# cbg-ethz/LongSom

Measured on AMD Instinct MI355X. Metric: genomic sites/s pileup+call, 10M-read BAM x 5k barcodes, 1/2/4/8 MI355X, higher is better.
Workload: dtype u32

## Files before the change

### longsom_amd/csrc/call.hip

```cpp
#include "lsg_ctx.h"
#include "call_rec.h"
#include "bb_tail.h"
#include <cstdio>
#include <cstring>
#include <cstdlib>
#include <hipcub/hipcub.hpp>

namespace lsg {

enum { CT_CAND = 0, CT_NCAND = 1, CT_HEADS = 4, CT_PASS = 6, CT_LIGHT = 16, CT_HEAVY = 32, CT_QTAIL = 48, CT_DEFER = 64, CT_WORDS = 80 };
struct CallArgs {
    const uint32_t* ne_units; const uint64_t* ne_mask; const uint32_t* ne_rowbase; const int2* ne_geom;
    uint32_t n_ne; int32_t n_ct;
    const uint32_t* rows[LSG_MAX_CELLTYPES]; uint64_t row_cap;
    const uint8_t* const* ref_ptr; const int64_t* contig_len;
    lsg_call_params p;
    double lgc0[2], lgcn[2];
    uint32_t* pass_list;
    const int16_t* tail_table;
    uint32_t* site_cnt; uint32_t* site_off;
    SiteRec* sites; CandCt* cands; uint64_t cand_cap;
    struct TailTask* light; struct TailTask* heavy; uint64_t task_cap;
    unsigned long long* counters;
    uint32_t arena_waves;
// ... 215 lines not shown
        h_next = h_new + (tot_h - h_room); h_end = h_new + HEAVY_CHUNK * ((tot_h - h_room + HEAVY_CHUNK - 1) / HEAVY_CHUNK);
    } else h_next += tot_h;
    if (!site) continue;
    const uint32_t cand = cbase + (uint32_t)__popcll(cm & below);
    uint32_t li = pl - n_light, hi = ph - n_heavy;
    const int16_t* TT = a.tail_table;
    auto table_at = [&](uint32_t k, uint32_t n, int set) { return TT[tail_in_table(k, n) ? (uint32_t)set * TAIL_ENTRIES + tail_index(k, n) : 0u]; };
    int16_t t_bc[NCT][4], t_cc[NCT][4];
#pragma unroll
    for (int ct = 0; ct < NCT; ++ct) {
#pragma unroll
        for (int s = 0; s < 4; ++s) { t_bc[ct][s] = 0; t_cc[ct][s] = 0; }
    }
    if (cm) {
#pragma unroll
        for (int ct = 0; ct < NCT; ++ct) {
#pragma unroll
            for (int s = 0; s < 4; ++s) { t_bc[ct][s] = table_at(v_bc[ct][s], v_dp[ct], 0); t_cc[ct][s] = table_at(v_cc[ct][s], v_nc[ct], 1); }
        }
    }
    const int16_t t_nb = table_at((uint32_t)s_alts_bc, (uint32_t)s_dp, 0), t_nc = table_at((uint32_t)s_alts_cc, (uint32_t)s_nc, 1);
    auto emit_task = [&](uint32_t k, uint32_t n, int set, int16_t* dst, int16_t* loc, int16_t from_table) {
        if (tail_in_table(k, n)) { *loc = from_table; return; }
        TailTask t; t.k = k; t.n = n; t.dst = (uint64_t)dst | (uint64_t)set;
        if (tail_work(k, n) > 64) { const uint32_t p = hi < h_room ? h_old + hi : h_new + (hi - h_room); if (p < a.task_cap) a.heavy[p] = t; ++hi; }
        else { const uint32_t p = li < l_room ? l_old + li : l_new + (li - l_room); if (p < a.task_cap) a.light[p] = t; ++li; }
    };

    SiteRec sr;
    sr.key = ((int64_t)tid << 32) | pos; sr.ref = refb; sr.present = 0; sr.considered = 0; sr.has_cand = 0;
    sr.pad[0] = sr.pad[1] = sr.pad[2] = 0; sr.pad2 = 0; sr.cand = has_any ? cand : 0xFFFFFFFFu;
    sr.site_filter = 0;
    int n_considered = 0;
    bool alts_differ = false;
    uint32_t first_altset = 0; bool have_first = false;
    int lc_up = 0, lc_down = 0;
    SiteRec* srp = &a.sites[idx];
    const bool all_known = (n_light | n_heavy) == 0u;
    int f_pass = 0, f_nonsig = 0, f_with = 0; bool f_multi = false;

#pragma unroll
    for (int ct = 0; ct < NCT; ++ct) {
        CandCt cd;
        cd.n_alt = 0; cd.ct_filter = 0; cd.pad[0] = cd.pad[1] = 0;
#pragma unroll
        for (int q = 0; q < LSG_CALL_MAX_ALT; ++q) { cd.alt[q] = 0; cd.alt_bc[q] = 0; cd.alt_cc[q] = 0; cd.p_bc[q] = 0; cd.p_cc[q] = 0; }
        CandCt* cdp = has_any && cand < a.cand_cap ? &a.cands[(uint64_t)cand * NCT + ct] : nullptr;
        if ((mask[ct] >> lane) & 1ull) {
            sr.present |= (uint8_t)(1u << ct);
            const uint32_t dp = v_dp[ct], nc = v_nc[ct];
            if ((int)dp >= P.min_cov && (int)nc >= P.min_cells) {
                sr.considered |= (uint8_t)(1u << ct);
                ++n_considered;
                int na = 0; uint32_t altset = 0;
#pragma unroll
                for (int oi = 0; oi < 4; ++oi) {
                    const int s = order[oi];
                    const uint32_t b = v_bc[ct][s];
                    if (s == rsym || b == 0) continue;
                    const uint32_t c = v_cc[ct][s];
                    if (na < LSG_CALL_MAX_ALT) {
                        cd.alt[na] = (uint8_t)s; cd.alt_bc[na] = b; cd.alt_cc[na] = c;
                        if (cdp) { emit_task(b, dp, 0, &cdp->p_bc[na], &cd.p_bc[na], t_bc[ct][s]); emit_task(c, nc, 1, &cdp->p_cc[na], &cd.p_cc[na], t_cc[ct][s]); }
                    }
                    ++na; altset |= 1u << s;
                }
                cd.n_alt = (uint8_t)na;
                if (na > 0) {
                    sr.has_cand |= (uint8_t)(1u << ct);
                    if (!have_first) { first_altset = altset; have_first = true; } else if (altset != first_altset) alts_differ = true;
                    if (have_ctx) {
                        int first_s = -1, last_s = -1;
                        for (int oi = 0; oi < 4; ++oi) { const int s = order[oi]; if ((altset >> s) & 1u) { if (first_s < 0) first_s = s; last_s = s; } }
                        const int u = base_of_sym(first_s) == up4 ? up_run + 1 : 1;
                        const int ub = u > up_best ? u : up_best;
                        lc_up = ub > lc_up ? ub : lc_up;
                        int db = 1;
                        if (down_len > 0) { const int d = base_of_sym(last_s) == dn0 ? dn_run + 1 : 1; db = d > dn_best ? d : dn_best; }
                        lc_down = db > lc_down ? db : lc_down;
                    }
                }
            }
        }
        if (all_known && cd.n_alt > 0) {
            int32_t min_pbc = 100000, min_pcc = 100000;
#pragma unroll
            for (int q = 0; q < LSG_CALL_MAX_ALT; ++q) if (q < (int)cd.n_alt) { min_pbc = cd.p_bc[q] < min_pbc ? cd.p_bc[q] : min_pbc; min_pcc = cd.p_cc[q] < min_pcc ? cd.p_cc[q] : min_pcc; }
            uint8_t f;
            if (min_pbc >= 500 || min_pcc >= 500) f = LSG_CF_NONSIG;
            else if ((min_pbc > 10 && min_pbc < 500) || (min_pcc > 10 && min_pcc < 500)) f = LSG_CF_LOWSIG;
            else if (cd.n_alt > 1) f = LSG_CF_MULTI;
            else if ((int)cd.alt_cc[0] < P.min_ac_cells) f = LSG_CF_LOW_CELLS;
            else if ((int)cd.alt_bc[0] < P.min_ac_reads) f = LSG_CF_LOW_READS;
            else f = LSG_CF_PASS;
            cd.ct_filter = f;
            ++f_with; f_pass += f == LSG_CF_PASS; f_nonsig += f == LSG_CF_NONSIG; f_multi |= f == LSG_CF_MULTI;
        }
        if (cdp) *cdp = cd;
    }
    sr.cell_types_min = (uint8_t)n_considered;
    sr.sum_alts_bc = s_alts_bc; sr.sum_dp = s_dp; sr.sum_alts_cc = s_alts_cc; sr.sum_nc = s_nc;
    sr.noise_p_bc = -1; sr.noise_p_cc = -1;
    if (s_alts_bc > 0) {
        sr.noise_p_bc = -2; sr.noise_p_cc = -2;
        if (s_dp >= 0) emit_task((uint32_t)s_alts_bc, (uint32_t)s_dp, 0, &srp->noise_p_bc, &sr.noise_p_bc, t_nb);
        if (s_nc >= 0 && s_alts_cc >= 0) emit_task((uint32_t)s_alts_cc, (uint32_t)s_nc, 1, &srp->noise_p_cc, &sr.noise_p_cc, t_nc);
    }
    uint32_t sf = 0;
    if (sr.has_cand) {
        sf |= LSG_SF_CANDIDATE;
        if (alts_differ) sf |= LSG_SF_MULTI_ALLELIC;
        if (n_considered < P.min_cell_types) sf |= LSG_SF_MIN_CELL_TYPES;
        if (have_ctx && lc_up >= 4) sf |= LSG_SF_LC_UP;
        if (have_ctx && lc_down >= 4) sf |= LSG_SF_LC_DOWN;
    }
    bool pass_site = false;
    if (all_known) {
        const int32_t npb = sr.noise_p_bc, npc = sr.noise_p_cc;
        if (sr.has_cand) {
            if (f_pass > P.max_cell_types) sf |= LSG_SF_MULTIPLE_CELL_TYPES;
            if (f_multi) sf |= LSG_SF_MULTI_ALLELIC;
            if (f_with - f_pass - f_nonsig > 0) sf |= LSG_SF_CELL_TYPE_NOISE;
            if (s_alts_bc > 0 && ((npb >= 0 && npb < 500) || (npc >= 0 && npc < 500))) sf |= LSG_SF_NOISY_SITE;
            pass_site = sf == (uint32_t)LSG_SF_CANDIDATE && f_pass > 0;
        } else if (s_alts_bc > 0 && ((npb >= 0 && npb < 10) || (npc >= 0 && npc < 10))) sf |= LSG_SF_NOISY_SITE;
    }
    sr.site_filter = sf;
    *srp = sr;
    if (pass_site) {
        const unsigned long long q = atomicAdd(&a.counters[CT_PASS], 1ull);
        if (q < PASS_CAP) a.pass_list[q] = (uint32_t)idx;
    }
    const unsigned long long dm = __ballot(!all_known);
    if (dm) {
        unsigned long long q0 = 0;
        if (lane == __ffsll((long long)dm) - 1) q0 = atomicAdd(&a.counters[CT_DEFER], (unsigned long long)__popcll(dm));
        q0 = ((unsigned long long)(uint32_t)__shfl((int)(uint32_t)(q0 >> 32), __ffsll((long long)dm) - 1) << 32) | (uint32_t)__shfl((int)(uint32_t)q0, __ffsll((long long)dm) - 1);
        const unsigned long long q = q0 + __popcll(dm & below);
        if (!all_known && q < a.defer_cap) a.defer_list[q] = (uint32_t)idx;
    }
    }
    TailTask nul; nul.k = 0; nul.n = 0; nul.dst = 0;
    for (uint32_t p = l_next + (uint32_t)lane; p < l_end; p += 64) if (p < a.task_cap) a.light[p] = nul;
    for (uint32_t p = h_next + (uint32_t)lane; p < h_end; p += 64) if (p < a.task_cap) a.heavy[p] = nul;
    if (lane == 0 && n_cand_exact) atomicAdd(&a.counters[CT_NCAND], (unsigned long long)n_cand_exact);
}

__device__ __forceinline__ double tail_of_task(const TailTask& t, const CallArgs& a) {
    const int set = (int)(t.dst & 1ull);
    const double al = set ? a.p.alpha2 : a.p.alpha1, be = set ? a.p.beta2 : a.p.beta1;
    return bb_upper_tail(t.k, t.n, al, be, bb_pm0(t.n, al, be, a.lgc0[set]), a.lgcn[set]);
}

__global__ __launch_bounds__(256) void k_call_tails(CallArgs a) {
    const uint64_t n_all = a.counters[CT_LIGHT] + (uint64_t)a.arena_waves * TASK_CHUNK;
    const uint64_t n = n_all < a.task_cap ? n_all : a.task_cap;
    for (uint64_t i = (uint64_t)blockIdx.x * blockDim.x + threadIdx.x; i < n; i += (uint64_t)gridDim.x * blockDim.x) {
        const TailTask t = a.light[i];
        if (!(t.dst & ~1ull)) continue;
        *reinterpret_cast<int16_t*>(t.dst & ~1ull) = (int16_t)round4(tail_of_task(t, a));
    }
}

template <int G>
__device__ __forceinline__ double group_tail(uint32_t k, uint32_t n, int set, const CallArgs& a, int lane, bool live = true) {
    const double al = set ? a.p.alpha2 : a.p.alpha1, be = set ? a.p.beta2 : a.p.beta1;
    const double dn = (double)n;
    const bool lower = (uint64_t)k <= (uint64_t)n - k + 1;
    const uint32_t m_lo = lower ? 0u : k, m_hi = live ? (lower ? k : n + 1) : m_lo;
    const uint32_t cnt = m_hi - m_lo, chunk = (cnt + G - 1) / G;
    const uint32_t b = m_lo + (uint32_t)(lane & (G - 1)) * chunk;
    const uint32_t e = b + chunk < m_hi ? b + chunk : m_hi;
    double sum = 0.0;
    if (b < e) {
        double pm = exp(bb_logpmf((double)b, dn, al, be));
        sum = pm;
        for (uint32_t m = b + 1; m < e; ++m) {
            if (((m - b) & 1023u) == 0) pm = exp(bb_logpmf((double)m, dn, al, be));
            else { const double mm = (double)(m - 1); pm *= (dn - mm) * (mm + al) / ((mm + 1.0) * (dn - mm - 1.0 + be)); }
            sum += pm;
        }
    }
    for (int o = G / 2; o > 0; o >>= 1) sum += __shfl_down(sum, o, G);
    return lower ? 1.0 - sum : sum;
}
__device__ __forceinline__ uint32_t tail_terms(uint32_t k, uint32_t n) { return (uint64_t)k <= (uint64_t)n - k + 1 ? k : n + 1 - k; }
constexpr uint32_t GROUP8_MAX_TERMS = 1024;

__global__ __launch_bounds__(256) void k_tail_table(CallArgs a, int16_t* table) {
    const int lane = threadIdx.x & 63;
    const uint64_t n_thr = (uint64_t)gridDim.x * blockDim.x, tid = (uint64_t)blockIdx.x * blockDim.x + threadIdx.x;
    for (uint64_t i = tid; i < 2ull * TAIL_ENTRIES; i += n_thr) {
        const int set = i >= TAIL_ENTRIES;
        const uint32_t idx = (uint32_t)(i - (set ? TAIL_ENTRIES : 0));
        uint32_t n = (uint32_t)((sqrt(8.0 * (double)idx + 1.0) - 1.0) * 0.5);
        while (tail_index(0, n + 1) <= idx) ++n;
        while (tail_index(0, n) > idx) --n;
        const uint32_t k = idx - tail_index(0, n);
        if (tail_work(k, n) > 64) continue;
        TailTask t; t.k = k; t.n = n; t.dst = (uint64_t)set;
        table[i] = (int16_t)round4(tail_of_task(t, a));
    }
    for (uint64_t i = tid >> 3; i < 2ull * TAIL_ENTRIES; i += n_thr >> 3) {
        const int set = i >= TAIL_ENTRIES;
        const uint32_t idx = (uint32_t)(i - (set ? TAIL_ENTRIES : 0));
        uint32_t n = (uint32_t)((sqrt(8.0 * (double)idx + 1.0) - 1.0) * 0.5);
        while (tail_index(0, n + 1) <= idx) ++n;
        while (tail_index(0, n) > idx) --n;
        const uint32_t k = idx - tail_index(0, n);
        const bool heavy = tail_work(k, n) > 64;
        const double tail = group_tail<8>(k, n, set, a, lane, heavy);
        if (heavy && (lane & 7) == 0) table[i] = (int16_t)round4(tail);
    }
}

__global__ __launch_bounds__(256) void k_call_tails_heavy(CallArgs a) {
    const int lane = threadIdx.x & 63;
    const uint64_t n_all = a.counters[CT_HEAVY] + (uint64_t)a.arena_waves * HEAVY_CHUNK;
    const uint64_t n_tasks = n_all < a.task_cap ? n_all : a.task_cap;
    const uint64_t n_waves = ((uint64_t)gridDim.x * blockDim.x) >> 6;
    uint64_t batch = ((uint64_t)blockIdx.x * blockDim.x + threadIdx.x) >> 6;
    const uint64_t n_batches = (n_tasks + 15) / 16;
    while (batch < n_batches) {
        const uint64_t i = (uint64_t)lane * n_batches + batch;
        TailTask t; t.k = 0; t.n = 0; t.dst = 0;
        if (lane < 16 && i < n_tasks) t = a.heavy[i];
        const bool is_live = (t.dst & ~1ull) != 0;
        const bool is_big = is_live && tail_terms(t.k, t.n) > GROUP8_MAX_TERMS;
#pragma unroll
        for (int round = 0; round < 2; ++round) {
            const int l = 8 * round + (lane >> 3);
            const uint32_t k = (uint32_t)__shfl((int)t.k, l), n = (uint32_t)__shfl((int)t.n, l);
            const uint64_t dst = ((uint64_t)(uint32_t)__shfl((int)(uint32_t)(t.dst >> 32), l) << 32) | (uint32_t)__shfl((int)(uint32_t)t.dst, l);
            const bool mine = (dst & ~1ull) != 0 && tail_terms(k, n) <= GROUP8_MAX_TERMS;
            if (__ballot(mine) == 0ull) continue;
            const double tail = group_tail<8>(k, n, (int)(dst & 1ull), a, lane, mine);
            if (mine && (lane & 7) == 0) *reinterpret_cast<int16_t*>(dst & ~1ull) = (int16_t)round4(tail);
        }
        unsigned long long big = __ballot(is_big);
        while (big) {
            const int l = __ffsll((long long)big) - 1; big &= big - 1;
            const uint32_t k = (uint32_t)__shfl((int)t.k, l), n = (uint32_t)__shfl((int)t.n, l);
            const uint64_t dst = ((uint64_t)(uint32_t)__shfl((int)(uint32_t)(t.dst >> 32), l) << 32) | (uint32_t)__shfl((int)(uint32_t)t.dst, l);
            const double tail = group_tail<64>(k, n, (int)(dst & 1ull), a, lane);
            if (lane == 0) *reinterpret_cast<int16_t*>(dst & ~1ull) = (int16_t)round4(tail);
        }
        unsigned long long nb = 0;
        if (lane == 0) nb = atomicAdd(&a.counters[CT_QTAIL], 1ull) + n_waves;
        batch = ((uint64_t)(uint32_t)__builtin_amdgcn_readfirstlane((int)(uint32_t)(nb >> 32)) << 32) | (uint32_t)__builtin_amdgcn_readfirstlane((int)(uint32_t)nb);
    }
}

__global__ void k_call_finish(CallArgs a, uint32_t n_sites) {
    const unsigned long long n_def = a.counters[CT_DEFER] < a.defer_cap ? a.counters[CT_DEFER] : a.defer_cap;
    for (unsigned long long j = (unsigned long long)blockIdx.x * blockDim.x + threadIdx.x; j < n_def; j += (unsigned long long)gridDim.x * blockDim.x) {
    const uint32_t i = a.defer_list[j];
    if (i >= n_sites) continue;
    SiteRec s = a.sites[i];
    const lsg_call_params& P = a.p;
    const int32_t npb = s.noise_p_bc, npc = s.noise_p_cc;
    const bool bc_lt05 = npb >= 0 && npb < 500, cc_lt05 = npc >= 0 && npc < 500;
    const bool bc_lt001 = npb >= 0 && npb < 10, cc_lt001 = npc >= 0 && npc < 10;
    uint32_t sf = s.site_filter;
    if (s.has_cand) {
        int n_pass = 0, n_nonsig = 0, n_with = 0; bool any_multi = false;
        for (int ct = 0; ct < a.n_ct; ++ct) {
            if (!((s.has_cand >> ct) & 1u)) continue;
            CandCt* d = &a.cands[(uint64_t)s.cand * a.n_ct + ct];
            const int na = d->n_alt;
            int32_t min_pbc = 100000, min_pcc = 100000;
            for (int q = 0; q < na && q < LSG_CALL_MAX_ALT; ++q) { min_pbc = d->p_bc[q] < min_pbc ? d->p_bc[q] : min_pbc; min_pcc = d->p_cc[q] < min_pcc ? d->p_cc[q] : min_pcc; }
            uint8_t f;
            if (min_pbc >= 500 || min_pcc >= 500) f = LSG_CF_NONSIG;
            else if ((min_pbc > 10 && min_pbc < 500) || (min_pcc > 10 && min_pcc < 500)) f = LSG_CF_LOWSIG;
            else if (na > 1) f = LSG_CF_MULTI;
            else if ((int)d->alt_cc[0] < P.min_ac_cells) f = LSG_CF_LOW_CELLS;
            else if ((int)d->alt_bc[0] < P.min_ac_reads) f = LSG_CF_LOW_READS;
            else f = LSG_CF_PASS;
            d->ct_filter = f;
            ++n_with; n_pass += f == LSG_CF_PASS; n_nonsig += f == LSG_CF_NONSIG; any_multi |= f == LSG_CF_MULTI;
        }
        if (n_pass > P.max_cell_types) sf |= LSG_SF_MULTIPLE_CELL_TYPES;
        if (any_multi) sf |= LSG_SF_MULTI_ALLELIC;
        if (n_with - n_pass - n_nonsig > 0) sf |= LSG_SF_CELL_TYPE_NOISE;
        if (s.sum_alts_bc > 0 && (bc_lt05 || cc_lt05)) sf |= LSG_SF_NOISY_SITE;
        if (sf == (uint32_t)LSG_SF_CANDIDATE && n_pass > 0) {
            const unsigned long long idx = atomicAdd(&a.counters[CT_PASS], 1ull);
            if (idx < PASS_CAP) a.pass_list[idx] = i;
        }
    } else if (s.sum_alts_bc > 0 && (bc_lt001 || cc_lt001)) {
        sf |= LSG_SF_NOISY_SITE;
    }
    if (sf != s.site_filter) a.sites[i].site_filter = sf;
    }
}

__device__ __forceinline__ bool keep_site(const SiteRec& s, const CandCt* cands, int n_ct, int kind) {
    if (kind == 0) return true;
    if (kind == 1) return s.site_filter != 0;
    if (s.site_filter != (uint32_t)LSG_SF_CANDIDATE) return false;
    bool pass = false;
    for (int ct = 0; ct < n_ct; ++ct) pass |= cands[(uint64_t)s.cand * n_ct + ct].ct_filter == LSG_CF_PASS;
    return pass;
}
__global__ void k_flag_keep(const SiteRec* sites, const CandCt* cands, int n_ct, int64_t n, int kind, uint32_t* keep) {
    int64_t i = (int64_t)blockIdx.x * blockDim.x + threadIdx.x;
    if (i <= n) keep[i] = (i < n && keep_site(sites[i], cands, n_ct, kind)) ? 1u : 0u;
}
__device__ __forceinline__ void expand_site(const SiteRec& s, const CandCt* cands, int n_ct, const uint8_t* const* ref_ptr, const int64_t* contig_len,
                                            lsg_call* dst) {
    lsg_call c;
    memset(&c, 0, sizeof(c));
    c.key = s.key; c.ref = s.ref; c.present = s.present; c.considered = s.considered; c.has_cand = s.has_cand;
    c.site_filter = s.site_filter; c.cell_types_min = s.cell_types_min;
    c.sum_alts_bc = s.sum_alts_bc; c.sum_dp = s.sum_dp; c.sum_alts_cc = s.sum_alts_cc; c.sum_nc = s.sum_nc;
    c.noise_p_bc = s.noise_p_bc; c.noise_p_cc = s.noise_p_cc;
    if (s.cand != 0xFFFFFFFFu) {
        for (int ct = 0; ct < n_ct; ++ct) {
            const CandCt& d = cands[(uint64_t)s.cand * n_ct + ct];
            c.n_alt[ct] = d.n_alt; c.ct_filter[ct] = d.ct_filter;
            for (int q = 0; q < LSG_CALL_MAX_ALT; ++q) {
                c.alt[ct][q] = d.alt[q]; c.alt_bc[ct][q] = d.alt_bc[q]; c.alt_cc[ct][q] = d.alt_cc[q];
                c.p_bc[ct][q] = d.p_bc[q]; c.p_cc[ct][q] = d.p_cc[q];
            }
        }
    }
    const int tid = (int)(s.key >> 32);
    const int64_t pos = s.key & 0xffffffffll;
    if (pos >= 5) {
        const uint8_t* ref = ref_ptr[tid];
        for (int q = 0; q < 5; ++q) c.up_ctx[q] = ref[pos - 5 + q];
        for (int q = 0; q < 5 && pos + 1 + q < contig_len[tid]; ++q) c.down_ctx[q] = ref[pos + 1 + q];
    }
    *dst = c;
}
__global__ void k_expand(const SiteRec* sites, const CandCt* cands, int n_ct, int64_t n, const uint32_t* keep, const uint32_t* off,
                         const uint8_t* const* ref_ptr, const int64_t* contig_len, lsg_call* out) {
    int64_t i = (int64_t)blockIdx.x * blockDim.x + threadIdx.x;
    if (i >= n || !keep[i]) return;
    expand_site(sites[i], cands, n_ct, ref_ptr, contig_len, out + off[i]);
}
__global__ __launch_bounds__(1024) void k_expand_list(const SiteRec* sites, const CandCt* cands, int n_ct, const uint32_t* list, uint32_t n,
                                                      const uint8_t* const* ref_ptr, const int64_t* contig_len, lsg_call* out) {
    __shared__ uint32_t v[PASS_CAP];
    const uint32_t t = threadIdx.x;
    uint32_t m = 1; while (m < n) m <<= 1;
    for (uint32_t i = t; i < m; i += 1024) v[i] = i < n ? list[i] : 0xFFFFFFFFu;
    __syncthreads();
    for (uint32_t k = 2; k <= m; k <<= 1)
        for (uint32_t j = k >> 1; j > 0; j >>= 1) {
            for (uint32_t i = t; i < m; i += 1024) {
                const uint32_t l = i ^ j;
                if (l > i) {
                    const uint32_t x = v[i], y = v[l];
                    if (((i & k) == 0) == (x > y)) { v[i] = y; v[l] = x; }
                }
            }
            __syncthreads();
        }
    for (uint32_t i = t; i < n; i += 1024) expand_site(sites[v[i]], cands, n_ct, ref_ptr, contig_len, out + i);
}

__global__ void k_probe(const int64_t* set, int64_t n_set, const int64_t* keys, int64_t n, uint8_t* hits) {
    int64_t i = (int64_t)blockIdx.x * blockDim.x + threadIdx.x;
    if (i >= n) return;
    const int64_t key = keys[i];
    int64_t lo = 0, hi = n_set;
    while (lo < hi) { int64_t mid = (lo + hi) >> 1; if (set[mid] < key) lo = mid + 1; else hi = mid; }
    hits[i] = (lo < n_set && set[lo] == key) ? 1 : 0;
}

__global__ void k_sf4_batch(const uint32_t* k, const uint32_t* n, int64_t items, double al, double be, double lgc0, double lgcn, int32_t* out, double* raw) {
    for (int64_t i = (int64_t)blockIdx.x * blockDim.x + threadIdx.x; i < items; i += (int64_t)gridDim.x * blockDim.x) {
        const double p = bb_upper_tail(k[i], n[i], al, be, bb_pm0(n[i], al, be, lgc0), lgcn);
        out[i] = round4(p);
        if (raw) raw[i] = p;
    }
}

int run_sf4(lsg_ctx* c, int64_t items, const uint32_t* k, const uint32_t* n, double al, double be, int32_t* out, double* raw) {
    if (items < 0 || (items > 0 && (!k || !n || !out))) { set_error("lsg_betabinom_sf4: bad arguments"); return -2; }
    if (!(al > 0.0) || !(be > 0.0)) { set_error("lsg_betabinom_sf4: alpha and beta must be positive"); return -2; }
    if (items == 0) return 0;
    hipStream_t st = c->stream;
    DevBuf dk, dn, dout, draw;
    auto done = [&](int rc) { dk.release(); dn.release(); dout.release(); draw.release(); return rc; };
    if (dk.reserve((size_t)items * 4) || dn.reserve((size_t)items * 4) || dout.reserve((size_t)items * 4) || (raw && draw.reserve((size_t)items * 8))) return done(-1);
    if (hipMemcpyAsync(dk.p, k, (size_t)items * 4, hipMemcpyHostToDevice, st) != hipSuccess ||
        hipMemcpyAsync(dn.p, n, (size_t)items * 4, hipMemcpyHostToDevice, st) != hipSuccess) { set_error("lsg_betabinom_sf4: upload failed"); return done(-1); }
    unsigned g = (unsigned)((items + 255) / 256); if (g > (unsigned)(c->n_cus * 16)) g = (unsigned)(c->n_cus * 16);
    hipLaunchKernelGGL(k_sf4_batch, dim3(g), dim3(256), 0, st, dk.as<uint32_t>(), dn.as<uint32_t>(), items, al, be,
                       lgamma(al + be) - lgamma(be), lgamma(al + be) - lgamma(al), dout.as<int32_t>(), raw ? draw.as<double>() : (double*)nullptr);
    if (raw && hipMemcpyAsync(raw, draw.p, (size_t)items * 8, hipMemcpyDeviceToHost, st) != hipSuccess) { set_error("lsg_betabinom_sf4: failed"); return done(-1); }
    if (hipMemcpyAsync(out, dout.p, (size_t)items * 4, hipMemcpyDeviceToHost, st) != hipSuccess || hipStreamSynchronize(st) != hipSuccess) { set_error("lsg_betabinom_sf4: failed"); return done(-1); }
    return done(0);
}

struct HasSites {
    const uint32_t* cnt;
    __host__ __device__ bool operator()(const uint32_t& w) const { return cnt[w] != 0; }
};

static int run_call_sized(lsg_ctx* c, const lsg_call_params* p, uint32_t tasks_per_site);
int run_call(lsg_ctx* c, const lsg_call_params* p) {
    int rc = run_call_sized(c, p, c->call_tasks_per_site);
    if (rc == -3) {
        c->call_tasks_per_site = (uint32_t)(8 * c->n_ct + 2);
        rc = run_call_sized(c, p, c->call_tasks_per_site);
    }
    return rc;
}
static int run_call_sized(lsg_ctx* c, const lsg_call_params* p, uint32_t tasks_per_site) {
    if (!c->counted) { set_error("lsg_call_step1: call lsg_pileup_count first"); return -2; }
    for (int t = 0; t < c->n_contigs; ++t)
        if (!c->ref_ptr[t]) { set_error("lsg_call_step1: reference of contig %d not loaded", t); return -2; }
    hipStream_t st = c->stream;
    const uint32_t n_ne = c->n_ne;
    c->n_sites = 0; c->n_cand = 0; c->n_pass = -1;
    if (n_ne == 0) { c->called = true; return 0; }
    if (c->d_site_off.reserve((size_t)(n_ne + 2) * 12 + 128 + CT_WORDS * 8 + (size_t)n_ne * 72 + 64)) return -1;
    CallArgs a{};
    a.ne_units = c->d_ne_units.as<uint32_t>(); a.ne_mask = c->d_ne_mask.as<uint64_t>(); a.ne_rowbase = c->d_ne_rowbase.as<uint32_t>();
    a.ne_geom = c->ws[WS_NE_GEOM].as<int2>();
    a.n_ne = n_ne; a.n_ct = c->n_ct;
    for (int i = 0; i < LSG_MAX_CELLTYPES; ++i) a.rows[i] = c->d_rows[i].as<uint32_t>();
    for (int i = 0; i < c->n_ct; ++i) if (!a.rows[i] || c->d_rows[i].cap < ROW_BLOCK_WORDS * 4) { set_error("lsg_call_step1: a cell type has no row block"); return -2; }
    a.row_cap = c->row_cap;
    a.ref_ptr = c->d_ref_ptrs.as<const uint8_t*>(); a.contig_len = c->d_contig_len.as<int64_t>();
    a.p = *p;
    a.lgc0[0] = lgamma(p->alpha1 + p->beta1) - lgamma(p->beta1); a.lgcn[0] = lgamma(p->alpha1 + p->beta1) - lgamma(p->alpha1);
    a.lgc0[1] = lgamma(p->alpha2 + p->beta2) - lgamma(p->beta2); a.lgcn[1] = lgamma(p->alpha2 + p->beta2) - lgamma(p->alpha2);
    {
        const double key[4] = {p->alpha1, p->beta1, p->alpha2, p->beta2};
        if (!c->tail_table_valid || memcmp(key, c->tail_table_key, sizeof key) != 0) {
            if (c->d_tail_table.reserve((size_t)2 * TAIL_ENTRIES * 2)) return -1;
            hipLaunchKernelGGL(k_tail_table, dim3((unsigned)(c->n_cus * 8)), dim3(256), 0, st, a, c->d_tail_table.as<int16_t>());
            memcpy(c->tail_table_key, key, sizeof key); c->tail_table_valid = true;
        }
        a.tail_table = c->d_tail_table.as<int16_t>();
    }
    if (c->d_pass_list.reserve((size_t)PASS_CAP * 4)) return -1;
    a.pass_list = c->d_pass_list.as<uint32_t>();
    a.site_cnt = c->d_site_off.as<uint32_t>();
    a.site_off = a.site_cnt + (n_ne + 2);
    a.counters = reinterpret_cast<unsigned long long*>(a.site_off + (n_ne + 2));
    uint32_t* heads = reinterpret_cast<uint32_t*>(a.counters + CT_WORDS);
    a.heads = heads;
    a.head_recs = reinterpret_cast<uint32_t*>((reinterpret_cast<uintptr_t>(heads + n_ne) + 63) & ~(uintptr_t)63);
    a.head_ref = reinterpret_cast<uint64_t*>(a.head_recs + (size_t)n_ne * 16);
    LSG_HIP(hipMemsetAsync(a.counters, 0, CT_WORDS * 8, st));
    hipLaunchKernelGGL(k_site_count, dim3((n_ne + 256) / 256), dim3(256), 0, st, a);
    size_t tb = 0;
    LSG_HIP(hipcub::DeviceScan::ExclusiveSum(nullptr, tb, a.site_cnt, a.site_off, (int)(n_ne + 1), st));
    if (c->d_cub_tmp.reserve(tb + 256)) return -1;
    tb = c->d_cub_tmp.cap;
    LSG_HIP(hipcub::DeviceScan::ExclusiveSum(c->d_cub_tmp.p, tb, a.site_cnt, a.site_off, (int)(n_ne + 1), st));
    {
        HasSites pred{a.site_cnt};
        hipcub::CountingInputIterator<uint32_t> it(0);
        uint32_t* d_nh = reinterpret_cast<uint32_t*>(a.counters + CT_HEADS);
        size_t tb2 = 0;
        LSG_HIP(hipcub::DeviceSelect::If(nullptr, tb2, it, heads, d_nh, (int)n_ne, pred, st));
        if (c->d_cub_tmp.reserve(tb2 + 256)) return -1;
        tb2 = c->d_cub_tmp.cap;
        LSG_HIP(hipcub::DeviceSelect::If(c->d_cub_tmp.p, tb2, it, heads, d_nh, (int)n_ne, pred, st));
    }
    hipLaunchKernelGGL(k_head_recs, dim3((n_ne + 255) / 256), dim3(256), 0, st, a);
    LSG_HIP(hipMemcpyAsync(c->h_pin, a.site_off + n_ne, 4, hipMemcpyDeviceToHost, st));
    LSG_HIP(hipStreamSynchronize(st));
    const uint32_t n_sites = *reinterpret_cast<const uint32_t*>(c->h_pin);
    if (n_sites > 0) {
        if (c->d_calls.reserve((size_t)n_sites * sizeof(SiteRec))) return -1;
        const unsigned gather_grid = (unsigned)(c->n_cus * 4);
        const uint64_t gather_waves = (uint64_t)gather_grid * GATHER_WAVES;
        if (c->ws[WS_CALL_CANDS].reserve(((size_t)n_sites + (size_t)2 * gather_waves * CAND_CHUNK) * sizeof(CandCt) * (size_t)c->n_ct)) return -1;
        a.arena_waves = (uint32_t)gather_waves;
        a.sites = c->d_calls.as<SiteRec>(); a.cands = c->ws[WS_CALL_CANDS].as<CandCt>(); a.cand_cap = n_sites + 2 * gather_waves * CAND_CHUNK;
        a.task_cap = (uint64_t)n_sites * (uint64_t)(8 * c->n_ct + 2);
        if (a.task_cap > (uint64_t)n_sites * tasks_per_site + 1024) a.task_cap = (uint64_t)n_sites * tasks_per_site + 1024;
        if (a.task_cap > 0x7fffffffull) a.task_cap = 0x7fffffffull;
        a.task_cap += gather_waves * TASK_CHUNK * 3;
        if (c->ws[WS_CALL_TASKS].reserve((size_t)a.task_cap * sizeof(TailTask) * 2)) return -1;
        a.light = c->ws[WS_CALL_TASKS].as<TailTask>(); a.heavy = a.light + a.task_cap;
        a.defer_cap = n_sites;
        if (c->d_defer_list.reserve((size_t)a.defer_cap * 4 + 64)) return -1;
        a.defer_list = c->d_defer_list.as<uint32_t>();
        switch (c->n_ct) {
            case 1: hipLaunchKernelGGL(k_call_gather<1>, dim3(gather_grid), dim3(GATHER_WAVES * 64), 0, st, a); break;
            case 2: hipLaunchKernelGGL(k_call_gather<2>, dim3(gather_grid), dim3(GATHER_WAVES * 64), 0, st, a); break;
            case 3: hipLaunchKernelGGL(k_call_gather<3>, dim3(gather_grid), dim3(GATHER_WAVES * 64), 0, st, a); break;
            default: hipLaunchKernelGGL(k_call_gather<4>, dim3(gather_grid), dim3(GATHER_WAVES * 64), 0, st, a); break;
        }
        hipLaunchKernelGGL(k_call_tails, dim3((unsigned)(c->n_cus * 16)), dim3(256), 0, st, a);
        hipLaunchKernelGGL(k_call_tails_heavy, dim3((unsigned)(c->n_cus * 8)), dim3(256), 0, st, a);
        hipLaunchKernelGGL(k_call_finish, dim3((unsigned)(c->n_cus * 2)), dim3(256), 0, st, a, n_sites);
        LSG_HIP(hipGetLastError());
    }
    unsigned long long cnt4[CT_WORDS];
    LSG_HIP(hipMemcpyAsync(c->h_pin, a.counters, CT_WORDS * 8, hipMemcpyDeviceToHost, st));
    LSG_HIP(hipStreamSynchronize(st));
    memcpy(cnt4, c->h_pin, CT_WORDS * 8);
    if (getenv("LSG_TIMING")) fprintf(stderr, "[lsg] call: %u sites in %llu tiles, light task slots %llu (+%llu of the first chunks), heavy %llu (+%llu), sites that waited for a tail %llu, PASS %llu\n", n_sites, cnt4[CT_HEADS],
                                      cnt4[CT_LIGHT], (unsigned long long)a.arena_waves * TASK_CHUNK, cnt4[CT_HEAVY], (unsigned long long)a.arena_waves * HEAVY_CHUNK, cnt4[CT_DEFER], cnt4[CT_PASS]);
    c->n_pass = (int64_t)cnt4[CT_PASS];
    const unsigned long long cand = cnt4[CT_NCAND];
    if (n_sites > 0 && (cnt4[CT_LIGHT] + (uint64_t)a.arena_waves * TASK_CHUNK > a.task_cap || cnt4[CT_HEAVY] + (uint64_t)a.arena_waves * HEAVY_CHUNK > a.task_cap)) { set_error("lsg_call_step1: tail task buffer too small (%llu/%llu tasks)", cnt4[CT_LIGHT], cnt4[CT_HEAVY]); return -3; }
    c->n_sites = n_sites; c->n_cand = (int64_t)cand;
    c->called = true;
    return 0;
}

int run_select_calls(lsg_ctx* c, int kind, lsg_call* dst_device, int64_t capacity, int64_t* n_out) {
    if (!c->called) { set_error("lsg_export_calls: call lsg_call_step1 first"); return -2; }
    hipStream_t st = c->stream;
    const int64_t n = c->n_sites;
    if (n_out) *n_out = 0;
    if (n == 0) return 0;
    if (kind == 2 && c->n_pass >= 0 && c->n_pass <= (int64_t)PASS_CAP && !getenv("LSG_NO_PASS_LIST")) {
        const int64_t k = c->n_pass;
        if (n_out) *n_out = k;
        if (!dst_device || k == 0) return 0;
        if (k > capacity) { set_error("lsg_export_calls: capacity %lld < %lld rows", (long long)capacity, (long long)k); return -2; }
        hipLaunchKernelGGL(k_expand_list, dim3(1), dim3(1024), 0, st, c->d_calls.as<SiteRec>(), c->ws[WS_CALL_CANDS].as<CandCt>(), c->n_ct,
                           c->d_pass_list.as<uint32_t>(), (uint32_t)k, c->d_ref_ptrs.as<const uint8_t*>(), c->d_contig_len.as<int64_t>(), dst_device);
        LSG_HIP(hipGetLastError());
        LSG_HIP(hipStreamSynchronize(st));
        if (getenv("LSG_TIMING")) fprintf(stderr, "[lsg] export: kind 2 from the PASS list, %lld rows\n", (long long)k);
        return 0;
    }
    DevBuf& flags = c->ws[WS_CALL_FLAGS];
    if (flags.reserve((size_t)(n + 2) * 8)) return -1;
    uint32_t* keep = flags.as<uint32_t>();
    uint32_t* off = keep + (n + 2);
    const SiteRec* sites = c->d_calls.as<SiteRec>();
    const CandCt* cands = c->ws[WS_CALL_CANDS].as<CandCt>();
    hipLaunchKernelGGL(k_flag_keep, dim3((unsigned)((n + 256) / 256)), dim3(256), 0, st, sites, cands, c->n_ct, n, kind, keep);
    size_t tb = 0;
    LSG_HIP(hipcub::DeviceScan::ExclusiveSum(nullptr, tb, keep, off, (int)(n + 1), st));
    if (c->d_cub_tmp.reserve(tb + 256)) return -1;
    tb = c->d_cub_tmp.cap;
    LSG_HIP(hipcub::DeviceScan::ExclusiveSum(c->d_cub_tmp.p, tb, keep, off, (int)(n + 1), st));
    LSG_HIP(hipMemcpyAsync(c->h_pin, off + n, 4, hipMemcpyDeviceToHost, st));
    LSG_HIP(hipStreamSynchronize(st));
    const uint32_t k = *reinterpret_cast<const uint32_t*>(c->h_pin);
    if (n_out) *n_out = k;
    if (!dst_device || k == 0) return 0;
    if ((int64_t)k > capacity) { set_error("lsg_export_calls: capacity %lld < %lld rows", (long long)capacity, (long long)k); return -2; }
    hipLaunchKernelGGL(k_expand, dim3((unsigned)((n + 255) / 256)), dim3(256), 0, st, sites, cands, c->n_ct, n, keep, off,
                       c->d_ref_ptrs.as<const uint8_t*>(), c->d_contig_len.as<int64_t>(), dst_device);
    LSG_HIP(hipGetLastError());
    LSG_HIP(hipStreamSynchronize(st));
    if (kind == 2 && getenv("LSG_TIMING")) fprintf(stderr, "[lsg] export: kind 2 from the scan, %u rows\n", k);
    return 0;
}

int run_fetch_calls(lsg_ctx* c, lsg_call* out, int64_t capacity, int candidates_only, int64_t* n_out) {
    if (!c->called) { set_error("lsg_fetch_calls: call lsg_call_step1 first"); return -2; }
    hipStream_t st = c->stream;
    if (n_out) *n_out = 0;
    if (c->n_sites == 0) return 0;
    int64_t k = 0;
    int rc = run_select_calls(c, candidates_only, nullptr, 0, &k);
    if (rc) return rc;
    if (k > capacity) { set_error("lsg_fetch_calls: capacity %lld < %lld rows", (long long)capacity, (long long)k); return -2; }
    if (k > 0) {
        DevBuf& sel = c->ws[WS_CALL_SEL];
        if (sel.reserve((size_t)k * sizeof(lsg_call))) return -1;
        rc = run_select_calls(c, candidates_only, sel.as<lsg_call>(), k, &k);
        if (rc) return rc;
        LSG_HIP(hipMemcpyAsync(out, sel.p, (size_t)k * sizeof(lsg_call), hipMemcpyDeviceToHost, st));
        LSG_HIP(hipStreamSynchronize(st));
    }
    if (n_out) *n_out = k;
    return 0;
}

int run_probe(lsg_ctx* c, const PosSet& s, const char* who, const int64_t* keys, int64_t n, uint8_t* hits, int on_device) {
    hipStream_t st = c->stream;
    if (n == 0) return 0;
    DevBuf dk, dh;
    const int64_t* k = keys; uint8_t* h = hits;
    int rc = 0;
    if (!on_device) {
        if (dk.reserve((size_t)n * 8) || dh.reserve((size_t)n)) { dk.release(); dh.release(); return -1; }
        if (hipMemcpyAsync(dk.p, keys, (size_t)n * 8, hipMemcpyHostToDevice, st) != hipSuccess) rc = -1;
        k = dk.as<int64_t>(); h = dh.as<uint8_t>();
    }
    if (!rc) {
        hipLaunchKernelGGL(k_probe, dim3((unsigned)((n + 255) / 256)), dim3(256), 0, st, s.keys.as<int64_t>(), s.n, k, n, h);
        if (!on_device && hipMemcpyAsync(hits, dh.p, (size_t)n, hipMemcpyDeviceToHost, st) != hipSuccess) rc = -1;
        if (hipStreamSynchronize(st) != hipSuccess) rc = -1;
    }
    if (rc) set_error("%s: %s", who, hipGetErrorString(hipGetLastError()));
    dk.release(); dh.release();
    return rc;
}

}
```

### longsom_amd/csrc/lsg_ctx.h

```cpp
#pragma once
#include <hip/hip_runtime.h>
#include <cstdint>
#include <cstdio>
#include <string>
#include <vector>
#include "../../include/longsom_hip.h"
#include "../../include/longsom_synth.h"

namespace lsg {

constexpr int TILE_W = 64;
constexpr int ROW_PLANES = 34;
constexpr int NCTR = 33;

constexpr int ROW_QUADS = (ROW_PLANES + 3) / 4;
constexpr uint64_t ROW_BLOCK_WORDS = (uint64_t)ROW_QUADS * 256;
constexpr uint64_t ROW_STORED_WORDS = (uint64_t)ROW_QUADS * 4;
constexpr uint32_t ROW_NARROW = 1u << 31;
constexpr uint32_t ROW_NARROW_MAX = 256;
static_assert(ROW_NARROW_MAX * 255u < (1u << 16), "a narrow row's quality sum (two planes share a word) fits 16 bits");
__host__ __device__ inline uint64_t row_word(uint64_t row, int plane) {
    return (row >> 6) * ROW_BLOCK_WORDS + (uint64_t)(plane >> 2) * 256 + (row & 63) * 4 + (uint64_t)(plane & 3);
}

void set_error(const char* fmt, ...);
const char* get_error();

#define LSG_HIP(call)                                                                          \
    do {                                                                                       \
        hipError_t e_ = (call);                                                                \
        if (e_ != hipSuccess) {                                                                \
            lsg::set_error("%s failed: %s (%s:%d)", #call, hipGetErrorString(e_), __FILE__, __LINE__); \
            return -1;                                                                         \
        }                                                                                      \
    } while (0)

struct DevBuf {
    void* p = nullptr;
    size_t cap = 0;
    int reserve(size_t bytes) {
        if (bytes <= cap) return 0;
        if (p) { (void)hipFree(p); p = nullptr; cap = 0; }
        const size_t slack = bytes / 16 < ((size_t)64 << 20) ? bytes / 16 : ((size_t)64 << 20);
        size_t want = bytes + slack + 256;
        LSG_HIP(hipMalloc(&p, want));
        cap = want;
        return 0;
    }
    void release() { if (p) (void)hipFree(p); p = nullptr; cap = 0; }
    template <class T> T* as() const { return reinterpret_cast<T*>(p); }
};

struct PosSet { DevBuf keys; int64_t n = 0; };

struct CellGeno {
    DevBuf keys, alt_sym, is_chrm, dp, alt, vaf4, p4, status, bin, n_cov, n_pass, text, scratch, filt;
    int64_t n_sites = 0; int32_t n_cb = 0; bool valid = false;
    bool cells_only = false;
    bool text_valid = false; int64_t n_long = 0, n_mat = 0; int32_t n_cols = 0, float_cells = 0;
    size_t head_off_at = 0, index_off_at = 0, label_off_at = 0, cb_off_at = 0, ct_off_at = 0, long_order_at = 0, mat_order_at = 0, col_src_at = 0,
           head_at = 0, index_at = 0, label_at = 0, cb_at = 0, ct_at = 0;
    bool filt_valid = false; int64_t n_rows_kept = 0; int32_t n_cols_kept = 0;
    size_t f_row_mut_at = 0, f_cov_kept_at = 0, f_cov_all_at = 0, f_rows_at = 0, f_cols_at = 0, f_nsel_at = 0, f_row_keep_at = 0, f_col_keep_at = 0,
           f_col_int_at = 0, f_col_ok_at = 0;
    void release() { for (DevBuf* b : {&keys, &alt_sym, &is_chrm, &dp, &alt, &vaf4, &p4, &status, &bin, &n_cov, &n_pass, &text, &scratch, &filt}) b->release(); valid = text_valid = filt_valid = false; }
};

struct Bnpc {
    DevBuf lab, raw, params, dist, cuts, sums, rank, flags, owner, cl16, idx, mean, part, ord2, small;
    DevBuf work, wsmall, rec;
    std::vector<double> Z;
    std::vector<int32_t> cut_order;
    int64_t n_samples = 0; int32_t n_cells = 0, pitch = 0, k_max = 0, n_muts = 0;
    bool valid = false, dist_valid = false, has_params = false, tree_valid = false;
    void release() {
        for (DevBuf* b : {&lab, &raw, &params, &dist, &cuts, &sums, &rank, &flags, &owner, &cl16, &idx, &mean, &part, &ord2, &small, &work, &wsmall, &rec}) b->release();
        Z = {}; cut_order = {};
        valid = dist_valid = has_params = tree_valid = false;
    }
};

struct Bnpcs {
    DevBuf one, zero, pop, seeds, lab, size, colof, live, nlive, hi, theta, L1, L0, LL, alpha, prow, n1, n0, rowml, rowb, order, keys, rec_lab, rec_sc, arena, err;
    DevBuf sm_i, sm_d, sm_c, sm_t, rec_sm;
    DevBuf rates, rec_err, err_cnt, err_out;
    DevBuf psrf, psrf_out;
    DevBuf used;
    double err_prob = 0.0, err_prior[4] = {}, mix[2] = {};
    bool learn = false, fixed_assign = false;
    double sm_prob = 0.0, sm_ratio[2] = {0.75, 0.25};
    int32_t sm_scans = 3;
    int32_t n_cells = 0, n_muts = 0, n_words = 0, n_chains = 0, steps1 = 0, k_max = 0, ll_pitch = 0, pending = -1, next_step = 0;
    int32_t test_ml_end = 0;
    int64_t arena_rows = 0;
    double p = 1.0, q = 1.0, g0 = 0.0, g1 = 0.0, dpa_prob = 0.0, betaln = 0.0;
    bool valid = false, prepared = false;
    std::vector<int32_t> h_k;
    std::vector<int64_t> h_used;
    void release() {
        for (DevBuf* b : {&one, &zero, &pop, &seeds, &lab, &size, &colof, &live, &nlive, &hi, &theta, &L1, &L0, &LL, &alpha, &prow, &n1, &n0, &rowml, &rowb, &order, &keys, &rec_lab, &rec_sc,
                          &arena, &err, &sm_i, &sm_d, &sm_c, &sm_t, &rec_sm, &rates, &rec_err, &err_cnt, &err_out, &psrf, &psrf_out, &used}) b->release();
        valid = prepared = false;
    }
};

struct Bbfit {
    DevBuf hist, tails, out, ref, tmp;
    int64_t cap = 0;
    bool valid = false;
    void release() { for (DevBuf* b : {&hist, &tails, &out, &ref, &tmp}) b->release(); valid = false; cap = 0; }
};

struct GeneCounts {
    DevBuf iv, row_of_gene, matrix, tallies, state, small, text, scratch;
    int64_t n_iv = 0; int32_t n_genes = 0, n_rows = 0, n_cb = 0, n_cols = 0; char sep = ',';
    bool ann_valid = false, mat_valid = false, text_valid = false;
    size_t row_off_at = 0, col_src_at = 0, col_off_at = 0, row_txt_at = 0, col_txt_at = 0;
    void release() { for (DevBuf* b : {&iv, &row_of_gene, &matrix, &tallies, &state, &small, &text, &scratch}) b->release(); ann_valid = mat_valid = text_valid = false; n_iv = 0; n_genes = n_rows = n_cb = n_cols = 0; }
};

enum { WS_NE_NSLOT = 0, WS_NE_ACC, WS_NE_GEOM, WS_MULTI_LIST, WS_MACC, WS_EXPORT_K, WS_EXPORT_R,
       WS_EXPORT_C, WS_CALL_FLAGS, WS_CALL_SEL, WS_CALL_CANDS, WS_CALL_TASKS, WS_SEG_INFO };

constexpr uint32_t CB_MASK = 0x00FFFFFFu;
constexpr uint32_t TM_RUNSTART = 1u << 31, TM_FWD = 1u << 30, TM_WHI = 1u << 29;
constexpr uint32_t TM_PAD_S0 = CB_MASK | TM_RUNSTART;
constexpr int TM_GROUP = 4;
enum { TM_STORE = 0, TM_S0, TM_B, TM_RD, TM_META, TM_BLK_TILE, TM_BLK_OFF, TM_EXT,
       TM_JOBS, TM_NE_UNITS, TM_NE_GEOM, TM_NE_NSLOT, TM_NE_ACC, TM_MULTI, TM_CHUNKS, TM_NBUF };
struct TmJob { uint32_t e0, e1, w0, slab, nj, cnt, tile, emid, base, off; int32_t tstart, tid; };
constexpr int TM_JOB_WORDS = 12;
static_assert(sizeof(TmJob) == 4 * TM_JOB_WORDS, "TmJob layout");
constexpr uint32_t TMJ_WIDE = 1u << 31;
constexpr int TM_JOB_TGT = 3072, TM_JOB_LIMIT = 4095;

}

struct lsg_ctx;
namespace lsg {
int build_store(lsg_ctx* c, const uint16_t* events, int64_t n_events, const int64_t* seg_ev_off, const lsg_reads* src = nullptr);
int ensure_plan(lsg_ctx* c);
void drop_store(lsg_ctx* c);
int live_read_bound(lsg_ctx* c);
int live_read_bound_exact(lsg_ctx* c);
int live_read_bound_all(lsg_ctx* c);
__global__ void k_read_end(const uint32_t* seg_read, const int32_t* seg_start, const int32_t* seg_len, int64_t n_segs, int32_t* read_end);
__global__ void k_read_end_init(const int32_t* read_pos, int64_t n_reads, int32_t* read_end);
int depth_cap_drops(lsg_ctx* c, const lsg_count_params* p);
struct GatherCountSrc { const uint16_t* events; int64_t n_events; const uint64_t* key; const uint32_t* rdv; int32_t cb_bits; int32_t src_shift; int32_t wsh; };
int unit_row_offsets(lsg_ctx* c, int ct, const uint32_t** off);
int run_gather_count(lsg_ctx* c, const lsg_count_params* p, const GatherCountSrc& src, bool direct);
}

struct lsg_ctx {
    int device = 0;
    hipStream_t stream = nullptr;
    hipStream_t own_stream = nullptr;
    hipStream_t copy_stream = nullptr;
    hipEvent_t ev_copy = nullptr;
    hipEvent_t ev_blk = nullptr;
    hipEvent_t ev_lpt = nullptr;
    hipEvent_t ev[6] = {nullptr, nullptr, nullptr, nullptr, nullptr, nullptr};
    hipEvent_t evb[5] = {nullptr, nullptr, nullptr, nullptr, nullptr};

    int32_t n_contigs = 0;
    std::vector<int64_t> contig_len;
    std::vector<uint32_t> tile_base;
    uint32_t n_tiles = 0;
    uint32_t tile_lo = 0, tile_hi = 0;
    lsg::DevBuf d_tile_base, d_contig_len, d_ref_ptrs;
    std::vector<lsg::DevBuf> ref;
    std::vector<const uint8_t*> ref_ptr;

    int32_t n_cb = 0, n_ct = 0;
    lsg::DevBuf d_celltype_of, d_ct_rank;
    std::vector<uint8_t> h_celltype_of;
    uint32_t ct_size[LSG_MAX_CELLTYPES] = {0, 0, 0, 0};

    lsg_reads rd{};
    lsg::DevBuf b_read_tid, b_read_pos, b_read_flag, b_read_mapq, b_read_cb;
    lsg::DevBuf b_seg_read, b_seg_start, b_seg_len, b_seg_ev_off, b_events;
    int32_t plp_window = 50000, st_window = 50000;
    int32_t lf_min_mq = 0, lf_ignore_orphans = 0; uint32_t lf_flag_exclude = 0;
    int32_t st_min_mq = 0, st_ignore_orphans = 0; uint32_t st_flag_exclude = 0;
    bool keep_unlisted = false;
    int32_t split_max_nm = -1, split_max_nh = -1, split_n_trim = 0;
    int64_t split_n[18] = {}, split_first[18] = {};
    bool keep_reads = false;
    lsg::DevBuf d_tile_cap, d_tile_off;
    lsg::DevBuf tm[lsg::TM_NBUF];
    lsg::DevBuf bt[18];
    uint64_t tm_n = 0;
    int64_t tm_events = 0;
    uint64_t tm_np = 0;
    uint32_t tm_nblk = 0, tm_njobs = 0, tm_nchunks = 0, tm_n_ne = 0, tm_n_multi = 0, tm_n_slabs = 0, tm_n_wide = 0;
    int plan_n_ct = 0;
    int plan1_n_ct = 0;
    uint32_t plan1_tot[4] = {0, 0, 0, 0};
    uint32_t plan_misc[2] = {0, 0};
    uint32_t* d_plan_misc = nullptr;
    bool cal_enabled = false; lsg_count_params cal_params{};
    bool counted_at_load = false;
    bool load_was_fused = false;
    bool tm_valid = false;
    int32_t store_policy = 0;
    bool store_skipped = false;
    double layout_build_ms = 0;
    float build_ms[4] = {0, 0, 0, 0};
    int64_t max_live_reads = -1;
    int64_t max_live_all = -1;
    int32_t wsh = 0;
    int32_t events_layout = 0;
    const void* hint_phased_events = nullptr;
    bool src_phased = false;
    bool line_loads = false;
    int64_t max_live_exact = -1;
    lsg::DevBuf d_read_drop;
    lsg::DevBuf d_drop_pairs; int64_t n_drop_pairs = 0;
    lsg::DevBuf d_read_adm;
    bool has_drops = false;
    int64_t n_depth_dropped = 0;

    lsg::DevBuf d_read_key;
    lsg::DevBuf d_ne_units, d_ne_mask, d_ne_rowbase, d_ne_rowoff, d_scalars, d_cub_tmp, d_ix_stat;
    lsg::DevBuf d_rows[LSG_MAX_CELLTYPES];
    uint64_t row_cap = 0;
    uint32_t arena = 256;
    uint32_t n_ne = 0;
    int64_t n_rows[LSG_MAX_CELLTYPES] = {0, 0, 0, 0};
    int64_t n_columns = 0;
    lsg_count_params last_params{};
    lsg_count_stats stats{};
    bool counted = false;

    lsg::DevBuf d_calls, d_site_off, d_tail_table;
    double tail_table_key[4] = {0, 0, 0, 0}; bool tail_table_valid = false;
    int64_t n_sites = 0, n_cand = 0, n_pass = -1;
    lsg::DevBuf d_pass_list, d_defer_list, d_xcd_queues;
    uint32_t call_tasks_per_site = 1;
    bool called = false;

    lsg::DevBuf tab_keys[LSG_MAX_CELLTYPES], tab_refs[LSG_MAX_CELLTYPES], tab_rows[LSG_MAX_CELLTYPES], tab_names, tab_scratch, tab_scratch2;
    int32_t tab_scratch_table = -1; int64_t tab_scratch_rows = 0;
    uint64_t tab_rows_serial[LSG_MAX_CELLTYPES] = {0, 0, 0, 0};
    uint64_t count_serial = 0;
    lsg::DevBuf tab_text[LSG_TABLE_ALL_SLOTS];
    int64_t tab_bytes[LSG_TABLE_ALL_SLOTS];
    lsg_ctx() { for (auto& b : tab_bytes) b = -1; }
    int32_t tab_n_contigs = 0, tab_n_ct = 0; uint32_t tab_ct_off_at = 0, tab_order_at = 0, tab_ct_txt_at = 0, tab_contig_txt_at = 0;

    lsg::CellGeno cg;

    lsg::Bnpc bnpc;
    lsg::Bnpcs bnpcs;
    lsg::Bbfit bb;
    lsg::GeneCounts gc;

    lsg::PosSet posset[3];
    lsg::PosSet alleleset; bool alleleset_loaded = false;
    lsg::DevBuf syn[12];
    lsg::DevBuf gen[10];
    lsg::DevBuf ws[16];
    int n_cus = 256;
    unsigned long long* h_pin = nullptr;
    uint32_t n_multi = 0;
};
```

### longsom_amd/csrc/pileup.hip

```cpp
#include "lsg_ctx.h"
#include <hipcub/hipcub.hpp>
#include <cstdio>
#include <cstdlib>
#include <cstring>

namespace lsg {

#define LSG_AS3 __attribute__((address_space(3)))
__device__ __forceinline__ uint32_t lds_addr(const void* p) { return (uint32_t)(uintptr_t)(LSG_AS3 const void*)p; }
constexpr int ARENA = 256;

enum { SC_COLS = 8, SC_OVERFLOW = 9, SC_READS = 10, SC_SEGS = 11, SC_EVENTS = 12, SC_ROWS_DEEP = 15,
       SC_ROWS = 16, SC_ROWS_SRC = 28, SC_NENT = 38, SC_QWALK = 48,
       SC_ROWALLOC = 160, SC_ROWALLOC_STRIDE = 16, SC_COUNT = SC_ROWALLOC + SC_ROWALLOC_STRIDE * LSG_MAX_CELLTYPES };

struct CountArgs {
    int64_t n_reads;
    const int32_t* read_tid; const uint16_t* read_flag; const uint8_t* read_mapq; const int32_t* read_cb;
    const int64_t* contig_len; const uint8_t* const* ref_ptr;
    const uint8_t* celltype_of;
    int32_t n_contigs, n_cb, n_ct;
    uint32_t tile_lo, tile_hi;
    int32_t min_bq, min_mq, min_dp, min_cc, ignore_orphans;
    uint32_t flag_exclude;
// ... 1420 lines not shown
            if (jb.nj == 1 && mine) { const int64_t pos = (int64_t)jb.tstart + 64 * wv + lane; if (pos >= 1 && pos < a.contig_len[jb.tid]) refb = a.ref_ptr[jb.tid][pos]; }
            __syncthreads();
            q.ask();
            if (counting) tm_zero_planes<2 * 2 * 2 * 8 * 64, 2 * 2 * 64>(pl, &nc_sh[0][0][0]);
            __syncthreads();
            const uint32_t s0r = wv ? jb.emid : jb.e0, s1r = wv ? jb.e1 : jb.emid;
            const uint32_t i0 = s0r - jb.base, i1 = s1r - jb.base < jb.tcnt ? s1r - jb.base : jb.tcnt;
            if (counting && i1 > i0) {
                TmState st0, st1; st0.nc = 0; st0.mask = 0; st1.nc = 0; st1.mask = 0;
                tw_range(a, tm, tg, st0, st1, stat, i0, i1, jb.off, jb.tcnt, thr, pkl0, one, lane, K64, kb);
                uint32_t* nq = &nc_sh[0][lane >> 5][2 * (lane & 31)];
                if (st0.nc & 0xffffu) atomicAdd(nq, st0.nc & 0xffffu);
                if (st0.nc >> 16) atomicAdd(nq + 128, st0.nc >> 16);
                if (st1.nc & 0xffffu) atomicAdd(nq + 1, st1.nc & 0xffffu);
                if (st1.nc >> 16) atomicAdd(nq + 129, st1.nc >> 16);
            }
            if (threadIdx.x == 0) s_q[2] = q.answer();
            const JobRec cj = jb;
            jb.load(jw);
            prefetch();
            __syncthreads();
            const uint32_t nn = rl(s_q[2], 0);
            if (mine) {
                for (int v = 0; v < 2; ++v) {
                    const int ct = tm.ct_base + v;
                    if (ct >= a.n_ct) break;
                    const uint32_t uw = (uint32_t)wv * (uint32_t)a.n_ct + (uint32_t)ct;
                    tm_finish<TwCounters>(a, pl + v * 1024 + wv * 512, nc_sh[v][wv][lane], cj.w0 + uw, cj.slab + uw * cj.nj, cj.nj, cj.tcnt, ct, cj.tid, cj.tstart + 64 * wv,
                                          lane, &book, refb, 2 * v);
                }
            }
            if (nxt == XcdQueue::NO_JOB) break;
            cur = nxt; nxt = nn;
        }
    }
    lds_fence();
    __syncthreads();
    stat_flush(tg.stat_slots, stat, lane, wv);
    books_flush(a, books, lane);
}

struct WideEntry {
    bool rs; uint32_t cls; bool fwd;
    uint32_t nev; bool segfirst;
    uint32_t ev[2];
};
__device__ __forceinline__ uint32_t tm_meta_one(const CountArgs& a, const TmArgs& tm, uint64_t p) {
    const uint32_t s = tm.s0[p], b8 = tm.b[p], cb = s & CB_MASK;
    uint32_t cls = 2;
    bool ok = cb < (uint32_t)a.n_cb;
    if (ok && a.adm) { const uint32_t r = tm.rd[p]; ok = (reinterpret_cast<const uint32_t*>(a.adm)[r >> 5] >> (r & 31u)) & 1u; }
    if (ok && a.drop_pairs && a.read_drop[tm.rd[p]] == 2) ok = !tm_dropped_here(a, tm.rd[p], tm.blk_tile[p >> 3], s);
    if (ok) { const uint32_t ct = a.celltype_of[cb]; if (ct < (uint32_t)a.n_ct && (ct >> 1) == (uint32_t)(tm.ct_base >> 1)) cls = ct & 1u; }
    uint32_t m = cls < 2 ? (cls ? (TMM_CT4 | TMM_CT12) : 0u) | ((s & TM_FWD) ? TMM_FWD : 0u) | ((b8 & 128u) ? TMM_SINGLE : 0u) : TMM_SKIP;
    if (s & TM_RUNSTART) m |= TMM_RS;
    return m;
}
struct WideFromStore {
    static constexpr int H = 1;
    int inline_meta;
    __device__ __forceinline__ unsigned long long* stat_slots() const { return nullptr; }
    __device__ __forceinline__ WideEntry entry(const CountArgs& a, const TmArgs& tm, const TmJob&, uint32_t p, int lane) const {
        const uint32_t m = rl(inline_meta ? tm_meta_one(a, tm, p) : tm.meta[p], 0);
        WideEntry e{(m & TMM_RS) != 0, (m & TMM_SKIP) ? 2u : ((m & TMM_CT4) ? 1u : 0u), (m & TMM_FWD) != 0, 0u, false, {0u, 0u}};
        if (e.cls < 2) {
            const uint32_t x = tm.ext[p >> 3];
            if ((uint32_t)lane >= (x & 0xffu) && (uint32_t)lane < (x >> 8)) e.ev[0] = reinterpret_cast<const uint16_t*>(tm.store)[((uint64_t)(p >> 3) * 64 + lane) * 8 + (p & 7u)];
        }
        return e;
    }
};
template <int WSH>
struct WideFromKeys {
    static constexpr int H = 1 << WSH;
    TgArgs tg;
    __device__ __forceinline__ unsigned long long* stat_slots() const { return tg.stat_slots; }
    __device__ __forceinline__ WideEntry entry(const CountArgs& a, const TmArgs& tm, const TmJob& jb, uint32_t p, int lane) const {
        constexpr uint32_t PB = 6 + WSH, PM = (1u << PB) - 1u;
        const uint32_t i = p - jb.base, cbm = (1u << tg.cb_bits) - 1u;
        const uint64_t k = tg.key[jb.off + i];
        const uint32_t v = tg.rdv ? tg.rdv[jb.off + i] : (uint32_t)(k >> 32) & (TG_RV_FWD | TG_RV_SEGFIRST), cb = (uint32_t)k & cbm, r = v & TG_RV_READ;
        const uint32_t geom = (uint32_t)(k >> tg.cb_bits), first = geom & PM, nev = ((geom >> PB) & PM) + 1u;
        const uint64_t src = (((k >> (tg.cb_bits + 2 * PB)) & tg.src_mask) << tg.src_shift) | (tg.src_shift ? first : 0u);
        uint32_t cls = 2;
        bool ok = cb < (uint32_t)a.n_cb;
        if (ok && a.adm) ok = (reinterpret_cast<const uint32_t*>(a.adm)[r >> 5] >> (r & 31u)) & 1u;
        if (ok) { const uint32_t ct = a.celltype_of[cb]; if (ct < (uint32_t)a.n_ct && (ct >> 1) == (uint32_t)(tm.ct_base >> 1)) cls = ct & 1u; }
        WideEntry e{i == 0 || ((uint32_t)tg.key[jb.off + i - 1] & cbm) != cb, cls, (v & TG_RV_FWD) != 0, nev, (v & TG_RV_SEGFIRST) != 0, {0u, 0u}};
        if (cls < 2)
            for (int h = 0; h < H; ++h) { const uint32_t q = (uint32_t)(64 * h + lane) - first; if (q < nev) e.ev[h] = tg.events[src + q]; }
        return e;
    }
};
static_assert(TM_JOB_TGT <= TM_JOB_LIMIT, "a one-job tile's job fits the packed planes: the wide walk writes slabs only");
template <class SRC>
__global__ __launch_bounds__(64) void k_tm_walk_wide(CountArgs a, TmArgs tm, SRC src, const uint32_t* n_wide) {
    constexpr int H = SRC::H;
    __shared__ uint32_t pl[H][2][4][8 * 64];
    const int lane = threadIdx.x;
    if (n_wide && rl(*n_wide, 0) == 0u) return;
    const uint32_t thr = bq_threshold(a);
    unsigned long long s_ev = 0, s_sg = 0, s_ne = 0;
    for (uint32_t jx = blockIdx.x; jx < tm.njobs; jx += gridDim.x) {
        const TmJob jb = tm.jobs[jx];
        bool in_t[H], any = false;
        for (int h = 0; h < H; ++h) { const uint32_t t = (uint32_t)H * jb.tile + h; in_t[h] = t >= a.tile_lo && t < a.tile_hi; any |= in_t[h]; }
        if (!(jb.nj & TMJ_WIDE) || !any) continue;
        const uint32_t nj = jb.nj & ~TMJ_WIDE;
        lds_fence();
        for (int i = lane; i < H * 2 * 4 * 8 * 64; i += 64) (&pl[0][0][0][0])[i] = 0;
        lds_fence();
        uint32_t nc[H][2], mask[H], run_ct = 0;
        for (int h = 0; h < H; ++h) { nc[h][0] = nc[h][1] = 0; mask[h] = 0; }
        for (uint32_t p = jb.e0; p < jb.e1 && p - jb.base < jb.cnt; ++p) {
            const WideEntry e = src.entry(a, tm, jb, p, lane);
            if (e.rs) for (int h = 0; h < H; ++h) { nc[h][run_ct] += mask[h] ? 1u : 0u; mask[h] = 0; }
            if (e.cls >= 2) continue;
            s_ev += e.nev; s_sg += e.segfirst ? 1u : 0u; ++s_ne;
            run_ct = e.cls;
            for (int h = 0; h < H; ++h) {
                const uint32_t ev = e.ev[h];
                if ((ev & 0x8ffu) >= thr) {
                    const uint32_t sym = (ev >> 8) & 7u;
                    uint32_t* w = &pl[h][run_ct][0][sym * 64 + lane];
                    w[0] += ev & 0xffu; w[512] += e.fwd ? 1u : 0u; w[1024] += 1u; w[1536] += (mask[h] >> sym) & 1u;
                    mask[h] |= 1u << sym;
                }
            }
        }
        for (int h = 0; h < H; ++h) nc[h][run_ct] += mask[h] ? 1u : 0u;
        lds_fence();
        for (int h = 0; h < H; ++h) {
            if (!in_t[h]) continue;
            for (int v = 0; v < 2; ++v) {
                const int ct = tm.ct_base + v;
                if (ct >= a.n_ct) break;
                const uint32_t* pc = &pl[h][v][0][0];
                uint32_t dp = 0;
#pragma unroll
                for (int k = 0; k < 8; ++k) dp += pc[1024 + k * 64 + lane];
                uint32_t* dst = a.macc + (uint64_t)(jb.slab + ((uint32_t)h * (uint32_t)a.n_ct + (uint32_t)ct) * nj) * (NCTR * 64);
                dst[lane] = dp - nc[h][v];
#pragma unroll
                for (int k = 0; k < 8; ++k) {
                    dst[(1 + k) * 64 + lane] = pc[1536 + k * 64 + lane]; dst[(9 + k) * 64 + lane] = pc[1024 + k * 64 + lane];
                    dst[(17 + k) * 64 + lane] = pc[k * 64 + lane]; dst[(25 + k) * 64 + lane] = pc[512 + k * 64 + lane];
                }
            }
        }
    }
    if (unsigned long long* slots = src.stat_slots()) stat_add(slots, blockIdx.x, s_ev, s_sg, s_ne, lane);
}

struct CountLaunch { CountArgs a; TmArgs tm; unsigned grid_walk, grid_fin; int n_pass; };
struct PrepOp { void* dst; const void* src; uint64_t words; };
struct PrepArgs { PrepOp op[10]; int n; };
__global__ __launch_bounds__(256) void k_prep_ops(PrepArgs a) {
    const uint64_t g = (uint64_t)blockIdx.x * blockDim.x + threadIdx.x, gs = (uint64_t)gridDim.x * blockDim.x;
    for (int k = 0; k < a.n; ++k) {
        uint32_t* d = reinterpret_cast<uint32_t*>(a.op[k].dst);
        const uint32_t* sp = reinterpret_cast<const uint32_t*>(a.op[k].src);
        const uint64_t nq = a.op[k].words / 4;
        for (uint64_t i = g; i < nq; i += gs) reinterpret_cast<uint4*>(d)[i] = sp ? reinterpret_cast<const uint4*>(sp)[i] : make_uint4(0u, 0u, 0u, 0u);
        for (uint64_t i = nq * 4 + g; i < a.op[k].words; i += gs) d[i] = sp ? sp[i] : 0u;
    }
}
static int count_prepare(lsg_ctx* c, const lsg_count_params* p, CountLaunch& L) {
    hipStream_t st = c->stream;
    const uint32_t n_ne = c->tm_n_ne;
    if (c->d_scalars.reserve(SC_COUNT * 8) || c->d_ne_units.reserve(((size_t)n_ne + 2) * 4) ||
        c->d_ne_mask.reserve(((size_t)n_ne + 2) * 8) || c->d_ne_rowbase.reserve(((size_t)n_ne + 2) * 4) || c->ws[WS_NE_NSLOT].reserve(((size_t)n_ne + 2) * 4) ||
        c->ws[WS_NE_ACC].reserve(((size_t)n_ne + 2) * 4) || c->ws[WS_NE_GEOM].reserve(((size_t)n_ne + 2) * 8) || c->ws[WS_MULTI_LIST].reserve(((size_t)c->tm_n_multi + 2) * 4) ||
        c->ws[WS_MACC].reserve(((size_t)c->tm_n_slabs + 1) * NCTR * 64 * 4) || c->d_ix_stat.reserve(IX_STAT_SLOTS * 64) ||
        c->d_read_adm.reserve(((size_t)c->rd.n_reads / 64 + 2) * 8))
        return -1;
    L.grid_walk = (unsigned)(c->n_cus * tune_int("LSG_GRID_TM", 16));
    L.grid_fin = (unsigned)(c->n_cus * 8);
    L.n_pass = (c->n_ct + 1) / 2;
    {
        uint64_t want_rows = (uint64_t)n_ne / (uint64_t)c->n_ct * TILE_W;
        if (p->min_dp > 0) {
            const uint64_t by_depth = (uint64_t)c->rd.n_events / (uint64_t)p->min_dp + 64;
            if (by_depth < want_rows) want_rows = by_depth;
        }
        const uint64_t emitters = (uint64_t)L.grid_walk * TMW_WAVES * 2 + L.grid_fin + (uint64_t)c->n_cus * 4 + (c->wsh ? (uint64_t)c->n_cus * 16 * TMW_WAVES * 4 : 0u);
        uint64_t arena = want_rows / (emitters * 8) / ARENA * ARENA;
        c->arena = (uint32_t)(arena < (uint64_t)ARENA ? (uint64_t)ARENA : (arena > 8ull * ARENA ? 8ull * ARENA : arena));
        want_rows += emitters * c->arena + 64;
        want_rows = (want_rows + 63) / 64 * 64 + 64;
        if (want_rows > c->row_cap) c->row_cap = want_rows;
        for (int i = 0; i < c->n_ct; ++i)
            if (c->d_rows[i].reserve((size_t)c->row_cap * ROW_STORED_WORDS * 4)) return -1;
    }
    c->n_ne = n_ne; c->n_multi = c->tm_n_multi;
    L.a = CountArgs{};
    fill_args(c, p, L.a);
    TmArgs& tm = L.tm;
    tm = TmArgs{};
    tm.store = c->tm[TM_STORE].as<uint4>(); tm.s0 = c->tm[TM_S0].as<uint32_t>(); tm.b = c->tm[TM_B].as<uint8_t>(); tm.rd = c->tm[TM_RD].as<uint32_t>();
    tm.meta = c->tm[TM_META].as<uint32_t>(); tm.blk_tile = c->tm[TM_BLK_TILE].as<uint32_t>(); tm.jobs = c->tm[TM_JOBS].as<TmJob>(); tm.np = c->tm_np; tm.nblk = c->tm_nblk;
    tm.njobs = c->tm_njobs; tm.nchunks = c->tm_nchunks; tm.chunk_start = c->tm[TM_CHUNKS].as<uint32_t>(); tm.ext = c->tm[TM_EXT].as<uint16_t>();
    LSG_HIP(hipEventRecord(c->ev[0], st));
    {
        PrepArgs pa{}; int k = 0;
        auto op = [&](void* dst, const void* src, size_t bytes) { if (bytes) { pa.op[k].dst = dst; pa.op[k].src = src; pa.op[k].words = (bytes + 3) / 4; ++k; } };
        op(c->d_scalars.p, nullptr, SC_COUNT * 8);
        op(c->d_ix_stat.p, nullptr, IX_STAT_SLOTS * 64);
        if (n_ne) {
            op(c->d_ne_units.p, c->tm[TM_NE_UNITS].p, (size_t)n_ne * 4);
            op(c->ws[WS_NE_GEOM].p, c->tm[TM_NE_GEOM].p, (size_t)n_ne * 8);
            op(c->ws[WS_NE_NSLOT].p, c->tm[TM_NE_NSLOT].p, ((size_t)n_ne + 1) * 4);
            op(c->ws[WS_NE_ACC].p, c->tm[TM_NE_ACC].p, ((size_t)n_ne + 1) * 4);
            if (c->tm_n_multi) op(c->ws[WS_MULTI_LIST].p, c->tm[TM_MULTI].p, (size_t)c->tm_n_multi * 4);
            op(c->d_ne_mask.p, nullptr, ((size_t)n_ne + 1) * 8);
            op(c->d_ne_rowbase.p, nullptr, ((size_t)n_ne + 1) * 4);
        }
        pa.n = k;
        hipLaunchKernelGGL(k_prep_ops, dim3((unsigned)(c->n_cus * 4)), dim3(256), 0, st, pa);
    }
    const int64_t R = c->rd.n_reads;
    if (R > 0) { unsigned g = (unsigned)((R + 255) / 256); if (g > (unsigned)(c->n_cus * 8)) g = (unsigned)(c->n_cus * 8); hipLaunchKernelGGL(k_read_stats, dim3(g), dim3(256), 0, st, L.a); }
    return 0;
}
static int count_passes(lsg_ctx* c, CountLaunch& L, int first_pass, bool wide_of_pass0) {
    hipStream_t st = c->stream;
    const unsigned grid_wide = c->tm_n_wide ? (c->tm_n_wide < (unsigned)(c->n_cus * 4) ? c->tm_n_wide : (unsigned)(c->n_cus * 4)) : 0u;
    for (int pass = wide_of_pass0 ? 0 : first_pass; pass < L.n_pass && c->tm_nblk; ++pass) {
        const bool wide_only = pass < first_pass;
        if (wide_only && !grid_wide) continue;
        L.tm.ct_base = 2 * pass;
        if (pass) LSG_HIP(hipMemsetAsync(L.a.scalars + SC_QWALK, 0, 8, st));
        if (L.a.drop_pairs) hipLaunchKernelGGL(k_tm_resolve<true>, dim3((c->tm_nblk + 255) / 256), dim3(256), 0, st, L.a, L.tm, wide_only ? (unsigned long long*)nullptr : c->d_ix_stat.as<unsigned long long>());
        else hipLaunchKernelGGL(k_tm_resolve<false>, dim3((c->tm_nblk + 255) / 256), dim3(256), 0, st, L.a, L.tm, wide_only ? (unsigned long long*)nullptr : c->d_ix_stat.as<unsigned long long>());
        if (pass == 0) { LSG_HIP(hipEventRecord(c->ev[1], st)); LSG_HIP(hipEventRecord(c->ev[3], st)); }
        if (c->tm_njobs && !wide_only) hipLaunchKernelGGL(k_tm_walk, dim3(L.grid_walk), dim3(TMW_WAVES * 64), 0, st, L.a, L.tm);
        if (pass == 0) LSG_HIP(hipEventRecord(c->ev[4], st));
        if (grid_wide) hipLaunchKernelGGL(k_tm_walk_wide<WideFromStore>, dim3(grid_wide), dim3(64), 0, st, L.a, L.tm, WideFromStore{0}, (const uint32_t*)nullptr);
    }
    return 0;
}
static int count_finish(lsg_ctx* c, const lsg_count_params* p, CountLaunch& L) {
    hipStream_t st = c->stream;
    if (c->tm_nblk) hipLaunchKernelGGL(k_resolve_stats, dim3(1), dim3(256), 0, st, L.a, c->d_ix_stat.as<unsigned long long>());
    if (c->tm_n_multi) hipLaunchKernelGGL(k_finalize_multi, dim3(c->tm_n_multi < L.grid_fin ? c->tm_n_multi : L.grid_fin), dim3(FIN_THREADS), 0, st, L.a);
    LSG_HIP(hipEventRecord(c->ev[5], st));
    LSG_HIP(hipGetLastError());
    unsigned long long sc[SC_COUNT];
    if (read_scalars(c, sc)) return -1;
    if (sc[SC_OVERFLOW]) { set_error("lsg_pileup_count: row buffer overflow (cap %llu)", (unsigned long long)c->row_cap); return -3; }
    for (int i = 0; i < LSG_MAX_CELLTYPES; ++i) c->n_rows[i] = (int64_t)sc[SC_ROWS + i];
    c->n_columns = (int64_t)sc[SC_COLS];
    c->stats.n_reads_admitted = (int64_t)sc[SC_READS];
    c->stats.n_segs_admitted = (int64_t)sc[SC_SEGS];
    c->stats.n_events_admitted = (int64_t)sc[SC_EVENTS];
    c->stats.n_units = c->n_ne;
    c->stats.n_deep_units = c->tm_n_multi;
    c->stats.n_entries = (int64_t)sc[SC_NENT];
    float ms = 0;
    LSG_HIP(hipEventElapsedTime(&ms, c->ev[0], c->ev[1])); c->stats.ms_bin = ms;
    LSG_HIP(hipEventElapsedTime(&ms, c->ev[1], c->ev[5])); c->stats.ms_deep = ms;
    LSG_HIP(hipEventElapsedTime(&ms, c->ev[3], c->ev[4])); c->stats.ms_walk = ms;
    c->stats.ms_wave = 0;
    LSG_HIP(hipEventElapsedTime(&ms, c->ev[0], c->ev[5])); c->stats.ms_total = ms;
    for (int i = 0; i < 4; ++i) { c->stats.rows_by_kernel[i] = (int64_t)sc[SC_ROWS_SRC + i]; c->stats.events_by_kernel[i] = 0; }
    c->stats.events_by_kernel[1] = (int64_t)sc[SC_EVENTS];
    c->stats.n_events_wave = 0; c->stats.n_events_deep = (int64_t)sc[SC_EVENTS];
    c->stats.n_rows_deep = (int64_t)sc[SC_ROWS_DEEP];
    c->stats.n_rows_wave = -c->stats.n_rows_deep;
    for (int i = 0; i < LSG_MAX_CELLTYPES; ++i) c->stats.n_rows_wave += c->n_rows[i];
    c->last_params = *p;
    c->counted = true;
    c->called = false;
    ++c->count_serial;
    return 0;
}

int run_gather_count(lsg_ctx* c, const lsg_count_params* p, const GatherCountSrc& src, bool direct) {
    hipStream_t st = c->stream;
    c->has_drops = false; c->n_depth_dropped = 0;
    CountLaunch L;
    if (int rc = count_prepare(c, p, L)) return rc;
    TgArgs tg{};
    tg.events = src.events; tg.n_events = src.n_events; tg.key = src.key; tg.rdv = src.rdv; tg.cb_bits = src.cb_bits;
    tg.src_mask = (1ull << ((src.rdv ? 52 : 50) - src.cb_bits)) - 1ull; tg.src_shift = src.src_shift;
    if (!src.rdv && (!direct || L.a.adm)) return 1;
    tg.tile_off = c->d_tile_off.as<uint32_t>(); tg.blk_off = c->tm[TM_BLK_OFF].as<uint32_t>();
    tg.s0 = c->tm[TM_S0].as<uint32_t>(); tg.b8 = c->tm[TM_B].as<uint8_t>(); tg.rd = c->tm[TM_RD].as<uint32_t>();
    tg.store = c->tm[TM_STORE].as<uint4>(); tg.ext = c->tm[TM_EXT].as<uint16_t>();
    tg.nchunks = c->d_plan_misc + 1; tg.stat_slots = c->d_ix_stat.as<unsigned long long>();
    L.tm.ct_base = 0;
    const bool dbg = getenv("LSG_DEBUG_SYNC") != nullptr;
    auto stage = [&](const char* what) { if (dbg) { const hipError_t e = hipStreamSynchronize(st); fprintf(stderr, "[lsg] fused load: %s: %s\n", what, hipGetErrorString(e)); fflush(stderr); } };
    stage("count prepared");
    LSG_HIP(hipEventRecord(c->ev[1], st)); LSG_HIP(hipEventRecord(c->ev[3], st));
    enum { GATHER, TILES, WINDOWS } form = !direct ? GATHER : (src.wsh ? WINDOWS : TILES);
    const char* what = "k_tm_gather_count";
    if (direct) {
        if (c->d_xcd_queues.reserve(8 * 128)) return -1;
        LSG_HIP(hipMemsetAsync(c->d_xcd_queues.p, 0, 8 * 128, st));
        tg.queues = c->d_xcd_queues.as<unsigned long long>();
    }
    if (form == WINDOWS) {
        if (tg.rdv || L.a.adm || p->min_bq < 1 || p->min_bq > 255 || tg.src_shift != 7) return 1;
        tg.src_mask = (1ull << (48 - src.cb_bits)) - 1ull;
        c->line_loads = true;
        const unsigned gridw = (unsigned)(c->n_cus * tune_int("LSG_GRID_TW", 9));
        hipLaunchKernelGGL(k_tm_count_win, dim3(gridw), dim3(TMW_WAVES * 64), 0, st, L.a, L.tm, tg);
        what = "k_tm_count_win";
    } else if (form == TILES) {
        const unsigned grid = (unsigned)(c->n_cus * tune_int("LSG_GRID_TD", 12));
        const bool al = tg.src_shift == 6 && p->min_bq >= 1 && p->min_bq <= 255;
        c->line_loads = al;
        if (tg.rdv && al) hipLaunchKernelGGL((k_tm_count_direct<false, true>), dim3(grid), dim3(TMW_WAVES * 64), 0, st, L.a, L.tm, tg);
        else if (tg.rdv) hipLaunchKernelGGL((k_tm_count_direct<false, false>), dim3(grid), dim3(TMW_WAVES * 64), 0, st, L.a, L.tm, tg);
        else if (al) hipLaunchKernelGGL((k_tm_count_direct<true, true>), dim3(grid), dim3(TMW_WAVES * 64), 0, st, L.a, L.tm, tg);
        else hipLaunchKernelGGL((k_tm_count_direct<true, false>), dim3(grid), dim3(TMW_WAVES * 64), 0, st, L.a, L.tm, tg);
        what = "k_tm_count_direct";
    } else {
        const unsigned grid = (unsigned)(c->n_cus * tune_int("LSG_GRID_TG", 9));
        hipLaunchKernelGGL(k_tm_gather_count, dim3(grid), dim3(TMW_WAVES * 64), 0, st, L.a, L.tm, tg);
    }
    LSG_HIP(hipEventRecord(c->ev[4], st));
    LSG_HIP(hipEventRecord(c->evb[4], st));
    stage(what);
    const dim3 grid_wide((unsigned)(c->n_cus * 2));
    const uint32_t* n_wide = c->d_plan_misc;
    if (form == WINDOWS) hipLaunchKernelGGL(k_tm_walk_wide<WideFromKeys<1>>, grid_wide, dim3(64), 0, st, L.a, L.tm, WideFromKeys<1>{tg}, n_wide);
    else if (form == TILES) hipLaunchKernelGGL(k_tm_walk_wide<WideFromKeys<0>>, grid_wide, dim3(64), 0, st, L.a, L.tm, WideFromKeys<0>{tg}, n_wide);
    else hipLaunchKernelGGL(k_tm_walk_wide<WideFromStore>, grid_wide, dim3(64), 0, st, L.a, L.tm, WideFromStore{1}, n_wide);
    stage("wide walk");
    return count_finish(c, p, L);
}

int run_count(lsg_ctx* c, const lsg_count_params* p) {
    if (c->n_contigs <= 0) { set_error("lsg_pileup_count: no contigs set"); return -2; }
    if (c->n_ct <= 0) { set_error("lsg_pileup_count: no barcodes set"); return -2; }
    if (c->store_skipped) { set_error("lsg_pileup_count: the load kept no store (lsg_set_store_policy): only the count it made is there - load the reads again to count with other parameters, tables or regions"); return -2; }
    if (!c->tm_valid) { set_error("lsg_pileup_count: no reads loaded"); return -2; }
    for (int t = 0; t < c->n_contigs; ++t)
        if (!c->ref_ptr[t]) { set_error("lsg_pileup_count: reference of contig %d not loaded", t); return -2; }
    if (int rc = ensure_plan(c)) return rc;
    if (depth_cap_drops(c, p)) return -1;
    CountLaunch L;
    if (int rc = count_prepare(c, p, L)) return rc;
    hipStream_t st = c->stream;
    if (int rc = count_passes(c, L, 0, false)) return rc;
    if (!c->tm_nblk) { LSG_HIP(hipEventRecord(c->ev[1], st)); LSG_HIP(hipEventRecord(c->ev[3], st)); LSG_HIP(hipEventRecord(c->ev[4], st)); }
    c->counted_at_load = false;
    return count_finish(c, p, L);
}

__global__ void k_unit_rowcount(const uint32_t* ne_units, const uint64_t* ne_mask, uint32_t n_ne, int n_ct, int ct, uint32_t* cnt) {
    uint32_t w = blockIdx.x * blockDim.x + threadIdx.x;
    if (w > n_ne) return;
    uint32_t v = 0;
    if (w < n_ne && (int)(ne_units[w] % (uint32_t)n_ct) == ct) v = (uint32_t)__popcll(ne_mask[w]);
    cnt[w] = v;
}

__global__ void k_export_rows(CountArgs a, int ct, const uint32_t* rowoff, int64_t* keys, uint8_t* refs, uint32_t* counts) {
    const int lane = threadIdx.x & 63;
    uint32_t w = (uint32_t)(((uint64_t)blockIdx.x * blockDim.x + threadIdx.x) >> 6);
    if (w >= a.n_ne) return;
    const int2 geom = a.ne_geom[w];
    if ((int)((uint32_t)geom.y >> 24) != ct) return;
    const int tid = geom.y & 0xffffff;
    uint64_t em = a.ne_mask[w];
    if (!((em >> lane) & 1ull)) return;
    const uint32_t rb = a.ne_rowbase[w];
    uint64_t src = (uint64_t)(rb & ~ROW_NARROW) + __popcll(em & ((1ull << lane) - 1ull));
    uint64_t dst = (uint64_t)rowoff[w] + __popcll(em & ((1ull << lane) - 1ull));
    int64_t pos = (int64_t)geom.x + lane;
    keys[dst] = ((int64_t)tid << 32) | pos;
    refs[dst] = a.ref_ptr[tid][pos];
    if (rb & ROW_NARROW) {
        const uint16_t* h = reinterpret_cast<const uint16_t*>(a.rows[ct] + (src >> 6) * ROW_BLOCK_WORDS);
        for (int k = 0; k < ROW_PLANES; ++k) counts[dst * LSG_ROW_WORDS + k] = h[(k >> 2) * 256 + (src & 63) * 4 + (k & 3)];
    } else {
        for (int k = 0; k < ROW_PLANES; ++k) counts[dst * LSG_ROW_WORDS + k] = a.rows[ct][row_word(src, k)];
    }
    for (int sy = 0; sy < 8; ++sy)
        counts[dst * LSG_ROW_WORDS + 34 + sy] = counts[dst * LSG_ROW_WORDS + 10 + sy] - counts[dst * LSG_ROW_WORDS + 26 + sy];
}

int unit_row_offsets(lsg_ctx* c, int ct, const uint32_t** off_out) {
    hipStream_t st = c->stream;
    const uint32_t n_ne = c->n_ne;
    if (c->d_ne_rowoff.reserve((size_t)(n_ne + 2) * 8)) return -1;
    uint32_t* cnt = c->d_ne_rowoff.as<uint32_t>();
    uint32_t* off = cnt + (n_ne + 2);
    hipLaunchKernelGGL(k_unit_rowcount, dim3((n_ne + 256) / 256), dim3(256), 0, st, c->d_ne_units.as<uint32_t>(), c->d_ne_mask.as<uint64_t>(), n_ne, c->n_ct, ct, cnt);
    SCAN_U32(cnt, off, n_ne + 1);
    *off_out = off;
    return 0;
}

int run_export_rows(lsg_ctx* c, int ct, DevBuf& dk, DevBuf& dr, DevBuf& dc) {
    int64_t n = c->n_rows[ct];
    if (n == 0) return 0;
    hipStream_t st = c->stream;
    CountArgs a{};
    fill_args(c, &c->last_params, a);
    uint32_t n_ne = c->n_ne;
    const uint32_t* off = nullptr;
    if (int rc = unit_row_offsets(c, ct, &off)) return rc;
    if (dk.reserve((size_t)n * 8) || dr.reserve((size_t)n) || dc.reserve((size_t)n * LSG_ROW_WORDS * 4)) return -1;
    uint64_t threads = (uint64_t)n_ne * 64;
    hipLaunchKernelGGL(k_export_rows, dim3((unsigned)((threads + 255) / 256)), dim3(256), 0, st, a, ct, off,
                       dk.as<int64_t>(), dr.as<uint8_t>(), dc.as<uint32_t>());
    LSG_HIP(hipGetLastError());
    return 0;
}

int run_fetch_counts(lsg_ctx* c, int ct, int64_t* keys, uint8_t* ref, uint32_t* counts, int64_t capacity) {
    if (!c->counted) { set_error("lsg_fetch_counts: call lsg_pileup_count first"); return -2; }
    if (ct < 0 || ct >= c->n_ct) { set_error("lsg_fetch_counts: bad cell type %d", ct); return -2; }
    int64_t n = c->n_rows[ct];
    if (capacity < n) { set_error("lsg_fetch_counts: capacity %lld < %lld rows", (long long)capacity, (long long)n); return -2; }
    if (n == 0) return 0;
    hipStream_t st = c->stream;
    DevBuf &dk = c->ws[WS_EXPORT_K], &dr = c->ws[WS_EXPORT_R], &dc = c->ws[WS_EXPORT_C];
    if (int rc = run_export_rows(c, ct, dk, dr, dc)) return rc;
    LSG_HIP(hipMemcpyAsync(keys, dk.p, (size_t)n * 8, hipMemcpyDeviceToHost, st));
    LSG_HIP(hipMemcpyAsync(ref, dr.p, (size_t)n, hipMemcpyDeviceToHost, st));
    LSG_HIP(hipMemcpyAsync(counts, dc.p, (size_t)n * LSG_ROW_WORDS * 4, hipMemcpyDeviceToHost, st));
    LSG_HIP(hipStreamSynchronize(st));
    return 0;
}

}
```

### longsom_amd/csrc/store.hip

```cpp
#include "lsg_ctx.h"
#include <hipcub/hipcub.hpp>
#include <chrono>
#include <cstdio>
#include <cstdlib>
#include <utility>

namespace lsg {

constexpr uint32_t KEY_INVALID = 0xFFFFFFFFu;

constexpr uint32_t RV_WHI = 1u << 29, RV_SEGFIRST = 1u << 30, RV_FWD = 1u << 31, RV_READ = RV_WHI - 1u;
__host__ __device__ __forceinline__ uint64_t sort_key(uint32_t cb, uint32_t first, uint32_t nev1, uint64_t src, int cb_bits, int wsh = 0) {
    return (uint64_t)cb | ((uint64_t)(first | (nev1 << (6 + wsh))) << cb_bits) | (src << (cb_bits + 12 + 2 * wsh));
}

struct BuildArgs {
    int64_t n_reads, n_segs, n_events;
    const int32_t* read_tid; const uint16_t* read_flag; const uint8_t* read_mapq; const int32_t* read_cb;
    const uint32_t* seg_read; const int32_t* seg_start; const int32_t* seg_len; const int64_t* seg_ev_off;
    const uint32_t* tile_base; const int64_t* contig_len;
    int32_t n_contigs; uint32_t n_tiles;
    uint2* seg_info;
    uint32_t* tile_cap;
    uint32_t* cursor;
    uint64_t* key; uint32_t* rdv;
    int32_t cb_bits;
    unsigned long long* qhead;
    int32_t lf_min_mq, lf_ignore_orphans; uint32_t lf_flag_exclude;
    uint32_t* bad;
    unsigned long long* n_ev;
    int32_t* span_diff;
    int32_t* cap_diff;
    int32_t window;
    int32_t wsh;
    int32_t src_shift;
};

__device__ __forceinline__ int64_t win_edge_after(int64_t x, int32_t W) { return 1 + (int64_t)W * (int64_t)((x >= 1 ? (uint32_t)(x - 1) / (uint32_t)W : 0u) + 1u); }
__device__ __forceinline__ int64_t win_edge_in_tile(int64_t tstart, int32_t W) {
    const int64_t b = win_edge_after(tstart, W);
    return b < tstart + TILE_W ? b : -1;
}

constexpr int SEG_THREADS = 256, SEG_U = 4, SEG_H = 2048, SEG_MAX_SINCE = 6;
__global__ __launch_bounds__(SEG_THREADS) void k_seg_static(BuildArgs a) {
    __shared__ uint32_t hkey[SEG_H];
    __shared__ int32_t hval[SEG_H];
    __shared__ unsigned long long s_ev;
    __shared__ uint32_t s_new, s_flush;
    for (int i = threadIdx.x; i < SEG_H; i += SEG_THREADS) { hkey[i] = KEY_INVALID; hval[i] = 0; }
    if (threadIdx.x == 0) { s_ev = 0; s_new = 0; s_flush = 0; }
    auto slot = [&](uint32_t t) -> int {
        uint32_t h = (t * 2654435761u) >> 21;
        for (int tries = 0; tries < 16; ++tries) {
            const uint32_t prev = atomicCAS(&hkey[h], KEY_INVALID, t);
            if (prev == KEY_INVALID) { atomicAdd(&s_new, 1u); return (int)h; }
            if (prev == t) return (int)h;
            h = (h + 1) & (SEG_H - 1);
        }
        return -1;
    };
    auto mark = [&](uint32_t t, int32_t v) { const int h = slot(t); if (h >= 0) atomicAdd(&hval[h], v); else atomicAdd(a.span_diff + t, v); };
    auto mark_cap = [&](uint32_t t, int32_t v) { const int h = slot(t); if (h >= 0) atomicAdd(&hval[h], v * 65536); else atomicAdd(a.cap_diff + t, v); };
    unsigned long long n_ev = 0;
    bool unphased = false;
    constexpr int64_t BATCH = (int64_t)SEG_THREADS * SEG_U;
    const int64_t n_batches = (a.n_segs + BATCH - 1) / BATCH;
    const int64_t per_wg = (n_batches + gridDim.x - 1) / gridDim.x;
    const int64_t b_lo = (int64_t)blockIdx.x * per_wg, b_hi = b_lo + per_wg < n_batches ? b_lo + per_wg : n_batches;
    const int64_t last_seg = a.n_segs - 1;
    int since = 0;
    __syncthreads();
    for (int64_t bt = b_lo; bt < b_hi; ++bt) {
        int64_t sg[SEG_U], st_[SEG_U], ln_[SEG_U], of_[SEG_U]; uint32_t rd_[SEG_U], rp_[SEG_U], rn_[SEG_U]; bool in_[SEG_U];
#pragma unroll
        for (int u = 0; u < SEG_U; ++u) {
            sg[u] = bt * BATCH + (int64_t)u * SEG_THREADS + threadIdx.x;
            in_[u] = sg[u] < a.n_segs;
            const int64_t si = in_[u] ? sg[u] : last_seg;
            rd_[u] = a.seg_read[si]; st_[u] = a.seg_start[si]; ln_[u] = a.seg_len[si]; of_[u] = a.seg_ev_off[si];
            rp_[u] = a.seg_read[si > 0 ? si - 1 : 0]; rn_[u] = a.seg_read[si < last_seg ? si + 1 : last_seg];
        }
        int32_t tid_[SEG_U], cb_[SEG_U]; uint32_t flag_[SEG_U], mq_[SEG_U];
#pragma unroll
        for (int u = 0; u < SEG_U; ++u) {
            const int64_t ri = (int64_t)rd_[u] < a.n_reads ? (int64_t)rd_[u] : 0;
            tid_[u] = a.read_tid[ri]; cb_[u] = a.read_cb[ri]; flag_[u] = a.read_flag[ri]; mq_[u] = (uint32_t)a.read_mapq[ri];
        }
        int64_t clen_[SEG_U]; uint32_t tb_[SEG_U], te_[SEG_U];
#pragma unroll
        for (int u = 0; u < SEG_U; ++u) {
            const int ti = tid_[u] >= 0 && tid_[u] < a.n_contigs ? tid_[u] : 0;
            clen_[u] = a.contig_len[ti]; tb_[u] = a.tile_base[ti]; te_[u] = a.tile_base[ti + 1];
        }
#pragma unroll
        for (int u = 0; u < SEG_U; ++u) {
        const int64_t s = sg[u];
        uint32_t edge_tile = KEY_INVALID;
        if (in_[u]) {
            const uint32_t r = rd_[u];
            uint32_t key = KEY_INVALID, tb = 0;
            if ((int64_t)r >= a.n_reads) atomicOr(a.bad, 2u);
            else {
                const int64_t st = st_[u], ln = ln_[u], o = of_[u];
                const int32_t tid = tid_[u], cb = cb_[u];
                const bool on_contig = tid >= 0 && tid < a.n_contigs;
                if (ln > 0 && (o < 0 || o + ln > a.n_events)) atomicOr(a.bad, 1u);
                else {
                    const uint32_t flag = flag_[u];
                    bool pool = (int)mq_[u] >= a.lf_min_mq && (flag & a.lf_flag_exclude) == 0;
                    if (pool && a.lf_ignore_orphans && (flag & 1u) && !(flag & 2u)) pool = false;
                    if (pool && on_contig && cb >= 0 && (uint32_t)cb < CB_MASK && !(st < 0 || ln <= 0 || st + ln > clen_[u])) {
                        key = (uint32_t)cb | (((flag >> 4) & 1u) << 24);
                        tb = tb_[u];
                        n_ev += (unsigned long long)ln;
                        unphased |= ((o - st) & (int64_t)((64 << a.wsh) - 1)) != 0;
                        mark_cap((tb + ((uint32_t)st >> 6)) >> a.wsh, 1);
                        mark_cap(((tb + ((uint32_t)(st + ln - 1) >> 6)) >> a.wsh) + 1, -1);
                        int nb = 0;
                        for (int64_t b = win_edge_after(st, a.window); b < st + ln; b += a.window) {
                            if ((b & (int64_t)((64 << a.wsh) - 1)) == 0) continue;
                            const uint32_t t = (tb + (uint32_t)(b >> 6)) >> a.wsh;
                            if (nb++ == 0) edge_tile = t;
                            else { atomicAdd(a.cap_diff + t, 1); atomicAdd(a.cap_diff + t + 1, -1); }
                        }
                    }
                }
                if (a.span_diff && on_contig && cb >= 0) {
                    const bool first = s == 0 || rp_[u] != r, last = s + 1 == a.n_segs || rn_[u] != r;
                    const uint32_t t0 = tb_[u], te = te_[u];
                    if ((first || last) && te > t0) {
                        int64_t b = st < 0 ? 0 : st, e = st + (ln > 0 ? ln : 0);
                        if (e < 0) e = 0;
                        if (first) { uint32_t t = t0 + (uint32_t)(b >> 6); if (t >= te) t = te - 1; mark(t >> a.wsh, 1); }
                        if (last) { uint32_t t = t0 + (uint32_t)(e >> 6); if (t >= te) t = te - 1; mark((t >> a.wsh) + 1, -1); }
                    }
                }
            }
            a.seg_info[s] = make_uint2(key, tb);
        }
        for (unsigned long long todo = __ballot(edge_tile != KEY_INVALID); todo;) {
            const uint32_t lt = (uint32_t)__shfl((int)edge_tile, __ffsll((long long)todo) - 1);
            const unsigned long long same = __ballot(edge_tile == lt);
            if ((threadIdx.x & 63) == (unsigned)(__ffsll((long long)todo) - 1)) { const int n = __popcll(same); atomicAdd(a.cap_diff + lt, n); atomicAdd(a.cap_diff + lt + 1, -n); }
            todo &= ~same;
        }
        }
        ++since;
        __syncthreads();
        if (threadIdx.x == 0) {
            s_flush = (bt + 1 == b_hi || s_new > SEG_H / 2 || since >= SEG_MAX_SINCE) ? 1u : 0u;
            if (s_flush) s_new = 0;
        }
        __syncthreads();
        if (s_flush) {
            since = 0;
            for (int i = threadIdx.x; i < SEG_H; i += SEG_THREADS)
                if (hkey[i] != KEY_INVALID) {
                    const int32_t w = hval[i], v = (int32_t)(int16_t)(w & 0xffff), cp = (w - v) >> 16;
                    if (v != 0) atomicAdd(a.span_diff + hkey[i], v);
                    if (cp != 0) atomicAdd(a.cap_diff + hkey[i], cp);
                    hkey[i] = KEY_INVALID; hval[i] = 0;
                }
            __syncthreads();
        }
    }
    for (int o = 32; o > 0; o >>= 1) n_ev += __shfl_down(n_ev, o);
    __syncthreads();
    if ((threadIdx.x & 63) == 0 && n_ev) atomicAdd(&s_ev, n_ev);
    __syncthreads();
    if (threadIdx.x == 0 && s_ev) atomicAdd(a.n_ev, s_ev);
    if (__syncthreads_or(unphased ? 1 : 0) && threadIdx.x == 0) atomicOr(a.bad, 4u);
}

constexpr int BIN_THREADS = 256;
constexpr int BIN_TPR = 8;
constexpr int BIN_H = 4096;
constexpr int BIN_SUPER = 16;
constexpr int BIN_MAXI = 32;
constexpr uint32_t BIN_FILL = BIN_H * 5 / 8;

template <class OP>
__device__ __forceinline__ uint32_t wave_reduce_last(uint32_t v, OP op) {
    v = op(v, (uint32_t)__builtin_amdgcn_update_dpp(0, (int)v, 0x111, 0xf, 0xf, true));
    v = op(v, (uint32_t)__builtin_amdgcn_update_dpp(0, (int)v, 0x112, 0xf, 0xf, true));
    v = op(v, (uint32_t)__builtin_amdgcn_update_dpp(0, (int)v, 0x114, 0xf, 0xf, true));
    v = op(v, (uint32_t)__builtin_amdgcn_update_dpp(0, (int)v, 0x118, 0xf, 0xf, true));
    v = op(v, (uint32_t)__builtin_amdgcn_update_dpp(0, (int)v, 0x142, 0xa, 0xf, false));
    v = op(v, (uint32_t)__builtin_amdgcn_update_dpp(0, (int)v, 0x143, 0xc, 0xf, false));
    return v;
}
struct BinSeg { uint32_t key, tb, t0, rd; int32_t st, ln, ntile; int64_t evoff, b1; };

struct BinRaw { uint2 info; int32_t st, ln; int64_t evoff; uint32_t rd; };
__device__ __forceinline__ BinRaw bin_fetch(const BuildArgs& a, int64_t s) {
    const int64_t si = s < a.n_segs ? s : a.n_segs - 1;
    BinRaw w;
    w.info = a.seg_info[si]; w.st = a.seg_start[si]; w.ln = a.seg_len[si]; w.evoff = a.seg_ev_off[si]; w.rd = a.seg_read[si];
    return w;
}
template <bool FULL>
__device__ __forceinline__ BinSeg bin_make(const BuildArgs& a, int64_t s, const BinRaw& w) {
    BinSeg g; g.key = KEY_INVALID; g.tb = 0; g.t0 = 0; g.rd = 0; g.b1 = 0; g.st = 0; g.ln = 0; g.ntile = 0; g.evoff = 0;
    if (FULL) asm volatile("" :: "v"(w.info.x), "v"(w.info.y), "v"(w.st), "v"(w.ln), "v"(w.evoff), "v"(w.rd));
    else asm volatile("" :: "v"(w.info.x), "v"(w.info.y), "v"(w.st), "v"(w.ln));
    const uint2 info = w.info;
    const int bs = 6 + a.wsh;
    if (s < a.n_segs && info.x != KEY_INVALID) {
        g.key = info.x; g.tb = info.y >> a.wsh;
        g.st = w.st; g.ln = w.ln; g.evoff = w.evoff; g.rd = w.rd;
        g.t0 = g.tb + ((uint32_t)g.st >> bs);
        g.ntile = (int)(((uint32_t)(g.st + g.ln - 1) >> bs) - ((uint32_t)g.st >> bs)) + 1;
        g.b1 = win_edge_after(g.st, a.window);
        for (int64_t b = g.b1; b < (int64_t)g.st + g.ln; b += a.window) g.ntile += (b & (int64_t)((1 << bs) - 1)) != 0;
    } else if (s < a.n_segs) g.tb = info.y >> a.wsh;
    return g;
}
__device__ __forceinline__ void bin_piece(const BinSeg& g, int32_t W, int bs, int k, uint32_t& tile_rel, int32_t& lo, int32_t& hi) {
    const int32_t en = g.st + g.ln;
    const int64_t bmask = (int64_t)((1 << bs) - 1);
    int shift = 0;
    int64_t b = g.b1;
    for (; b < en; b += W) {
        if ((b & bmask) == 0) continue;
        const int idx = (int)((b >> bs) - (g.st >> bs)) + shift + 1;
        if (k < idx) break;
        if (k == idx) {
            tile_rel = (uint32_t)((b >> bs) - (g.st >> bs)); lo = (int32_t)b;
            const int32_t tend = (int32_t)(((b >> bs) + 1) << bs);
            hi = en < tend ? en : tend;
            return;
        }
        ++shift;
    }
    tile_rel = (uint32_t)(k - shift);
    const int32_t tstart = (int32_t)((((uint32_t)g.st >> bs) + tile_rel) << bs);
    lo = g.st > tstart ? g.st : tstart;
    hi = en < tstart + (1 << bs) ? en : tstart + (1 << bs);
    if (b < hi && b > lo && (b & bmask) != 0) hi = (int32_t)b;
}

__global__ __launch_bounds__(BIN_THREADS) void k_bin(BuildArgs a) {
    __shared__ uint32_t hkey[BIN_H], hcnt[BIN_H];
    __shared__ uint32_t s_newb[BIN_MAXI], s_ib[BIN_MAXI], s_ir[BIN_MAXI];
    __shared__ int s_maxb[BIN_MAXI];
    __shared__ uint32_t s_super;
    const int t = threadIdx.x, lane = t & 63;
    constexpr int HSHIFT = 32 - __builtin_ctz(BIN_H);
    for (int i = t; i < BIN_H; i += BIN_THREADS) { hkey[i] = KEY_INVALID; hcnt[i] = 0; }
    const int64_t n_batches = (a.n_segs + BIN_THREADS - 1) / BIN_THREADS;
    const int64_t n_super = (n_batches + BIN_SUPER - 1) / BIN_SUPER;
    for (bool first = true;; first = false) {
        __syncthreads();
        if (t == 0) s_super = first ? blockIdx.x : (uint32_t)atomicAdd(a.qhead, 1ull) + gridDim.x;
        __syncthreads();
        const int64_t sup = (uint32_t)__builtin_amdgcn_readfirstlane((int)s_super);
        if (sup >= n_super) break;
        const int64_t b0 = sup * BIN_SUPER;
        const int64_t b1 = b0 + BIN_SUPER < n_batches ? b0 + BIN_SUPER : n_batches;
        int64_t cb = b0; int cr = 0;
        BinRaw nx = bin_fetch(a, cb * BIN_THREADS + t);
        while (cb < b1) {
            if (t < BIN_MAXI) { s_newb[t] = 0; s_maxb[t] = 0; }
            __syncthreads();
            int ni = 0; uint32_t tot = 0;
            int64_t b = cb; int r = cr;
            bool stop = false;
            while (!stop && b < b1) {
                const BinSeg g = bin_make<false>(a, b * BIN_THREADS + t, nx);
                nx = bin_fetch(a, (b + 1 < b1 ? b + 1 : b) * BIN_THREADS + t);
                const int ni_first = ni;
                const int wmax = (int)wave_reduce_last((uint32_t)g.ntile, [](uint32_t x, uint32_t y) { return x > y ? x : y; });
                if (lane == 63 && wmax) atomicMax(&s_maxb[ni_first], wmax);
                int R = -1;
                for (;;) {
                    uint32_t newc = 0;
                    uint32_t x[BIN_TPR], h[BIN_TPR], prev[BIN_TPR];
#pragma unroll
                    for (int j = 0; j < BIN_TPR; ++j) {
                        const int k = r * BIN_TPR + j;
                        x[j] = KEY_INVALID; h[j] = 0; prev[j] = 0;
                        if (k < g.ntile) {
                            uint32_t trel; int32_t lo_, hi_;
                            bin_piece(g, a.window, 6 + a.wsh, k, trel, lo_, hi_);
                            x[j] = g.t0 + trel;
                            h[j] = (x[j] * 2654435761u) >> HSHIFT;
                        }
                    }
#pragma unroll
                    for (int j = 0; j < BIN_TPR; ++j)
                        if (x[j] != KEY_INVALID) prev[j] = atomicCAS(&hkey[h[j]], KEY_INVALID, x[j]);
#pragma unroll
                    for (int j = 0; j < BIN_TPR; ++j)
                        if (x[j] != KEY_INVALID) {
                            uint32_t hh = h[j], p = prev[j];
                            if (p == KEY_INVALID) ++newc;
                            else
                                while (p != x[j]) {
                                    hh = (hh + 1) & (BIN_H - 1);
                                    p = atomicCAS(&hkey[hh], KEY_INVALID, x[j]);
                                    if (p == KEY_INVALID) { ++newc; break; }
                                }
                            atomicAdd(&hcnt[hh], 1u);
                        }
                    newc = wave_reduce_last(newc, [](uint32_t x, uint32_t y) { return x + y; });
                    if (lane == 63 && newc) atomicAdd(&s_newb[ni], newc);
                    if (t == 0) { s_ib[ni] = (uint32_t)(b - b0); s_ir[ni] = (uint32_t)r; }
                    __syncthreads();
                    if (R < 0) R = __builtin_amdgcn_readfirstlane((s_maxb[ni_first] + BIN_TPR - 1) / BIN_TPR);
                    tot += (uint32_t)__builtin_amdgcn_readfirstlane((int)s_newb[ni]);
                    ++ni; ++r;
                    if (r >= R) { ++b; r = 0; }
                    if (ni >= BIN_MAXI || tot + BIN_THREADS * BIN_TPR > BIN_FILL) { stop = true; break; }
                    if (r == 0) break;
                }
            }
            nx = bin_fetch(a, cb * BIN_THREADS + t);
            for (int i = t; i < BIN_H; i += BIN_THREADS) {
                const uint32_t cnt = hcnt[i];
                if (cnt) hcnt[i] = atomicAdd(&a.cursor[hkey[i]], cnt);
            }
            __syncthreads();
            {
                const uint32_t ibl = (uint32_t)__builtin_amdgcn_readfirstlane((int)s_ib[ni - 1]);
                const int64_t b_next = b < b1 ? b : b1 - 1;
                uint32_t ib = (uint32_t)(cb - b0);
                BinSeg g = bin_make<true>(a, cb * BIN_THREADS + t, nx);
                nx = bin_fetch(a, (ib < ibl ? b0 + ib + 1 : b_next) * BIN_THREADS + t);
                for (int it = 0; it < ni; ++it) {
                    const int rr = __builtin_amdgcn_readfirstlane((int)s_ir[it]);
                    const uint32_t nb = it + 1 < ni ? (uint32_t)__builtin_amdgcn_readfirstlane((int)s_ib[it + 1]) : ib;
                    uint32_t x_[BIN_TPR], h_[BIN_TPR], hk_[BIN_TPR], pos_[BIN_TPR]; int32_t lo_[BIN_TPR], hi_[BIN_TPR];
#pragma unroll
                    for (int j = 0; j < BIN_TPR; ++j) {
                        const int k = rr * BIN_TPR + j;
                        x_[j] = KEY_INVALID; h_[j] = 0; hk_[j] = KEY_INVALID; pos_[j] = 0; lo_[j] = 0; hi_[j] = 0;
                        if (k < g.ntile) {
                            uint32_t trel;
                            bin_piece(g, a.window, 6 + a.wsh, k, trel, lo_[j], hi_[j]);
                            x_[j] = g.t0 + trel;
                            h_[j] = (x_[j] * 2654435761u) >> HSHIFT;
                            hk_[j] = hkey[h_[j]];
                        }
                    }
#pragma unroll
                    for (int j = 0; j < BIN_TPR; ++j)
                        if (x_[j] != KEY_INVALID) {
                            while (hk_[j] != x_[j]) { h_[j] = (h_[j] + 1) & (BIN_H - 1); hk_[j] = hkey[h_[j]]; }
                            pos_[j] = atomicAdd(&hcnt[h_[j]], 1u);
                        }
                    BinSeg gn = g;
                    if (nb != ib) {
                        gn = bin_make<true>(a, (b0 + nb) * BIN_THREADS + t, nx);
                        nx = bin_fetch(a, (nb < ibl ? b0 + nb + 1 : b_next) * BIN_THREADS + t);
                    }
#pragma unroll
                    for (int j = 0; j < BIN_TPR; ++j) {
                        if (x_[j] != KEY_INVALID) {
                            const uint32_t x = x_[j]; const int32_t lo = lo_[j], hi = hi_[j];
                            const uint32_t pos = pos_[j];
                            const int32_t tstart = (int32_t)((x - g.tb) << (6 + a.wsh));
                            int64_t edge = -1;
                            { int64_t e = g.b1 - a.window; while (e + a.window <= lo) e += a.window; if (e > tstart && e <= lo && e > 1) edge = e; }
                            const uint64_t src = (uint64_t)(g.evoff + (lo - g.st)) >> a.src_shift;
                            const uint64_t key = sort_key(g.key & CB_MASK, (uint32_t)(lo - tstart), (uint32_t)(hi - lo - 1), src, a.cb_bits, a.wsh);
                            const uint32_t flags = (lo == g.st ? RV_SEGFIRST : 0u) | (((g.key >> 24) & 1u) ? 0u : RV_FWD);
                            if (a.rdv) { a.key[pos] = key; a.rdv[pos] = g.rd | flags | (edge >= 0 && lo >= edge ? RV_WHI : 0u); }
                            else a.key[pos] = key | ((uint64_t)flags << 32);
                        }
                    }
                    g = gn; ib = nb;
                }
                __syncthreads();
                for (int i = t; i < BIN_H; i += BIN_THREADS)
                    if (hkey[i] != KEY_INVALID) { hkey[i] = KEY_INVALID; hcnt[i] = 0; }
            }
            cb = b; cr = r;
        }
    }
}

constexpr int TT_THREADS = 256, TT_SUB = TT_THREADS * 4, TT_MAX_CHUNKS = 1024;
struct TtAgg1 { int32_t d, s, smax, pad; };
struct TtAgg2 { unsigned long long c; uint32_t b, ne; };
struct TtArgs {
    const int32_t* cap_diff; const int32_t* span_diff; uint32_t T; uint32_t chunk;
    uint32_t n_chunks;
    TtAgg1* agg1; int32_t* din; TtAgg2* agg2; TtAgg2* in2;
    uint32_t* cap; uint32_t* tile_off; uint32_t* blk_off; uint32_t* netile;
    uint32_t* d_small; unsigned long long* d_sum;
};
template <int NT, class V>
__device__ __forceinline__ V tt_wg_exscan(V v, V& total, V* sh ) {
    const int lane = threadIdx.x & 63, wv = threadIdx.x >> 6;
    V inc = v;
    for (int o = 1; o < 64; o <<= 1) { const V u = __shfl_up(inc, o); if (lane >= o) inc += u; }
    __syncthreads();
    if (lane == 63) sh[wv] = inc;
    __syncthreads();
    V base = 0, tot = 0;
    for (int w = 0; w < NT / 64; ++w) { const V x = sh[w]; if (w < wv) base += x; tot += x; }
    total = tot;
    return base + inc - v;
}
__global__ __launch_bounds__(TT_THREADS) void k_tt_marks(TtArgs a) {
    __shared__ int32_t sh[TT_THREADS / 64 + 1];
    __shared__ int32_t sh_max[TT_THREADS / 64];
    const uint32_t lo = blockIdx.x * a.chunk, hi = lo + a.chunk < a.T + 1 ? lo + a.chunk : a.T + 1;
    int32_t dsum = 0, srun = 0, smax = INT32_MIN;
    for (uint32_t b0 = lo; b0 < hi; b0 += TT_SUB) {
        const uint32_t i0 = b0 + threadIdx.x * 4;
        int32_t d[4], sp[4];
#pragma unroll
        for (int k = 0; k < 4; ++k) { const bool in = i0 + k < hi; d[k] = in ? a.cap_diff[i0 + k] : 0; sp[k] = in && a.span_diff ? a.span_diff[i0 + k] : 0; }
        int32_t ds = d[0] + d[1] + d[2] + d[3];
        int32_t r = 0, m = INT32_MIN;
#pragma unroll
        for (int k = 0; k < 4; ++k) { r += sp[k]; if (i0 + k < hi) m = r > m ? r : m; }
        int32_t tot_s; const int32_t ex = tt_wg_exscan<TT_THREADS>(r, tot_s, sh);
        if (m != INT32_MIN) { const int32_t v = srun + ex + m; smax = v > smax ? v : smax; }
        srun += tot_s; dsum += ds;
    }
    for (int o = 32; o > 0; o >>= 1) { const int32_t u = __shfl_down(smax, o); smax = u > smax ? u : smax; dsum += __shfl_down(dsum, o); }
    __syncthreads();
    if ((threadIdx.x & 63) == 0) { sh_max[threadIdx.x >> 6] = smax; sh[threadIdx.x >> 6] = dsum; }
    __syncthreads();
    if (threadIdx.x == 0) {
        int32_t m = INT32_MIN, dd = 0;
        for (int w = 0; w < TT_THREADS / 64; ++w) { m = sh_max[w] > m ? sh_max[w] : m; dd += sh[w]; }
        a.agg1[blockIdx.x] = TtAgg1{dd, srun, m, 0};
    }
}
__global__ __launch_bounds__(TT_MAX_CHUNKS) void k_tt_scan1(TtArgs a) {
    __shared__ int32_t sh[TT_MAX_CHUNKS / 64 + 1];
    __shared__ int32_t sh_max[TT_MAX_CHUNKS / 64];
    const uint32_t i = threadIdx.x;
    TtAgg1 g{0, 0, INT32_MIN, 0};
    if (i < a.n_chunks) g = a.agg1[i];
    int32_t tot;
    const int32_t din = tt_wg_exscan<TT_MAX_CHUNKS>(g.d, tot, sh);
    const int32_t sin = tt_wg_exscan<TT_MAX_CHUNKS>(g.s, tot, sh);
    if (i < a.n_chunks) a.din[i] = din;
    int32_t m = i < a.n_chunks && g.smax != INT32_MIN ? sin + g.smax : INT32_MIN;
    for (int o = 32; o > 0; o >>= 1) { const int32_t u = __shfl_down(m, o); m = u > m ? u : m; }
    __syncthreads();
    if ((i & 63) == 0) sh_max[i >> 6] = m;
    __syncthreads();
    if (i == 0) { int32_t mm = INT32_MIN; for (int w = 0; w < TT_MAX_CHUNKS / 64; ++w) mm = sh_max[w] > mm ? sh_max[w] : mm; a.d_small[3] = (uint32_t)mm; }
}
__global__ __launch_bounds__(TT_THREADS) void k_tt_caps(TtArgs a) {
    __shared__ int32_t sh[TT_THREADS / 64 + 1];
    __shared__ unsigned long long sh_c[TT_THREADS / 64];
    __shared__ uint32_t sh_b[TT_THREADS / 64], sh_n[TT_THREADS / 64];
    const uint32_t lo = blockIdx.x * a.chunk, hi = lo + a.chunk < a.T + 1 ? lo + a.chunk : a.T + 1;
    int32_t run = a.din[blockIdx.x];
    unsigned long long csum = 0; uint32_t bsum = 0, nsum = 0;
    for (uint32_t b0 = lo; b0 < hi; b0 += TT_SUB) {
        const uint32_t i0 = b0 + threadIdx.x * 4;
        int32_t d[4];
#pragma unroll
        for (int k = 0; k < 4; ++k) d[k] = i0 + k < hi ? a.cap_diff[i0 + k] : 0;
        int32_t tot; const int32_t ex = tt_wg_exscan<TT_THREADS>(d[0] + d[1] + d[2] + d[3], tot, sh);
        int32_t r = run + ex;
#pragma unroll
        for (int k = 0; k < 4; ++k) {
            r += d[k];
            if (i0 + k < hi) {
                a.cap[i0 + k] = (uint32_t)r;
                if (i0 + k < a.T) { const uint32_t cv = (uint32_t)r; csum += cv; bsum += (cv + 7u) / 8u; nsum += cv != 0u; }
            }
        }
        run += tot;
    }
    for (int o = 32; o > 0; o >>= 1) { csum += __shfl_down(csum, o); bsum += __shfl_down(bsum, o); nsum += __shfl_down(nsum, o); }
    __syncthreads();
    if ((threadIdx.x & 63) == 0) { sh_c[threadIdx.x >> 6] = csum; sh_b[threadIdx.x >> 6] = bsum; sh_n[threadIdx.x >> 6] = nsum; }
    __syncthreads();
    if (threadIdx.x == 0) {
        TtAgg2 g{0, 0, 0};
        for (int w = 0; w < TT_THREADS / 64; ++w) { g.c += sh_c[w]; g.b += sh_b[w]; g.ne += sh_n[w]; }
        a.agg2[blockIdx.x] = g;
    }
}
__global__ __launch_bounds__(TT_MAX_CHUNKS) void k_tt_scan2(TtArgs a) {
    __shared__ unsigned long long sh64[TT_MAX_CHUNKS / 64 + 1];
    __shared__ uint32_t sh32[TT_MAX_CHUNKS / 64 + 1];
    const uint32_t i = threadIdx.x;
    TtAgg2 g{0, 0, 0};
    if (i < a.n_chunks) g = a.agg2[i];
    unsigned long long tc; uint32_t tb, tn;
    TtAgg2 in;
    in.c = tt_wg_exscan<TT_MAX_CHUNKS>(g.c, tc, sh64);
    in.b = tt_wg_exscan<TT_MAX_CHUNKS>(g.b, tb, sh32);
    in.ne = tt_wg_exscan<TT_MAX_CHUNKS>(g.ne, tn, sh32);
    if (i < a.n_chunks) a.in2[i] = in;
    if (i == 0) { *a.d_sum = tc; a.d_small[1] = tn; }
}
__global__ __launch_bounds__(TT_THREADS) void k_tt_offsets(TtArgs a) {
    __shared__ uint32_t sh[TT_THREADS / 64 + 1];
    const uint32_t lo = blockIdx.x * a.chunk, hi = lo + a.chunk < a.T + 1 ? lo + a.chunk : a.T + 1;
    const TtAgg2 in = a.in2[blockIdx.x];
    uint32_t crun = (uint32_t)in.c, brun = in.b, nrun = in.ne;
    for (uint32_t b0 = lo; b0 < hi; b0 += TT_SUB) {
        const uint32_t i0 = b0 + threadIdx.x * 4;
        uint32_t cv[4], bv[4], nv[4];
#pragma unroll
        for (int k = 0; k < 4; ++k) { cv[k] = i0 + k < hi && i0 + k < a.T ? a.cap[i0 + k] : 0u; bv[k] = (cv[k] + 7u) / 8u; nv[k] = cv[k] != 0u; }
        uint32_t tc, tb, tn;
        uint32_t ec = crun + tt_wg_exscan<TT_THREADS>(cv[0] + cv[1] + cv[2] + cv[3], tc, sh);
        uint32_t eb = brun + tt_wg_exscan<TT_THREADS>(bv[0] + bv[1] + bv[2] + bv[3], tb, sh);
        uint32_t en = nrun + tt_wg_exscan<TT_THREADS>(nv[0] + nv[1] + nv[2] + nv[3], tn, sh);
#pragma unroll
        for (int k = 0; k < 4; ++k) {
            if (i0 + k < hi) {
                a.tile_off[i0 + k] = ec; a.blk_off[i0 + k] = eb;
                if (nv[k]) a.netile[en] = i0 + k;
            }
            ec += cv[k]; eb += bv[k]; en += nv[k];
        }
        crun += tc; brun += tb; nrun += tn;
    }
}
constexpr uint32_t SORT_LARGE = 256;
__global__ void k_seg_bounds(const uint32_t* netile, uint32_t n, const uint32_t* tile_off, uint32_t* begin, uint32_t* end, uint32_t* begin2, uint32_t* end2) {
    const uint32_t i = blockIdx.x * blockDim.x + threadIdx.x;
    if (i >= n) return;
    const uint32_t t = netile[i], b = tile_off[t], e = tile_off[t + 1];
    const bool large = e - b > SORT_LARGE;
    begin[i] = b; end[i] = large ? e : b;
    begin2[i] = b; end2[i] = large ? b : e;
}
__global__ void k_tile_caps(const uint32_t* tiles, uint32_t n, const uint32_t* cap, uint32_t* out) {
    const uint32_t i = blockIdx.x * blockDim.x + threadIdx.x;
    if (i < n) out[i] = cap[tiles[i]] >> 11;
}
__global__ void k_tm_blk_mark(const uint32_t* cap, const uint32_t* blk_off, uint32_t n_tiles, uint32_t* blk_tile) {
    const uint32_t t = blockIdx.x * blockDim.x + threadIdx.x;
    if (t < n_tiles && cap[t]) blk_tile[blk_off[t]] = t;
}

constexpr int TMG_BLOCKS = 4, TMG_WAVES = 4;
typedef uint32_t u32x4 __attribute__((ext_vector_type(4)));
struct __attribute__((packed, aligned(2))) U4A2 { u32x4 v; };
__global__ __launch_bounds__(TMG_WAVES * 64) void k_tm_gather(const uint16_t* events, int64_t n_events, const uint64_t* key, const uint32_t* rdv, int cb_bits, int src_shift,
                                                               const uint32_t* tile_off, const uint32_t* blk_off, const uint32_t* blk_tile, uint32_t nblk,
                                                               uint32_t* s0, uint8_t* b8, uint32_t* rd, uint4* store, uint16_t* ext) {
    __shared__ __attribute__((aligned(16))) uint16_t lds[TMG_WAVES][TMG_BLOCKS][8][64];
    const int lane = threadIdx.x & 63, wv = threadIdx.x >> 6;
    const uint32_t per_xcd = gridDim.x >> 3;
    const uint32_t vwg = (blockIdx.x & 7u) * per_xcd + (blockIdx.x >> 3);
    const uint32_t blk0 = (vwg * TMG_WAVES + (uint32_t)wv) * TMG_BLOCKS;
    if (blk0 >= nblk) return;
    uint32_t e_src = 0, e_info = 0;
    if (lane < 8 * TMG_BLOCKS) {
        const uint32_t blk = blk0 + ((uint32_t)lane >> 3);
        if (blk < nblk) {
            const uint64_t p = (uint64_t)blk * 8 + (lane & 7);
            const uint32_t t = blk_tile[blk];
            const uint32_t i = (uint32_t)(p - (uint64_t)blk_off[t] * 8), off = tile_off[t], n = tile_off[t + 1] - off;
            auto put = [](auto* q, auto v) { __builtin_nontemporal_store(v, q); };
            if (i >= n) { put(s0 + p, (uint32_t)TM_PAD_S0); put(b8 + p, (uint8_t)0); put(rd + p, 0u); }
            else {
                const uint32_t j = off + i, cbm = (1u << cb_bits) - 1u;
                const uint64_t k64 = key[j];
                const uint32_t k = (uint32_t)k64 & cbm, v = rdv[j];
                const bool rs = i == 0 || ((uint32_t)key[j - 1] & cbm) != k;
                const bool single = rs && (i + 1 == n || ((uint32_t)key[j + 1] & cbm) != k);
                const uint32_t geom = (uint32_t)(k64 >> cb_bits), first = geom & 63u, nev1 = (geom >> 6) & 63u;
                const uint64_t src = ((k64 >> (cb_bits + 12)) << src_shift) | (src_shift ? first : 0u);
                put(s0 + p, k | ((v & RV_FWD) ? TM_FWD : 0u) | ((v & RV_WHI) ? TM_WHI : 0u) | (rs ? TM_RUNSTART : 0u));
                put(b8 + p, (uint8_t)(nev1 | ((v & RV_SEGFIRST) ? 64u : 0u) | (single ? 128u : 0u)));
                put(rd + p, v & RV_READ);
                e_src = (uint32_t)src; e_info = (uint32_t)(src >> 32) | (first << 8) | ((nev1 + 1u) << 16);
            }
        }
    }
    const int u = lane >> 3, c = lane & 7;
    u32x4 chunk[TMG_BLOCKS];
    uint32_t info[TMG_BLOCKS];
#pragma unroll
    for (int q = 0; q < TMG_BLOCKS; ++q) {
        chunk[q] = u32x4{0u, 0u, 0u, 0u};
        const uint32_t lo32 = (uint32_t)__shfl((int)e_src, q * 8 + u), inf = (uint32_t)__shfl((int)e_info, q * 8 + u);
        info[q] = inf;
        const uint32_t nev = inf >> 16;
        if ((uint32_t)c * 8u < nev) {
            const int64_t off = (int64_t)(((uint64_t)(inf & 0xffu) << 32) | lo32) + c * 8;
            if (off + 8 <= n_events) chunk[q] = reinterpret_cast<const U4A2*>(events + off)->v;
            else {
                uint32_t w[4] = {0u, 0u, 0u, 0u};
                for (int i = 0; i < 8; ++i) if (off + i < n_events) w[i >> 1] |= (uint32_t)events[off + i] << (16 * (i & 1));
                chunk[q] = u32x4{w[0], w[1], w[2], w[3]};
            }
        }
    }
#pragma unroll
    for (int q = 0; q < TMG_BLOCKS; ++q) *reinterpret_cast<u32x4*>(&lds[wv][q][u][c * 8]) = chunk[q];
    __builtin_amdgcn_fence(__ATOMIC_ACQ_REL, "workgroup");
    __builtin_amdgcn_wave_barrier();
#pragma unroll
    for (int q = 0; q < TMG_BLOCKS; ++q) {
        const uint32_t blk = blk0 + q;
        if (blk >= nblk) break;
        uint32_t e[8], any = 0;
#pragma unroll
        for (int uu = 0; uu < 8; ++uu) {
            const uint32_t inf = (uint32_t)__builtin_amdgcn_readlane((int)info[q], uu * 8);
            const uint32_t idx = (uint32_t)lane - ((inf >> 8) & 63u);
            e[uu] = idx < (inf >> 16) ? (uint32_t)lds[wv][q][uu][idx & 63u] : 0u;
            any |= e[uu];
        }
        const unsigned long long m = __ballot(any != 0u);
        const int first = m ? __ffsll((long long)m) - 1 : 0, last = m ? 64 - __clzll((long long)m) : 0;
        if (lane >= first && lane < last) {
            const u32x4 row = {e[0] | (e[1] << 16), e[2] | (e[3] << 16), e[4] | (e[5] << 16), e[6] | (e[7] << 16)};
            u32x4* dst = reinterpret_cast<u32x4*>(store) + (uint64_t)blk * 64 + lane;
            __builtin_nontemporal_store(row, dst);
        }
        if (lane == 0) ext[blk] = (uint16_t)(first | (last << 8));
    }
}

#define SCAN_U32(in, out, n)                                                                              \
    do {                                                                                                  \
        size_t tb_ = 0;                                                                                   \
        LSG_HIP(hipcub::DeviceScan::ExclusiveSum(nullptr, tb_, (in), (out), (int)(n), st));              \
        if (c->d_cub_tmp.reserve(tb_ + 256)) return -1;                                                   \
        tb_ = c->d_cub_tmp.cap;                                                                           \
        LSG_HIP(hipcub::DeviceScan::ExclusiveSum(c->d_cub_tmp.p, tb_, (in), (out), (int)(n), st));       \
    } while (0)

enum { BT_KEY_A = 0, BT_KEY_B, BT_VAL_A, BT_VAL_B, BT_PEX, BT_NETILE, BT_SEG_BEGIN, BT_SEG_END, BT_TMP, BT_PER_TILE, BT_OFFS, BT_SPAN, BT_CURSOR, BT_LPT, BT_COPY_TMP, BT_N };

void drop_store(lsg_ctx* c) {
    c->tm_valid = false; c->plan_n_ct = 0; c->plan1_n_ct = 0; c->tm_n = 0; c->tm_events = 0; c->tm_np = 0; c->tm_nblk = 0; c->tm_njobs = 0; c->tm_nchunks = 0;
    c->tm_n_ne = 0; c->tm_n_multi = 0; c->tm_n_slabs = 0; c->tm_n_wide = 0;
    c->max_live_reads = -1; c->max_live_all = -1; c->max_live_exact = -1; c->has_drops = false;
    c->counted = c->called = false; c->counted_at_load = false; c->load_was_fused = false; c->store_skipped = false;
}

static void settle_temporaries(lsg_ctx* c) {
    size_t held = 0, mem_free = 0, mem_total = 0;
    for (auto& b : c->bt) held += b.cap;
    held += c->ws[WS_SEG_INFO].cap;
    if (hipMemGetInfo(&mem_free, &mem_total) != hipSuccess) return;
    const bool tight = c->store_skipped ? mem_free < mem_total / 4 : (held > mem_total / 8 || mem_free < mem_total / 8);
    if (tight) { for (auto& b : c->bt) b.release(); c->ws[WS_SEG_INFO].release(); c->plan1_n_ct = 0; }
}

static int plan_tiles(lsg_ctx* c, hipStream_t st);
static int plan_jobs(lsg_ctx* c, bool finish, const uint64_t* skey = nullptr, int cb_bits = 0);
static void plan_finish(lsg_ctx* c);
static void plan_finish_tiles(lsg_ctx* c);

template <unsigned RB, unsigned BS = 256, unsigned IPT = 8>
using LsgSortConfig = rocprim::segmented_radix_sort_config<RB, rocprim::kernel_config<BS, IPT>, rocprim::WarpSortConfig<16, 4, 256, 64, 32, 8, 256>>;
template <unsigned RB, unsigned BS, unsigned IPT, class... Args>
static hipError_t lsg_segmented_sort(Args&&... args) { return rocprim::segmented_radix_sort_pairs<LsgSortConfig<RB, BS, IPT>>(std::forward<Args>(args)...); }
template <unsigned RB, unsigned BS, unsigned IPT, class... Args>
static hipError_t lsg_segmented_sort_keys(Args&&... args) { return rocprim::segmented_radix_sort_keys<LsgSortConfig<RB, BS, IPT>>(std::forward<Args>(args)...); }

static bool count_in_load(const lsg_ctx* c) { return c->cal_enabled && c->n_ct >= 1 && c->n_ct <= 2 && c->n_cb > 0 && c->copy_stream; }

static int print_tile_hist(const lsg_ctx* c, uint32_t T) {
    std::vector<uint32_t> caps(T);
    LSG_HIP(hipMemcpy(caps.data(), c->d_tile_cap.p, (size_t)T * 4, hipMemcpyDeviceToHost));
    unsigned long long nt[8] = {0}, ne[8] = {0}; uint32_t mx = 0;
    const uint32_t lim[7] = {64, 256, 2048, 8192, 32768, 131072, 524288};
    for (uint32_t i = 0; i < T; ++i) { const uint32_t v = caps[i]; if (!v) continue; int k = 0; while (k < 7 && v > lim[k]) ++k; ++nt[k]; ne[k] += v; if (v > mx) mx = v; }
    for (int k = 0; k < 8; ++k) fprintf(stderr, "tiles <= %u: %llu tiles, %llu entries\n", k < 7 ? lim[k] : 0xffffffffu, nt[k], ne[k]);
    fprintf(stderr, "largest tile: %u entries\n", mx);
    return 0;
}

enum LoadRung { RUNG_WINDOWS = 1, RUNG_TILE_KEYS, RUNG_TILE_VALUES };

static int build_once(lsg_ctx* c, const uint16_t* events, int64_t n_events, const int64_t* seg_ev_off, const lsg_reads* src, int rung) {
    drop_store(c);
    hipStream_t st = c->stream;
    const int64_t S = c->rd.n_segs, R = c->rd.n_reads;
    const bool counts = count_in_load(c) && n_events >= 64 && n_events < (1ll << 39);
    const bool skip_store = c->cal_enabled && c->store_policy == LSG_STORE_SKIP_WHEN_COUNTED;
    const bool win = rung == RUNG_WINDOWS && skip_store && counts && n_events >= 128 &&
                     (c->events_layout == LSG_LAYOUT_PHASED || (c->hint_phased_events && c->hint_phased_events == (const void*)events)) && ((uintptr_t)events & 255u) == 0 && c->plp_window >= 128 &&
                     c->cal_params.min_bq >= 1 && c->cal_params.min_bq <= 255 && (c->n_tiles & 1u) == 0;
    const int wsh = win ? 1 : 0;
    c->wsh = wsh;
    const uint32_t T = c->n_tiles >> wsh;
    const auto t_wall = std::chrono::steady_clock::now();
    auto finish = [&]() {
        c->layout_build_ms = std::chrono::duration<double, std::milli>(std::chrono::steady_clock::now() - t_wall).count();
        c->tm_valid = true;
        return 0;
    };
    for (auto& v : c->build_ms) v = 0;
    c->st_min_mq = c->lf_min_mq; c->st_flag_exclude = c->lf_flag_exclude; c->st_ignore_orphans = c->lf_ignore_orphans;
    if (c->d_tile_cap.reserve(((size_t)T + 2) * 4) || c->d_tile_off.reserve(((size_t)T + 2) * 4) || c->d_scalars.reserve(512 * 8)) return -1;
    LSG_HIP(hipMemsetAsync(c->d_tile_cap.p, 0, ((size_t)T + 2) * 4, st));
    LSG_HIP(hipMemsetAsync(c->d_tile_off.p, 0, ((size_t)T + 2) * 4, st));
    if (S <= 0 || T == 0) { LSG_HIP(hipStreamSynchronize(st)); return finish(); }
    if (c->ws[WS_SEG_INFO].reserve(((size_t)S + 1) * 8)) return -1;
    LSG_HIP(hipMemsetAsync(c->d_scalars.p, 0, 64, st));
    BuildArgs a{};
    a.n_reads = R; a.n_segs = S; a.n_events = n_events;
    const lsg_reads& in = src ? *src : c->rd;
    a.read_tid = in.read_tid; a.read_flag = in.read_flag; a.read_mapq = in.read_mapq; a.read_cb = in.read_cb;
    a.seg_read = in.seg_read; a.seg_start = in.seg_start; a.seg_len = in.seg_len; a.seg_ev_off = seg_ev_off;
    a.tile_base = c->d_tile_base.as<uint32_t>(); a.contig_len = c->d_contig_len.as<int64_t>(); a.n_contigs = c->n_contigs; a.n_tiles = T;
    a.seg_info = c->ws[WS_SEG_INFO].as<uint2>(); a.tile_cap = c->d_tile_cap.as<uint32_t>();
    a.lf_min_mq = c->lf_min_mq; a.lf_flag_exclude = c->lf_flag_exclude; a.lf_ignore_orphans = c->lf_ignore_orphans;
    a.window = c->plp_window; c->st_window = c->plp_window; a.wsh = wsh;
    a.qhead = c->d_scalars.as<unsigned long long>(); a.bad = reinterpret_cast<uint32_t*>(c->d_scalars.as<unsigned long long>() + 2);
    a.n_ev = c->d_scalars.as<unsigned long long>() + 3;
    if (c->bt[BT_SPAN].reserve(((size_t)T + 2) * 4)) return -1;
    LSG_HIP(hipMemsetAsync(c->bt[BT_SPAN].p, 0, ((size_t)T + 2) * 4, st));
    a.span_diff = c->bt[BT_SPAN].as<int32_t>();
    uint32_t* d_small = reinterpret_cast<uint32_t*>(c->d_scalars.as<unsigned long long>() + 4);
    DevBuf& tmp = c->bt[BT_TMP];
    LSG_HIP(hipEventRecord(c->evb[0], st));
    unsigned g_seg = (unsigned)((S + 256 * SEG_U - 1) / (256 * SEG_U)); if (g_seg > (unsigned)(c->n_cus * 16)) g_seg = (unsigned)(c->n_cus * 16);
    unsigned g_bin = (unsigned)((S + 256 * BIN_SUPER - 1) / (256 * BIN_SUPER)); if (g_bin > (unsigned)(c->n_cus * 8)) g_bin = (unsigned)(c->n_cus * 8);
    if (c->bt[BT_PER_TILE].reserve(((size_t)T + 2) * 4)) return -1;
    LSG_HIP(hipMemsetAsync(c->bt[BT_PER_TILE].p, 0, ((size_t)T + 2) * 4, st));
    a.cap_diff = c->bt[BT_PER_TILE].as<int32_t>();
    hipLaunchKernelGGL(k_seg_static, dim3(g_seg), dim3(256), 0, st, a);
    if (c->bt[BT_NETILE].reserve(((size_t)T + 2) * 4) || c->tm[TM_BLK_OFF].reserve(((size_t)T + 2) * 4)) return -1;
    uint32_t* blk_off = c->tm[TM_BLK_OFF].as<uint32_t>();
    unsigned long long* d_sum = c->d_scalars.as<unsigned long long>() + 8;
    {
        size_t tb = 0;
        LSG_HIP(hipcub::DeviceReduce::Max(nullptr, tb, in.read_cb, reinterpret_cast<int32_t*>(d_small + 2), (int)(R > 0 ? R : 1), st));
        if (tmp.reserve(tb + 256 + 64 * 1024)) return -1;
        tb = tmp.cap;
        if (R > 0) LSG_HIP(hipcub::DeviceReduce::Max(tmp.p, tb, in.read_cb, reinterpret_cast<int32_t*>(d_small + 2), (int)R, st));
    }
    {
        if (c->d_cub_tmp.reserve(64 * 1024)) return -1;
        TtArgs ta{};
        ta.cap_diff = a.cap_diff; ta.span_diff = a.span_diff; ta.T = T;
        const uint64_t per = ((uint64_t)T + 1 + TT_MAX_CHUNKS - 1) / TT_MAX_CHUNKS;
        ta.chunk = (uint32_t)((per + TT_SUB - 1) / TT_SUB * TT_SUB);
        ta.n_chunks = (uint32_t)(((uint64_t)T + 1 + ta.chunk - 1) / ta.chunk);
        char* scratch = reinterpret_cast<char*>(c->d_cub_tmp.p);
        ta.agg1 = reinterpret_cast<TtAgg1*>(scratch); ta.agg2 = reinterpret_cast<TtAgg2*>(scratch + 16 * 1024); ta.in2 = reinterpret_cast<TtAgg2*>(scratch + 32 * 1024);
        ta.din = reinterpret_cast<int32_t*>(scratch + 48 * 1024);
        ta.cap = c->d_tile_cap.as<uint32_t>(); ta.tile_off = c->d_tile_off.as<uint32_t>(); ta.blk_off = blk_off; ta.netile = c->bt[BT_NETILE].as<uint32_t>();
        ta.d_small = d_small; ta.d_sum = d_sum;
        hipLaunchKernelGGL(k_tt_marks, dim3(ta.n_chunks), dim3(TT_THREADS), 0, st, ta);
        hipLaunchKernelGGL(k_tt_scan1, dim3(1), dim3(TT_MAX_CHUNKS), 0, st, ta);
        hipLaunchKernelGGL(k_tt_caps, dim3(ta.n_chunks), dim3(TT_THREADS), 0, st, ta);
        hipLaunchKernelGGL(k_tt_scan2, dim3(1), dim3(TT_MAX_CHUNKS), 0, st, ta);
        hipLaunchKernelGGL(k_tt_offsets, dim3(ta.n_chunks), dim3(TT_THREADS), 0, st, ta);
    }
    uint32_t total = 0, bad = 0, n_netile = 0, nblk = 0; int32_t max_cb = 0, max_live = 0;
    unsigned long long n_ev = 0, sum = 0;
    LSG_HIP(hipMemcpyAsync(c->h_pin, c->d_scalars.p, 9 * 8, hipMemcpyDeviceToHost, st));
    LSG_HIP(hipMemcpyAsync(c->h_pin + 16, blk_off + T, 4, hipMemcpyDeviceToHost, st));
    LSG_HIP(hipStreamSynchronize(st));
    {
        const unsigned long long* hp = c->h_pin;
        const uint32_t* hs = reinterpret_cast<const uint32_t*>(hp + 4);
        bad = (uint32_t)hp[2]; n_ev = hp[3]; n_netile = hs[1]; max_cb = R > 0 ? (int32_t)hs[2] : 0; max_live = (int32_t)hs[3]; sum = hp[8];
        nblk = (uint32_t)hp[16];
    }
    if (win && (bad & 4u) && !(bad & 3u)) return RUNG_TILE_KEYS;
    const int src_shift = !(bad & 4u) && ((uintptr_t)events & (wsh ? 255u : 127u)) == 0 ? 6 + wsh : 0;
    c->src_phased = src_shift != 0;
    if (bad & 2u) { set_error("lsg_load_reads: a segment's read index lies outside the read arrays"); return -2; }
    if (bad & 1u) { set_error("lsg_load_reads: a segment's event range lies outside the events array"); return -2; }
    if (sum >= 0x7FFFFFF0ull) { set_error("lsg_load_reads: %llu tile entries exceed the 31-bit entry index; load the reads in windows", sum); return -2; }
    total = (uint32_t)sum;
    const uint64_t N = total;
    c->tm_n = N; c->tm_events = (int64_t)n_ev;
    c->max_live_all = max_live > 0 ? max_live : 0;
    if (N == 0) return finish();
    if (getenv("LSG_TILE_HIST")) { if (int rc = print_tile_hist(c, T)) return rc; }
    int bits = 1; while (bits < 24 && (1ll << bits) <= (long long)max_cb) ++bits;
    DevBuf &key_a = c->bt[BT_KEY_A], &key_b = c->bt[BT_KEY_B], &val_a = c->bt[BT_VAL_A], &val_b = c->bt[BT_VAL_B];
    if ((n_events >> src_shift) >= (1ll << (52 - bits - 2 * wsh))) {
        set_error("lsg_load_reads: %lld events with %d-bit barcode ids do not fit the packed sort key (events < 2^%d): load the reads in windows", (long long)n_events, bits, 52 - bits + src_shift);
        return -2;
    }
    bool keys_only = rung <= RUNG_TILE_KEYS && skip_store && counts && (n_events >> src_shift) < (1ll << (50 - bits - 2 * wsh));
    bool cap_out = true;
    if (c->cal_enabled && c->cal_params.max_depth > 0 && c->max_live_all + 1 > (int64_t)c->cal_params.max_depth) {
        cap_out = false;
        if (count_in_load(c)) {
            LSG_HIP(hipStreamSynchronize(c->copy_stream));
            if (live_read_bound(c)) return -1;
            cap_out = c->max_live_reads + 1 <= (int64_t)c->cal_params.max_depth;
            if (!cap_out) {
                if (live_read_bound_exact(c)) return -1;
                cap_out = c->max_live_exact <= (int64_t)c->cal_params.max_depth;
            }
        }
    }
    if (keys_only) {
        const lsg_count_params& q = c->cal_params;
        if (q.min_mq != c->st_min_mq || q.flag_exclude != c->st_flag_exclude || (q.ignore_orphans != 0) != (c->st_ignore_orphans != 0)) keys_only = false;
        if (!cap_out) keys_only = false;
        for (int t = 0; t < c->n_contigs && keys_only; ++t) if (!c->ref_ptr[t]) keys_only = false;
    }
    if (win && !keys_only) return RUNG_TILE_KEYS;
    if (keys_only && getenv("LSG_TIMING")) fprintf(stderr, "[lsg] load: keys alone through the scatter and the sort (8 bytes an entry)%s\n", win ? ", entries binned by 128-position windows" : "");
    if (key_a.reserve(N * 8 + 16) || key_b.reserve(N * 8 + 16) || (!keys_only && (val_a.reserve(N * 4 + 16) || val_b.reserve(N * 4 + 16))) ||
        c->bt[BT_CURSOR].reserve(((size_t)T + 2) * 4)) return -1;
    a.cursor = c->bt[BT_CURSOR].as<uint32_t>(); a.key = key_a.as<uint64_t>(); a.rdv = keys_only ? nullptr : val_a.as<uint32_t>(); a.cb_bits = bits; a.src_shift = src_shift;
    LSG_HIP(hipMemcpyAsync(a.cursor, c->d_tile_off.p, ((size_t)T + 1) * 4, hipMemcpyDeviceToDevice, st));
    LSG_HIP(hipMemsetAsync(c->d_scalars.p, 0, 8, st));
    hipLaunchKernelGGL(k_bin, dim3(g_bin), dim3(BIN_THREADS), 0, st, a);
    LSG_HIP(hipEventRecord(c->evb[1], st));
    if (c->tm[TM_BLK_TILE].reserve(((size_t)nblk + 2) * 4)) return -1;
    bool blk_tiles_made = false;
    const bool lpt = n_netile > 1;
    const uint32_t* lpt_tiles = nullptr;
    auto blk_tiles = [&](hipStream_t s_) -> int {
        uint32_t* bt_ = c->tm[TM_BLK_TILE].as<uint32_t>();
        LSG_HIP(hipMemsetAsync(bt_, 0, (size_t)nblk * 4, s_));
        hipLaunchKernelGGL(k_tm_blk_mark, dim3((T + 255) / 256), dim3(256), 0, s_, c->d_tile_cap.as<uint32_t>(), blk_off, T, bt_);
        size_t tb = c->bt[BT_COPY_TMP].cap;
        LSG_HIP(hipcub::DeviceScan::InclusiveScan(c->bt[BT_COPY_TMP].p, tb, bt_, bt_, hipcub::Max(), (int)nblk, s_));
        LSG_HIP(hipEventRecord(c->ev_blk, s_));
        blk_tiles_made = true;
        return 0;
    };
    {
        hipStream_t bs = c->copy_stream;
        DevBuf& lk = c->bt[BT_LPT];
        const size_t lpt_pitch = ((size_t)n_netile + 64) & ~(size_t)63;
        if (lpt && lk.reserve(lpt_pitch * 4 * 3)) return -1;
        uint32_t* k_in = lk.as<uint32_t>(); uint32_t* k_out = k_in + lpt_pitch; uint32_t* t_out = k_out + lpt_pitch;
        uint32_t* bt_ = c->tm[TM_BLK_TILE].as<uint32_t>();
        size_t tb_lpt = 0, tb_blk = 0;
        if (lpt) LSG_HIP(hipcub::DeviceRadixSort::SortPairsDescending(nullptr, tb_lpt, k_in, k_out, c->bt[BT_NETILE].as<uint32_t>(), t_out, (int)n_netile, 0, 21, bs));
        LSG_HIP(hipcub::DeviceScan::InclusiveScan(nullptr, tb_blk, bt_, bt_, hipcub::Max(), (int)nblk, bs));
        size_t tb_sort2 = 0;
        if (n_netile) {
            if (keys_only) LSG_HIP((lsg_segmented_sort_keys<7, 256, 8>(nullptr, tb_sort2, (uint64_t*)nullptr, (uint64_t*)nullptr, (unsigned)N, (unsigned)n_netile, (uint32_t*)nullptr, (uint32_t*)nullptr, 0u, (unsigned)bits, bs, false)));
            else LSG_HIP((lsg_segmented_sort<7, 256, 8>(nullptr, tb_sort2, (uint64_t*)nullptr, (uint64_t*)nullptr, (uint32_t*)nullptr, (uint32_t*)nullptr, (unsigned)N, (unsigned)n_netile,
                                                        (uint32_t*)nullptr, (uint32_t*)nullptr, 0u, (unsigned)bits, bs, false)));
        }
        size_t tb_max = tb_lpt > tb_blk ? tb_lpt : tb_blk;
        if (tb_sort2 > tb_max) tb_max = tb_sort2;
        if (c->bt[BT_COPY_TMP].reserve(tb_max + 256)) return -1;
        void* scratch = c->bt[BT_COPY_TMP].p;
        if (lpt) {
            hipLaunchKernelGGL(k_tile_caps, dim3((n_netile + 255) / 256), dim3(256), 0, bs, c->bt[BT_NETILE].as<uint32_t>(), n_netile, c->d_tile_cap.as<uint32_t>(), k_in);
            size_t tb = c->bt[BT_COPY_TMP].cap;
            LSG_HIP(hipcub::DeviceRadixSort::SortPairsDescending(scratch, tb, k_in, k_out, c->bt[BT_NETILE].as<uint32_t>(), t_out, (int)n_netile, 0, 21, bs));
            LSG_HIP(hipEventRecord(c->ev_lpt, bs));
            lpt_tiles = t_out;
        }
        if (!skip_store) { if (int rc = blk_tiles(bs)) return rc; }
    }
    const bool tiles_planned = count_in_load(c);
    if (tiles_planned) {
        if (int rc = plan_tiles(c, c->copy_stream)) return rc;
        plan_finish_tiles(c);
    }
    if (n_netile) {
        const size_t seg_pitch = ((size_t)n_netile + 64) & ~(size_t)63;
        if (c->bt[BT_SEG_BEGIN].reserve(seg_pitch * 8) || c->bt[BT_SEG_END].reserve(seg_pitch * 8)) return -1;
        uint32_t* sb1 = c->bt[BT_SEG_BEGIN].as<uint32_t>(); uint32_t* se1 = c->bt[BT_SEG_END].as<uint32_t>();
        uint32_t* sb2 = sb1 + seg_pitch; uint32_t* se2 = se1 + seg_pitch;
        if (lpt) LSG_HIP(hipStreamWaitEvent(st, c->ev_lpt, 0));
        hipLaunchKernelGGL(k_seg_bounds, dim3((n_netile + 255) / 256), dim3(256), 0, st, lpt ? lpt_tiles : c->bt[BT_NETILE].as<uint32_t>(), n_netile, c->d_tile_off.as<uint32_t>(), sb1, se1, sb2, se2);
        LSG_HIP(hipEventRecord(c->ev_copy, st));
        size_t tb = 0;
        const bool big_blocks = N < (64ull << 20);
        auto sort = [&](void* tmp_p, size_t& tmp_n) {
            if (keys_only && big_blocks) return lsg_segmented_sort_keys<7, 512, 8>(tmp_p, tmp_n, key_a.as<uint64_t>(), key_b.as<uint64_t>(), (unsigned)N, (unsigned)n_netile, sb1, se1, 0u, (unsigned)bits, st, false);
            if (keys_only) return lsg_segmented_sort_keys<7, 256, 8>(tmp_p, tmp_n, key_a.as<uint64_t>(), key_b.as<uint64_t>(), (unsigned)N, (unsigned)n_netile, sb1, se1, 0u, (unsigned)bits, st, false);
            return lsg_segmented_sort<7, 256, 8>(tmp_p, tmp_n, key_a.as<uint64_t>(), key_b.as<uint64_t>(), val_a.as<uint32_t>(), val_b.as<uint32_t>(), (unsigned)N, (unsigned)n_netile,
                                                 sb1, se1, 0u, (unsigned)bits, st, false);
        };
        LSG_HIP(sort(nullptr, tb));
        if (tmp.reserve(tb + 256)) return -1;
        tb = tmp.cap;
        LSG_HIP(sort(tmp.p, tb));
        hipStream_t bs = c->copy_stream;
        LSG_HIP(hipStreamWaitEvent(bs, c->ev_copy, 0));
        size_t tb2 = c->bt[BT_COPY_TMP].cap;
        if (keys_only) LSG_HIP((lsg_segmented_sort_keys<7, 256, 8>(c->bt[BT_COPY_TMP].p, tb2, key_a.as<uint64_t>(), key_b.as<uint64_t>(), (unsigned)N, (unsigned)n_netile, sb2, se2, 0u, (unsigned)bits, bs, false)));
        else LSG_HIP((lsg_segmented_sort<7, 256, 8>(c->bt[BT_COPY_TMP].p, tb2, key_a.as<uint64_t>(), key_b.as<uint64_t>(), val_a.as<uint32_t>(), val_b.as<uint32_t>(), (unsigned)N, (unsigned)n_netile,
                                                    sb2, se2, 0u, (unsigned)bits, bs, false)));
        LSG_HIP(hipEventRecord(c->ev_lpt, bs));
        LSG_HIP(hipStreamWaitEvent(st, c->ev_lpt, 0));
    }
    LSG_HIP(hipEventRecord(c->evb[2], st));
    const uint64_t np = (uint64_t)nblk * 8;
    c->tm_np = np; c->tm_nblk = nblk;
    auto reserve_store = [&]() -> int {
    if (c->tm[TM_S0].reserve((np + 16) * 4) || c->tm[TM_B].reserve(np + 16) ||
        c->tm[TM_RD].reserve((np + 16) * 4) || c->tm[TM_META].reserve((np + 8 * (TM_GROUP + 1)) * 4) ||
        c->tm[TM_BLK_TILE].reserve(((size_t)nblk + 2) * 4) || c->tm[TM_EXT].reserve(((size_t)nblk + TM_GROUP + 2) * 2)) return -1;
    LSG_HIP(hipMemsetD32Async(reinterpret_cast<hipDeviceptr_t>(c->tm[TM_S0].as<uint32_t>() + np), (int)TM_PAD_S0, 16, st));
    LSG_HIP(hipMemsetAsync(c->tm[TM_B].as<uint8_t>() + np, 0, 16, st));
    if (c->tm[TM_STORE].cap < ((size_t)nblk + TM_GROUP) * 1024) {
        size_t mem_free = 0, mem_total = 0;
        if (hipMemGetInfo(&mem_free, &mem_total) == hipSuccess && ((size_t)nblk + TM_GROUP) * 1088 + (mem_total >> 5) > mem_free) {
            LSG_HIP(hipStreamSynchronize(st));
            key_a.release(); val_a.release(); c->ws[WS_SEG_INFO].release(); c->bt[BT_SPAN].release(); c->bt[BT_PEX].release(); c->bt[BT_OFFS].release();
        }
        if (c->tm[TM_STORE].reserve(((size_t)nblk + TM_GROUP) * 1024)) return -1;
    }
    return 0;
    };
    LSG_HIP(hipEventRecord(c->evb[3], st));
    bool fused = counts;
    if (fused) {
        const lsg_count_params& q = c->cal_params;
        if (q.min_mq < c->st_min_mq || (c->st_flag_exclude & ~q.flag_exclude) != 0 || (c->st_ignore_orphans && !q.ignore_orphans)) fused = false;
        if (fused && !cap_out) fused = false;
        for (int t = 0; t < c->n_contigs && fused; ++t) if (!c->ref_ptr[t]) fused = false;
    }
    const bool dbg = getenv("LSG_DEBUG_SYNC") != nullptr;
    auto stage = [&](const char* what) { if (dbg) { const hipError_t e = hipStreamSynchronize(st); fprintf(stderr, "[lsg] fused load: %s: %s\n", what, hipGetErrorString(e)); fflush(stderr); } };
    auto fused_plan = [&]() -> int {
        stage("scatter + sort + block tables");
        c->tm_np = np; c->tm_nblk = nblk;
        if (int rc = plan_jobs(c, false, key_b.as<uint64_t>(), bits)) return rc;
        stage("plan");
        return 0;
    };
    const GatherCountSrc gsrc{events, n_events, key_b.as<uint64_t>(), keys_only ? nullptr : val_b.as<uint32_t>(), bits, src_shift, wsh};
    bool planned = false;
    if (win && !fused) return RUNG_TILE_KEYS;
    if (keys_only && getenv("LSG_TEST_KEYS_ONLY_REFUSED")) return win ? RUNG_TILE_KEYS : RUNG_TILE_VALUES;
    if (fused && skip_store) {
        if (int rc = fused_plan()) return rc;
        planned = true;
        const int rc = run_gather_count(c, &c->cal_params, gsrc, true);
        LSG_HIP(hipStreamSynchronize(st));
        if (hipGetLastError() != hipSuccess) { set_error("lsg_load_reads: the count pass failed"); return -1; }
        if (rc < 0 && rc != -3) return rc;
        if (rc == 0) {
            plan_finish(c);
            LSG_HIP(hipStreamSynchronize(c->copy_stream));
            c->load_was_fused = true; c->counted_at_load = true; c->store_skipped = true;
            for (int i = 0; i < 4; ++i) { float ms = 0; if (hipEventElapsedTime(&ms, c->evb[i], c->evb[i + 1]) == hipSuccess) c->build_ms[i] = ms; }
            settle_temporaries(c);
            c->layout_build_ms = std::chrono::duration<double, std::milli>(std::chrono::steady_clock::now() - t_wall).count();
            return 0;
        }
        c->counted = false;
        fused = false;
    }
    if (win) return RUNG_TILE_KEYS;
    if (keys_only) return RUNG_TILE_VALUES;
    if (int rc = reserve_store()) return rc;
    if (!blk_tiles_made) {
        LSG_HIP(hipStreamSynchronize(c->copy_stream));
        if (int rc = blk_tiles(st)) return rc;
    }
    if (fused) {
        if (int rc = fused_plan()) return rc;
        c->tm_valid = true;
        int rc = run_gather_count(c, &c->cal_params, gsrc, false);
        LSG_HIP(hipStreamSynchronize(st));
        if (hipGetLastError() != hipSuccess) { c->tm_valid = false; set_error("lsg_load_reads: the fused gather + count pass failed"); return -1; }
        if (rc < 0 && rc != -3) { c->tm_valid = false; return rc; }
        plan_finish(c);
        c->load_was_fused = true;
        c->counted_at_load = rc == 0;
        if (rc) c->counted = false;
    } else {
    LSG_HIP(hipStreamWaitEvent(st, c->ev_blk, 0));
    const bool plan_early = c->n_ct > 0 && c->copy_stream && c->ev_copy && !planned;
    if (plan_early) LSG_HIP(hipEventRecord(c->ev_copy, st));
    {
        const dim3 grid((unsigned)(((((uint64_t)nblk + TMG_BLOCKS - 1) / TMG_BLOCKS + TMG_WAVES - 1) / TMG_WAVES + 7) / 8 * 8));
        hipLaunchKernelGGL(k_tm_gather, grid, dim3(TMG_WAVES * 64), 0, st,
                           events, n_events, key_b.as<uint64_t>(), val_b.as<uint32_t>(), bits, src_shift, c->d_tile_off.as<uint32_t>(), blk_off, c->tm[TM_BLK_TILE].as<uint32_t>(), nblk,
                           c->tm[TM_S0].as<uint32_t>(), c->tm[TM_B].as<uint8_t>(), c->tm[TM_RD].as<uint32_t>(),
                           c->tm[TM_STORE].as<uint4>(), c->tm[TM_EXT].as<uint16_t>());
    }
    LSG_HIP(hipEventRecord(c->evb[4], st));
    LSG_HIP(hipGetLastError());
    int plan_rc = 0;
    if (plan_early) {
        LSG_HIP(hipStreamWaitEvent(c->copy_stream, c->ev_copy, 0));
        plan_rc = tiles_planned ? 0 : plan_tiles(c, c->copy_stream);
        if (!plan_rc) {
            c->tm_np = np; c->tm_nblk = nblk;
            plan_rc = plan_jobs(c, false);
        }
    }
    LSG_HIP(hipStreamSynchronize(st));
    if (plan_early) LSG_HIP(hipStreamSynchronize(c->copy_stream));
    if (plan_rc) return plan_rc;
    if (plan_early || planned) plan_finish(c);
    }
    for (int i = 0; i < 4; ++i) { float ms = 0; if (hipEventElapsedTime(&ms, c->evb[i], c->evb[i + 1]) == hipSuccess) c->build_ms[i] = ms; }
    settle_temporaries(c);
    if (getenv("LSG_TIMING"))
        fprintf(stderr, "[lsg] tile store: %llu entries, %u blocks (%.2f GB): capacities + scatter %.2f, sort %.2f, fill %.2f, gather %.2f ms\n",
                (unsigned long long)N, nblk, (double)nblk * 1024 / 1e9, c->build_ms[0], c->build_ms[1], c->build_ms[2], c->build_ms[3]);
    return finish();
}

int build_store(lsg_ctx* c, const uint16_t* events, int64_t n_events, const int64_t* seg_ev_off, const lsg_reads* src) {
    int rc = build_once(c, events, n_events, seg_ev_off, src, RUNG_WINDOWS);
    while (rc > 0) {
        LSG_HIP(hipStreamSynchronize(c->stream)); LSG_HIP(hipStreamSynchronize(c->copy_stream));
        if (getenv("LSG_TIMING"))
            fprintf(stderr, rc == RUNG_TILE_KEYS ? "[lsg] load: not a load for 128-position windows after all, starting again by tiles\n"
                                                 : "[lsg] load: the count from keys alone was not made, loading again with values\n");
        rc = build_once(c, events, n_events, seg_ev_off, src, rc);
    }
    return rc;
}

constexpr uint32_t TM_CHUNK_WORK = 4096, TM_JOB_W0 = 32;

__global__ void k_tm_tiles(const uint32_t* cap, uint32_t n_tiles, int n_ct, uint32_t job_tgt, uint32_t H, uint32_t* ne, uint32_t* nj, uint32_t* slabs, uint32_t* multi) {
    const uint32_t t = blockIdx.x * blockDim.x + threadIdx.x;
    if (t > n_tiles) return;
    const uint32_t n = t < n_tiles ? cap[t] : 0u;
    const uint32_t j = n == 0 ? 0u : (n <= job_tgt ? 1u : (n + job_tgt - 1) / job_tgt);
    ne[t] = n ? H : 0u; nj[t] = j; slabs[t] = j > 1 ? j * (uint32_t)n_ct * H : 0u; multi[t] = j > 1 ? H : 0u;
}
struct RunSrc { const uint32_t* s0; const uint64_t* key; uint32_t cbm; };
__device__ __forceinline__ void tm_make_job(const RunSrc& rs, uint64_t base, uint32_t off, uint32_t n, uint32_t J, uint32_t j, uint32_t w0, uint32_t slab, uint32_t tile, int2 geom,
                                            TmJob* out, uint32_t* n_wide) {
    auto starts = [&](uint32_t x) -> bool {
        if (!rs.key) return (rs.s0[base + x] & TM_RUNSTART) != 0;
        return x == 0 || (((uint32_t)rs.key[off + x] ^ (uint32_t)rs.key[off + x - 1]) & rs.cbm) != 0;
    };
    auto cut = [&](uint32_t x) -> uint32_t { while (x < n && !starts(x)) ++x; return x < n ? x : n; };
    const uint32_t e0 = j == 0 ? 0u : cut((uint32_t)(((uint64_t)n * j) / J));
    uint32_t e1 = j + 1 == J ? n : cut((uint32_t)(((uint64_t)n * (j + 1)) / J));
    if (e1 < e0) e1 = e0;
    TmJob jb;
    jb.e0 = (uint32_t)(base + e0); jb.e1 = (uint32_t)(base + e1); jb.w0 = w0;
    jb.slab = J > 1 ? slab : 0xFFFFFFFFu; jb.nj = J; jb.cnt = n; jb.tile = tile;
    jb.base = (uint32_t)base; jb.off = off; jb.tstart = geom.x; jb.tid = geom.y & 0xffffff;
    uint32_t mid = e1;
    if (e1 - e0 >= 64u) { mid = cut(e0 + (e1 - e0) / 2u); if (mid > e1) mid = e1; }
    jb.emid = (uint32_t)(base + mid);
    if (e1 - e0 > (uint32_t)TM_JOB_LIMIT) { jb.nj |= TMJ_WIDE; atomicAdd(n_wide, 1u); }
    *out = jb;
}
__global__ void k_tm_jobs(const uint32_t* tile_base, int n_contigs, int n_ct, int wsh, RunSrc rs, const uint32_t* tile_off, const uint32_t* cap, const uint32_t* blk_off, const uint32_t* ne_off,
                          const uint32_t* nj, const uint32_t* job_off, const uint32_t* slab_off, const uint32_t* multi_off, uint32_t n_tiles, TmJob* jobs,
                          uint32_t* ne_units, int2* ne_geom, uint32_t* ne_nslot, uint32_t* ne_acc, uint32_t* multi, uint32_t* n_wide) {
    const uint32_t t = blockIdx.x * blockDim.x + threadIdx.x;
    if (t >= n_tiles) return;
    const uint32_t n = cap[t];
    if (!n) return;
    const uint32_t J = nj[t], ord = ne_off[t];
    const uint64_t base = (uint64_t)blk_off[t] * 8;
    const uint32_t tile0 = t << wsh;
    int tid = 0;
    { int lo = 0, hi = n_contigs; while (hi - lo > 1) { const int mid = (lo + hi) >> 1; if (tile_base[mid] <= tile0) lo = mid; else hi = mid; } tid = lo; }
    const int32_t tstart = (int32_t)((tile0 - tile_base[tid]) << 6);
    for (uint32_t h = 0; h < (1u << wsh); ++h)
    for (int ct = 0; ct < n_ct; ++ct) {
        const uint32_t w = (ord + h) * (uint32_t)n_ct + ct;
        ne_units[w] = (tile0 + h) * (uint32_t)n_ct + ct;
        ne_geom[w] = make_int2(tstart + 64 * (int32_t)h, tid | (ct << 24));
        ne_nslot[w] = J;
        ne_acc[w] = J > 1 ? slab_off[t] + (h * (uint32_t)n_ct + (uint32_t)ct) * J : 0u;
        if (J > 1) multi[(multi_off[t] + h) * (uint32_t)n_ct + ct] = w;
    }
    if (J > 1) return;
    tm_make_job(rs, base, tile_off[t], n, 1u, 0u, ord * (uint32_t)n_ct, 0xFFFFFFFFu, t, make_int2(tstart, tid), jobs + job_off[t], n_wide);
}
__global__ __launch_bounds__(64) void k_tm_jobs_multi(int n_ct, int wsh, RunSrc rs, const uint32_t* tile_off, const uint32_t* cap, const uint32_t* blk_off, const uint32_t* ne_off, const uint32_t* nj,
                                                      const uint32_t* job_off, const uint32_t* slab_off, const uint32_t* multi, const uint32_t* ne_units, const int2* ne_geom, uint32_t n_mt,
                                                      TmJob* jobs, uint32_t* n_wide) {
    const uint32_t i = blockIdx.x;
    if (i >= n_mt) return;
    const uint32_t w = multi[((size_t)i << wsh) * (uint32_t)n_ct], t = (ne_units[w] / (uint32_t)n_ct) >> wsh;
    const uint32_t n = cap[t], J = nj[t];
    const int2 geom = ne_geom[w];
    const uint64_t base = (uint64_t)blk_off[t] * 8;
    for (uint32_t j = threadIdx.x; j < J; j += 64u)
        tm_make_job(rs, base, tile_off[t], n, J, j, ne_off[t] * (uint32_t)n_ct, slab_off[t] + j, t, geom, jobs + job_off[t] + j, n_wide);
}
struct TmJobWork {
    const TmJob* jobs;
    __host__ __device__ uint32_t operator()(const uint32_t& j) const { return jobs[j].e1 - jobs[j].e0 + TM_JOB_W0; }
};
__global__ void k_tm_chunks(const uint32_t* pex, uint32_t njobs, uint32_t chunk_work, uint32_t* chunk_start, uint32_t* n_chunks) {
    const uint32_t j = blockIdx.x * blockDim.x + threadIdx.x;
    if (j >= njobs) return;
    const uint32_t ck = pex[j] / chunk_work;
    const int64_t prev = j ? (int64_t)(pex[j - 1] / chunk_work) : -1;
    for (int64_t k = prev + 1; k <= (int64_t)ck; ++k) chunk_start[k] = j;
    if (j == njobs - 1) { chunk_start[ck + 1] = njobs; *n_chunks = ck + 1; }
}

static int plan_tiles(lsg_ctx* c, hipStream_t st) {
    const uint32_t T = c->n_tiles >> c->wsh;
    const uint64_t N = c->tm_n;
    DevBuf &per_tile = c->bt[BT_PER_TILE], &offs = c->bt[BT_OFFS];
    if (per_tile.reserve((size_t)(T + 2) * 4 * 4) || offs.reserve((size_t)(T + 2) * 4 * 4 + 64)) return -1;
    uint32_t* ne = per_tile.as<uint32_t>(); uint32_t* nj = ne + (T + 2); uint32_t* slabs = nj + (T + 2); uint32_t* multi = slabs + (T + 2);
    uint32_t* ne_off = offs.as<uint32_t>(); uint32_t* job_off = ne_off + (T + 2); uint32_t* slab_off = job_off + (T + 2); uint32_t* multi_off = slab_off + (T + 2);
    uint32_t* d_misc = multi_off + (T + 2);
    uint32_t job_tgt = TM_JOB_TGT;
    { const uint64_t per = N / ((uint64_t)c->n_cus * 14 * 4); if (per < job_tgt) job_tgt = (uint32_t)(per < 768 ? 768 : per); }
    hipLaunchKernelGGL(k_tm_tiles, dim3((T + 256) / 256), dim3(256), 0, st, c->d_tile_cap.as<uint32_t>(), T, c->n_ct, job_tgt, 1u << c->wsh, ne, nj, slabs, multi);
    SCAN_U32(ne, ne_off, T + 1); SCAN_U32(nj, job_off, T + 1); SCAN_U32(slabs, slab_off, T + 1); SCAN_U32(multi, multi_off, T + 1);
    LSG_HIP(hipMemsetAsync(d_misc, 0, 8, st));
    uint32_t* srcs[4] = {ne_off, job_off, slab_off, multi_off};
    for (int i = 0; i < 4; ++i) LSG_HIP(hipMemcpyAsync(&c->plan1_tot[i], srcs[i] + T, 4, hipMemcpyDeviceToHost, st));
    LSG_HIP(hipStreamSynchronize(st));
    const uint32_t n_net = c->plan1_tot[0], njobs = c->plan1_tot[1], n_mt = c->plan1_tot[3];
    const size_t n_ne = (size_t)n_net * (size_t)c->n_ct, n_multi = (size_t)n_mt * (size_t)c->n_ct;
    if (c->tm[TM_JOBS].reserve(((size_t)njobs + 1) * sizeof(TmJob)) || c->tm[TM_NE_UNITS].reserve((n_ne + 2) * 4) || c->tm[TM_NE_GEOM].reserve((n_ne + 2) * 8) ||
        c->tm[TM_NE_NSLOT].reserve((n_ne + 2) * 4) || c->tm[TM_NE_ACC].reserve((n_ne + 2) * 4) || c->tm[TM_MULTI].reserve((n_multi + 2) * 4)) return -1;
    LSG_HIP(hipMemsetAsync(c->tm[TM_NE_NSLOT].p, 0, (n_ne + 2) * 4, st));
    LSG_HIP(hipMemsetAsync(c->tm[TM_NE_ACC].p, 0, (n_ne + 2) * 4, st));
    LSG_HIP(hipStreamSynchronize(st));
    c->plan1_n_ct = c->n_ct;
    return 0;
}

static int plan_jobs(lsg_ctx* c, bool finish, const uint64_t* skey, int cb_bits) {
    hipStream_t st = c->stream;
    const RunSrc rs{c->tm[TM_S0].as<uint32_t>(), skey, skey ? (1u << cb_bits) - 1u : 0u};
    const uint32_t T = c->n_tiles >> c->wsh;
    DevBuf &per_tile = c->bt[BT_PER_TILE], &offs = c->bt[BT_OFFS];
    uint32_t* nj = per_tile.as<uint32_t>() + (T + 2);
    uint32_t* ne_off = offs.as<uint32_t>(); uint32_t* job_off = ne_off + (T + 2); uint32_t* slab_off = job_off + (T + 2); uint32_t* multi_off = slab_off + (T + 2);
    uint32_t* d_misc = multi_off + (T + 2);
    const uint32_t* tot = c->plan1_tot;
    const uint32_t njobs = tot[1], n_mt = tot[3];
    hipLaunchKernelGGL(k_tm_jobs, dim3((T + 255) / 256), dim3(256), 0, st, c->d_tile_base.as<uint32_t>(), c->n_contigs, c->n_ct, c->wsh, rs, c->d_tile_off.as<uint32_t>(),
                       c->d_tile_cap.as<uint32_t>(), c->tm[TM_BLK_OFF].as<uint32_t>(), ne_off, nj, job_off, slab_off, multi_off, T,
                       c->tm[TM_JOBS].as<TmJob>(), c->tm[TM_NE_UNITS].as<uint32_t>(), c->tm[TM_NE_GEOM].as<int2>(), c->tm[TM_NE_NSLOT].as<uint32_t>(),
                       c->tm[TM_NE_ACC].as<uint32_t>(), c->tm[TM_MULTI].as<uint32_t>(), d_misc);
    if (n_mt) hipLaunchKernelGGL(k_tm_jobs_multi, dim3(n_mt >> c->wsh), dim3(64), 0, st, c->n_ct, c->wsh, rs, c->d_tile_off.as<uint32_t>(), c->d_tile_cap.as<uint32_t>(), c->tm[TM_BLK_OFF].as<uint32_t>(),
                                 ne_off, nj, job_off, slab_off, c->tm[TM_MULTI].as<uint32_t>(), c->tm[TM_NE_UNITS].as<uint32_t>(), c->tm[TM_NE_GEOM].as<int2>(), n_mt >> c->wsh, c->tm[TM_JOBS].as<TmJob>(), d_misc);
    {
        DevBuf& pex = c->bt[BT_PEX];
        const uint64_t total_work = c->tm_np + (uint64_t)njobs * TM_JOB_W0;
        const uint64_t cw = total_work / ((uint64_t)c->n_cus * 14 * 6);
        const uint32_t chunk_work = (uint32_t)(cw < 256 ? 256 : (cw > TM_CHUNK_WORK ? TM_CHUNK_WORK : cw));
        if (pex.reserve(((size_t)njobs + 2) * 4) || c->tm[TM_CHUNKS].reserve(((size_t)(total_work / chunk_work) + 4) * 4)) return -1;
        hipcub::CountingInputIterator<uint32_t> iota(0);
        TmJobWork wf{c->tm[TM_JOBS].as<TmJob>()};
        hipcub::TransformInputIterator<uint32_t, TmJobWork, hipcub::CountingInputIterator<uint32_t>> it(iota, wf);
        SCAN_U32(it, pex.as<uint32_t>(), njobs);
        hipLaunchKernelGGL(k_tm_chunks, dim3((njobs + 255) / 256), dim3(256), 0, st, pex.as<uint32_t>(), njobs, chunk_work, c->tm[TM_CHUNKS].as<uint32_t>(), d_misc + 1);
    }
    LSG_HIP(hipMemcpyAsync(c->plan_misc, d_misc, 8, hipMemcpyDeviceToHost, st));
    c->d_plan_misc = d_misc;
    LSG_HIP(hipGetLastError());
    if (finish) LSG_HIP(hipStreamSynchronize(st));
    return 0;
}

static void plan_finish_tiles(lsg_ctx* c) {
    const uint32_t* tot = c->plan1_tot;
    c->tm_njobs = tot[1];
    c->tm_n_ne = (uint32_t)((size_t)tot[0] * (size_t)c->n_ct); c->tm_n_multi = (uint32_t)((size_t)tot[3] * (size_t)c->n_ct); c->tm_n_slabs = tot[2];
}
static void plan_finish(lsg_ctx* c) {
    plan_finish_tiles(c);
    c->tm_nchunks = c->plan_misc[1]; c->tm_n_wide = c->plan_misc[0];
    c->plan_n_ct = c->n_ct;
    if (getenv("LSG_TIMING")) {
        std::vector<TmJob> jobs(c->tm_njobs);
        uint32_t longest = 0;
        if (c->tm_njobs && hipMemcpy(jobs.data(), c->tm[TM_JOBS].p, (size_t)c->tm_njobs * sizeof(TmJob), hipMemcpyDeviceToHost) != hipSuccess) { (void)hipGetLastError(); return; }
        for (const TmJob& jb : jobs) if (!(jb.nj & TMJ_WIDE) && jb.e1 - jb.e0 > longest) longest = jb.e1 - jb.e0;
        fprintf(stderr, "[lsg] plan: %u jobs, %u multi-job tiles, %u wide, longest packed job %u entries\n", c->tm_njobs, c->plan1_tot[3], c->tm_n_wide, longest);
    }
}

int ensure_plan(lsg_ctx* c) {
    if (!c->tm_valid) { set_error("lsg_pileup_count: no reads loaded"); return -2; }
    if (c->plan_n_ct == c->n_ct) return 0;
    c->plan_n_ct = 0;
    c->tm_njobs = c->tm_nchunks = c->tm_n_ne = c->tm_n_multi = c->tm_n_slabs = c->tm_n_wide = 0;
    if (c->tm_nblk == 0) { c->plan_n_ct = c->n_ct; return 0; }
    if (c->plan1_n_ct != c->n_ct) { if (int rc = plan_tiles(c, c->stream)) return rc; }
    if (int rc = plan_jobs(c, true)) return rc;
    plan_finish(c);
    return 0;
}

}
```

Measured before the change: 3.596 billion.

## Merge tail kernels, batch memsets into prep ops, and defer chunk planning

The light and heavy tail-probability kernels are merged into one launch, with the grid partitioned by block index. Many hipMemsetAsync calls in the store build are replaced with a single batched k_prep_ops launch. Count preparation can now run early so its zeroing and read-stats work is skipped later. Planning is restructured: k_tm_units moves into plan_tiles, the two job kernels merge into one, and chunk creation is deferred until it is needed. The store build also tracks max cell barcode, and the bin queue moves to a separate scalars slot. Together these aim to cut launch count and serialization, at the cost of more complex state flags that could go stale.

```diff
diff --git a/longsom_amd/csrc/call.hip b/longsom_amd/csrc/call.hip
--- a/longsom_amd/csrc/call.hip
+++ b/longsom_amd/csrc/call.hip
@@ -391,10 +391,10 @@
     return bb_upper_tail(t.k, t.n, al, be, bb_pm0(t.n, al, be, a.lgc0[set]), a.lgcn[set]);
 }
 
-__global__ __launch_bounds__(256) void k_call_tails(CallArgs a) {
+__device__ __forceinline__ void tails_light(const CallArgs& a, uint32_t blk, uint32_t n_blk) {
     const uint64_t n_all = a.counters[CT_LIGHT] + (uint64_t)a.arena_waves * TASK_CHUNK;
     const uint64_t n = n_all < a.task_cap ? n_all : a.task_cap;
-    for (uint64_t i = (uint64_t)blockIdx.x * blockDim.x + threadIdx.x; i < n; i += (uint64_t)gridDim.x * blockDim.x) {
+    for (uint64_t i = (uint64_t)blk * blockDim.x + threadIdx.x; i < n; i += (uint64_t)n_blk * blockDim.x) {
         const TailTask t = a.light[i];
         if (!(t.dst & ~1ull)) continue;
         *reinterpret_cast<int16_t*>(t.dst & ~1ull) = (int16_t)round4(tail_of_task(t, a));
@@ -453,11 +453,11 @@
     }
 }
 
-__global__ __launch_bounds__(256) void k_call_tails_heavy(CallArgs a) {
+__device__ __forceinline__ void tails_heavy(const CallArgs& a, uint32_t n_blk) {
     const int lane = threadIdx.x & 63;
     const uint64_t n_all = a.counters[CT_HEAVY] + (uint64_t)a.arena_waves * HEAVY_CHUNK;
     const uint64_t n_tasks = n_all < a.task_cap ? n_all : a.task_cap;
-    const uint64_t n_waves = ((uint64_t)gridDim.x * blockDim.x) >> 6;
+    const uint64_t n_waves = ((uint64_t)n_blk * blockDim.x) >> 6;
     uint64_t batch = ((uint64_t)blockIdx.x * blockDim.x + threadIdx.x) >> 6;
     const uint64_t n_batches = (n_tasks + 15) / 16;
     while (batch < n_batches) {
@@ -488,6 +488,11 @@
         if (lane == 0) nb = atomicAdd(&a.counters[CT_QTAIL], 1ull) + n_waves;
         batch = ((uint64_t)(uint32_t)__builtin_amdgcn_readfirstlane((int)(uint32_t)(nb >> 32)) << 32) | (uint32_t)__builtin_amdgcn_readfirstlane((int)(uint32_t)nb);
     }
+}
+
+__global__ __launch_bounds__(256) void k_call_tails(CallArgs a, uint32_t heavy_blocks) {
+    if (blockIdx.x < heavy_blocks) tails_heavy(a, heavy_blocks);
+    else tails_light(a, blockIdx.x - heavy_blocks, gridDim.x - heavy_blocks);
 }
 
 __global__ void k_call_finish(CallArgs a, uint32_t n_sites) {
@@ -730,8 +735,7 @@
             case 3: hipLaunchKernelGGL(k_call_gather<3>, dim3(gather_grid), dim3(GATHER_WAVES * 64), 0, st, a); break;
             default: hipLaunchKernelGGL(k_call_gather<4>, dim3(gather_grid), dim3(GATHER_WAVES * 64), 0, st, a); break;
         }
-        hipLaunchKernelGGL(k_call_tails, dim3((unsigned)(c->n_cus * 16)), dim3(256), 0, st, a);
-        hipLaunchKernelGGL(k_call_tails_heavy, dim3((unsigned)(c->n_cus * 8)), dim3(256), 0, st, a);
+        hipLaunchKernelGGL(k_call_tails, dim3((unsigned)(c->n_cus * 24)), dim3(256), 0, st, a, (uint32_t)(c->n_cus * 8));
         hipLaunchKernelGGL(k_call_finish, dim3((unsigned)(c->n_cus * 2)), dim3(256), 0, st, a, n_sites);
         LSG_HIP(hipGetLastError());
     }
diff --git a/longsom_amd/csrc/lsg_ctx.h b/longsom_amd/csrc/lsg_ctx.h
--- a/longsom_amd/csrc/lsg_ctx.h
+++ b/longsom_amd/csrc/lsg_ctx.h
@@ -150,6 +150,11 @@
 struct GatherCountSrc { const uint16_t* events; int64_t n_events; const uint64_t* key; const uint32_t* rdv; int32_t cb_bits; int32_t src_shift; int32_t wsh; };
 int unit_row_offsets(lsg_ctx* c, int ct, const uint32_t** off);
 int run_gather_count(lsg_ctx* c, const lsg_count_params* p, const GatherCountSrc& src, bool direct);
+struct PrepOp { void* dst; const void* src; uint64_t words; };
+struct PrepArgs { PrepOp op[10]; int n; };
+int prep_ops(lsg_ctx* c, hipStream_t st, const PrepArgs& pa);
+int count_prepare_early(lsg_ctx* c, const lsg_count_params* p, hipStream_t s);
+constexpr int SCALARS_BIN_QUEUE = 256;
 }
 
 struct lsg_ctx {
@@ -199,6 +204,9 @@
     uint32_t plan1_tot[4] = {0, 0, 0, 0};
     uint32_t plan_misc[2] = {0, 0};
     uint32_t* d_plan_misc = nullptr;
+    bool prep_early = false;
+    uint32_t prep_early_n_ne = 0;
+    bool tm_chunks_made = false;
     bool cal_enabled = false; lsg_count_params cal_params{};
     bool counted_at_load = false;
     bool load_was_fused = false;
diff --git a/longsom_amd/csrc/pileup.hip b/longsom_amd/csrc/pileup.hip
--- a/longsom_amd/csrc/pileup.hip
+++ b/longsom_amd/csrc/pileup.hip
@@ -1596,9 +1596,7 @@
     if (unsigned long long* slots = src.stat_slots()) stat_add(slots, blockIdx.x, s_ev, s_sg, s_ne, lane);
 }
 
-struct CountLaunch { CountArgs a; TmArgs tm; unsigned grid_walk, grid_fin; int n_pass; };
-struct PrepOp { void* dst; const void* src; uint64_t words; };
-struct PrepArgs { PrepOp op[10]; int n; };
+struct CountLaunch { CountArgs a; TmArgs tm; unsigned grid_walk, grid_fin; int n_pass; bool early; };
 __global__ __launch_bounds__(256) void k_prep_ops(PrepArgs a) {
     const uint64_t g = (uint64_t)blockIdx.x * blockDim.x + threadIdx.x, gs = (uint64_t)gridDim.x * blockDim.x;
     for (int k = 0; k < a.n; ++k) {
@@ -1609,9 +1607,39 @@
         for (uint64_t i = nq * 4 + g; i < a.op[k].words; i += gs) d[i] = sp ? sp[i] : 0u;
     }
 }
+int prep_ops(lsg_ctx* c, hipStream_t st, const PrepArgs& pa) {
+    hipLaunchKernelGGL(k_prep_ops, dim3((unsigned)(c->n_cus * 4)), dim3(256), 0, st, pa);
+    LSG_HIP(hipGetLastError());
+    return 0;
+}
+int count_prepare_early(lsg_ctx* c, const lsg_count_params* p, hipStream_t s) {
+    c->prep_early = false;
+    const uint32_t n_ne = c->tm_n_ne;
+    if (c->d_scalars.reserve(SC_COUNT * 8) || c->d_ix_stat.reserve(IX_STAT_SLOTS * 64) || c->d_ne_mask.reserve(((size_t)n_ne + 2) * 8) ||
+        c->d_ne_rowbase.reserve(((size_t)n_ne + 2) * 4) || c->d_xcd_queues.reserve(8 * 128)) return -1;
+    c->has_drops = false; c->n_depth_dropped = 0;
+    CountArgs a{};
+    fill_args(c, p, a);
+    if (a.adm) return 0;
+    PrepArgs pa{}; int k = 0;
+    auto op = [&](void* dst, size_t bytes) { pa.op[k].dst = dst; pa.op[k].src = nullptr; pa.op[k].words = (bytes + 3) / 4; ++k; };
+    op(c->d_scalars.p, SC_COUNT * 8);
+    op(c->d_ix_stat.p, IX_STAT_SLOTS * 64);
+    op(c->d_xcd_queues.p, 8 * 128);
+    if (n_ne) { op(c->d_ne_mask.p, ((size_t)n_ne + 1) * 8); op(c->d_ne_rowbase.p, ((size_t)n_ne + 1) * 4); }
+    pa.n = k;
+    if (int rc = prep_ops(c, s, pa)) return rc;
+    const int64_t R = c->rd.n_reads;
+    if (R > 0) { unsigned g = (unsigned)((R + 255) / 256); if (g > (unsigned)(c->n_cus * 8)) g = (unsigned)(c->n_cus * 8); hipLaunchKernelGGL(k_read_stats, dim3(g), dim3(256), 0, s, a); }
+    LSG_HIP(hipGetLastError());
+    c->prep_early = true; c->prep_early_n_ne = n_ne;
+    return 0;
+}
 static int count_prepare(lsg_ctx* c, const lsg_count_params* p, CountLaunch& L) {
     hipStream_t st = c->stream;
     const uint32_t n_ne = c->tm_n_ne;
+    const bool was_early = c->prep_early && c->prep_early_n_ne == n_ne;
+    c->prep_early = false;
     if (c->d_scalars.reserve(SC_COUNT * 8) || c->d_ne_units.reserve(((size_t)n_ne + 2) * 4) ||
         c->d_ne_mask.reserve(((size_t)n_ne + 2) * 8) || c->d_ne_rowbase.reserve(((size_t)n_ne + 2) * 4) || c->ws[WS_NE_NSLOT].reserve(((size_t)n_ne + 2) * 4) ||
         c->ws[WS_NE_ACC].reserve(((size_t)n_ne + 2) * 4) || c->ws[WS_NE_GEOM].reserve(((size_t)n_ne + 2) * 8) || c->ws[WS_MULTI_LIST].reserve(((size_t)c->tm_n_multi + 2) * 4) ||
@@ -1639,6 +1667,7 @@
     c->n_ne = n_ne; c->n_multi = c->tm_n_multi;
     L.a = CountArgs{};
     fill_args(c, p, L.a);
+    L.early = was_early && !L.a.adm;
     TmArgs& tm = L.tm;
     tm = TmArgs{};
     tm.store = c->tm[TM_STORE].as<uint4>(); tm.s0 = c->tm[TM_S0].as<uint32_t>(); tm.b = c->tm[TM_B].as<uint8_t>(); tm.rd = c->tm[TM_RD].as<uint32_t>();
@@ -1648,22 +1677,26 @@
     {
         PrepArgs pa{}; int k = 0;
         auto op = [&](void* dst, const void* src, size_t bytes) { if (bytes) { pa.op[k].dst = dst; pa.op[k].src = src; pa.op[k].words = (bytes + 3) / 4; ++k; } };
-        op(c->d_scalars.p, nullptr, SC_COUNT * 8);
-        op(c->d_ix_stat.p, nullptr, IX_STAT_SLOTS * 64);
+        if (!L.early) {
+            op(c->d_scalars.p, nullptr, SC_COUNT * 8);
+            op(c->d_ix_stat.p, nullptr, IX_STAT_SLOTS * 64);
+        }
         if (n_ne) {
             op(c->d_ne_units.p, c->tm[TM_NE_UNITS].p, (size_t)n_ne * 4);
             op(c->ws[WS_NE_GEOM].p, c->tm[TM_NE_GEOM].p, (size_t)n_ne * 8);
             op(c->ws[WS_NE_NSLOT].p, c->tm[TM_NE_NSLOT].p, ((size_t)n_ne + 1) * 4);
             op(c->ws[WS_NE_ACC].p, c->tm[TM_NE_ACC].p, ((size_t)n_ne + 1) * 4);
             if (c->tm_n_multi) op(c->ws[WS_MULTI_LIST].p, c->tm[TM_MULTI].p, (size_t)c->tm_n_multi * 4);
-            op(c->d_ne_mask.p, nullptr, ((size_t)n_ne + 1) * 8);
-            op(c->d_ne_rowbase.p, nullptr, ((size_t)n_ne + 1) * 4);
+            if (!L.early) {
+                op(c->d_ne_mask.p, nullptr, ((size_t)n_ne + 1) * 8);
+                op(c->d_ne_rowbase.p, nullptr, ((size_t)n_ne + 1) * 4);
+            }
         }
         pa.n = k;
-        hipLaunchKernelGGL(k_prep_ops, dim3((unsigned)(c->n_cus * 4)), dim3(256), 0, st, pa);
+        if (k) { if (int rc = prep_ops(c, st, pa)) return rc; }
     }
     const int64_t R = c->rd.n_reads;
-    if (R > 0) { unsigned g = (unsigned)((R + 255) / 256); if (g > (unsigned)(c->n_cus * 8)) g = (unsigned)(c->n_cus * 8); hipLaunchKernelGGL(k_read_stats, dim3(g), dim3(256), 0, st, L.a); }
+    if (R > 0 && !L.early) { unsigned g = (unsigned)((R + 255) / 256); if (g > (unsigned)(c->n_cus * 8)) g = (unsigned)(c->n_cus * 8); hipLaunchKernelGGL(k_read_stats, dim3(g), dim3(256), 0, st, L.a); }
     return 0;
 }
 static int count_passes(lsg_ctx* c, CountLaunch& L, int first_pass, bool wide_of_pass0) {
@@ -1741,7 +1774,7 @@
     const char* what = "k_tm_gather_count";
     if (direct) {
         if (c->d_xcd_queues.reserve(8 * 128)) return -1;
-        LSG_HIP(hipMemsetAsync(c->d_xcd_queues.p, 0, 8 * 128, st));
+        if (!L.early) LSG_HIP(hipMemsetAsync(c->d_xcd_queues.p, 0, 8 * 128, st));
         tg.queues = c->d_xcd_queues.as<unsigned long long>();
     }
     if (form == WINDOWS) {
diff --git a/longsom_amd/csrc/store.hip b/longsom_amd/csrc/store.hip
--- a/longsom_amd/csrc/store.hip
+++ b/longsom_amd/csrc/store.hip
@@ -29,6 +29,7 @@
     int32_t lf_min_mq, lf_ignore_orphans; uint32_t lf_flag_exclude;
     uint32_t* bad;
     unsigned long long* n_ev;
+    int32_t* max_cb;
     int32_t* span_diff;
     int32_t* cap_diff;
     int32_t window;
@@ -47,9 +48,10 @@
     __shared__ uint32_t hkey[SEG_H];
     __shared__ int32_t hval[SEG_H];
     __shared__ unsigned long long s_ev;
+    __shared__ int32_t s_cb;
     __shared__ uint32_t s_new, s_flush;
     for (int i = threadIdx.x; i < SEG_H; i += SEG_THREADS) { hkey[i] = KEY_INVALID; hval[i] = 0; }
-    if (threadIdx.x == 0) { s_ev = 0; s_new = 0; s_flush = 0; }
+    if (threadIdx.x == 0) { s_ev = 0; s_cb = 0; s_new = 0; s_flush = 0; }
     auto slot = [&](uint32_t t) -> int {
         uint32_t h = (t * 2654435761u) >> 21;
         for (int tries = 0; tries < 16; ++tries) {
@@ -63,6 +65,7 @@
     auto mark = [&](uint32_t t, int32_t v) { const int h = slot(t); if (h >= 0) atomicAdd(&hval[h], v); else atomicAdd(a.span_diff + t, v); };
     auto mark_cap = [&](uint32_t t, int32_t v) { const int h = slot(t); if (h >= 0) atomicAdd(&hval[h], v * 65536); else atomicAdd(a.cap_diff + t, v); };
     unsigned long long n_ev = 0;
+    int32_t max_cb = 0;
     bool unphased = false;
     constexpr int64_t BATCH = (int64_t)SEG_THREADS * SEG_U;
     const int64_t n_batches = (a.n_segs + BATCH - 1) / BATCH;
@@ -114,6 +117,7 @@
                         key = (uint32_t)cb | (((flag >> 4) & 1u) << 24);
                         tb = tb_[u];
                         n_ev += (unsigned long long)ln;
+                        max_cb = cb > max_cb ? cb : max_cb;
                         unphased |= ((o - st) & (int64_t)((64 << a.wsh) - 1)) != 0;
                         mark_cap((tb + ((uint32_t)st >> 6)) >> a.wsh, 1);
                         mark_cap(((tb + ((uint32_t)(st + ln - 1) >> 6)) >> a.wsh) + 1, -1);
@@ -165,11 +169,13 @@
             __syncthreads();
         }
     }
-    for (int o = 32; o > 0; o >>= 1) n_ev += __shfl_down(n_ev, o);
+    for (int o = 32; o > 0; o >>= 1) { n_ev += __shfl_down(n_ev, o); const int32_t u = __shfl_down(max_cb, o); max_cb = u > max_cb ? u : max_cb; }
     __syncthreads();
     if ((threadIdx.x & 63) == 0 && n_ev) atomicAdd(&s_ev, n_ev);
+    if ((threadIdx.x & 63) == 0 && max_cb) atomicMax(&s_cb, max_cb);
     __syncthreads();
     if (threadIdx.x == 0 && s_ev) atomicAdd(a.n_ev, s_ev);
+    if (threadIdx.x == 0 && s_cb) atomicMax(a.max_cb, s_cb);
     if (__syncthreads_or(unphased ? 1 : 0) && threadIdx.x == 0) atomicOr(a.bad, 4u);
 }
 
@@ -388,6 +394,7 @@
     uint32_t n_chunks;
     TtAgg1* agg1; int32_t* din; TtAgg2* agg2; TtAgg2* in2;
     uint32_t* cap; uint32_t* tile_off; uint32_t* blk_off; uint32_t* netile;
+    uint32_t* cursor;
     uint32_t* d_small; unsigned long long* d_sum;
 };
 template <int NT, class V>
@@ -513,7 +520,7 @@
 #pragma unroll
         for (int k = 0; k < 4; ++k) {
             if (i0 + k < hi) {
-                a.tile_off[i0 + k] = ec; a.blk_off[i0 + k] = eb;
+                a.tile_off[i0 + k] = ec; a.cursor[i0 + k] = ec; a.blk_off[i0 + k] = eb;
                 if (nv[k]) a.netile[en] = i0 + k;
             }
             ec += cv[k]; eb += bv[k]; en += nv[k];
@@ -633,7 +640,7 @@
 enum { BT_KEY_A = 0, BT_KEY_B, BT_VAL_A, BT_VAL_B, BT_PEX, BT_NETILE, BT_SEG_BEGIN, BT_SEG_END, BT_TMP, BT_PER_TILE, BT_OFFS, BT_SPAN, BT_CURSOR, BT_LPT, BT_COPY_TMP, BT_N };
 
 void drop_store(lsg_ctx* c) {
-    c->tm_valid = false; c->plan_n_ct = 0; c->plan1_n_ct = 0; c->tm_n = 0; c->tm_events = 0; c->tm_np = 0; c->tm_nblk = 0; c->tm_njobs = 0; c->tm_nchunks = 0;
+    c->tm_valid = false; c->plan_n_ct = 0; c->plan1_n_ct = 0; c->tm_n = 0; c->tm_events = 0; c->tm_np = 0; c->tm_nblk = 0; c->tm_njobs = 0; c->tm_nchunks = 0; c->tm_chunks_made = false; c->prep_early = false;
     c->tm_n_ne = 0; c->tm_n_multi = 0; c->tm_n_slabs = 0; c->tm_n_wide = 0;
     c->max_live_reads = -1; c->max_live_all = -1; c->max_live_exact = -1; c->has_drops = false;
     c->counted = c->called = false; c->counted_at_load = false; c->load_was_fused = false; c->store_skipped = false;
@@ -649,7 +656,8 @@
 }
 
 static int plan_tiles(lsg_ctx* c, hipStream_t st);
-static int plan_jobs(lsg_ctx* c, bool finish, const uint64_t* skey = nullptr, int cb_bits = 0);
+static int plan_jobs(lsg_ctx* c, bool finish, const uint64_t* skey = nullptr, int cb_bits = 0, bool chunks = true);
+static int plan_chunks(lsg_ctx* c);
 static void plan_finish(lsg_ctx* c);
 static void plan_finish_tiles(lsg_ctx* c);
 
@@ -696,11 +704,22 @@
     for (auto& v : c->build_ms) v = 0;
     c->st_min_mq = c->lf_min_mq; c->st_flag_exclude = c->lf_flag_exclude; c->st_ignore_orphans = c->lf_ignore_orphans;
     if (c->d_tile_cap.reserve(((size_t)T + 2) * 4) || c->d_tile_off.reserve(((size_t)T + 2) * 4) || c->d_scalars.reserve(512 * 8)) return -1;
-    LSG_HIP(hipMemsetAsync(c->d_tile_cap.p, 0, ((size_t)T + 2) * 4, st));
-    LSG_HIP(hipMemsetAsync(c->d_tile_off.p, 0, ((size_t)T + 2) * 4, st));
-    if (S <= 0 || T == 0) { LSG_HIP(hipStreamSynchronize(st)); return finish(); }
-    if (c->ws[WS_SEG_INFO].reserve(((size_t)S + 1) * 8)) return -1;
-    LSG_HIP(hipMemsetAsync(c->d_scalars.p, 0, 64, st));
+    if (S <= 0 || T == 0) {
+        LSG_HIP(hipMemsetAsync(c->d_tile_cap.p, 0, ((size_t)T + 2) * 4, st));
+        LSG_HIP(hipMemsetAsync(c->d_tile_off.p, 0, ((size_t)T + 2) * 4, st));
+        LSG_HIP(hipStreamSynchronize(st));
+        return finish();
+    }
+    if (c->ws[WS_SEG_INFO].reserve(((size_t)S + 1) * 8) || c->bt[BT_SPAN].reserve(((size_t)T + 2) * 4) || c->bt[BT_PER_TILE].reserve(((size_t)T + 2) * 4) ||
+        c->bt[BT_CURSOR].reserve(((size_t)T + 2) * 4)) return -1;
+    {
+        PrepArgs pa{}; int k = 0;
+        for (void* q : {c->d_tile_cap.p, c->d_tile_off.p, c->bt[BT_SPAN].p, c->bt[BT_PER_TILE].p}) { pa.op[k].dst = q; pa.op[k].src = nullptr; pa.op[k].words = (uint64_t)T + 2; ++k; }
+        pa.op[k].dst = c->d_scalars.p; pa.op[k].src = nullptr; pa.op[k].words = 16; ++k;
+        pa.op[k].dst = c->d_scalars.as<unsigned long long>() + SCALARS_BIN_QUEUE; pa.op[k].src = nullptr; pa.op[k].words = 2; ++k;
+        pa.n = k;
+        if (int rc = prep_ops(c, st, pa)) return rc;
+    }
     BuildArgs a{};
     a.n_reads = R; a.n_segs = S; a.n_events = n_events;
     const lsg_reads& in = src ? *src : c->rd;
@@ -710,30 +729,20 @@
     a.seg_info = c->ws[WS_SEG_INFO].as<uint2>(); a.tile_cap = c->d_tile_cap.as<uint32_t>();
     a.lf_min_mq = c->lf_min_mq; a.lf_flag_exclude = c->lf_flag_exclude; a.lf_ignore_orphans = c->lf_ignore_orphans;
     a.window = c->plp_window; c->st_window = c->plp_window; a.wsh = wsh;
-    a.qhead = c->d_scalars.as<unsigned long long>(); a.bad = reinterpret_cast<uint32_t*>(c->d_scalars.as<unsigned long long>() + 2);
+    a.qhead = c->d_scalars.as<unsigned long long>() + SCALARS_BIN_QUEUE; a.bad = reinterpret_cast<uint32_t*>(c->d_scalars.as<unsigned long long>() + 2);
     a.n_ev = c->d_scalars.as<unsigned long long>() + 3;
-    if (c->bt[BT_SPAN].reserve(((size_t)T + 2) * 4)) return -1;
-    LSG_HIP(hipMemsetAsync(c->bt[BT_SPAN].p, 0, ((size_t)T + 2) * 4, st));
+    a.max_cb = reinterpret_cast<int32_t*>(c->d_scalars.as<unsigned long long>() + 5);
     a.span_diff = c->bt[BT_SPAN].as<int32_t>();
     uint32_t* d_small = reinterpret_cast<uint32_t*>(c->d_scalars.as<unsigned long long>() + 4);
     DevBuf& tmp = c->bt[BT_TMP];
     LSG_HIP(hipEventRecord(c->evb[0], st));
     unsigned g_seg = (unsigned)((S + 256 * SEG_U - 1) / (256 * SEG_U)); if (g_seg > (unsigned)(c->n_cus * 16)) g_seg = (unsigned)(c->n_cus * 16);
     unsigned g_bin = (unsigned)((S + 256 * BIN_SUPER - 1) / (256 * BIN_SUPER)); if (g_bin > (unsigned)(c->n_cus * 8)) g_bin = (unsigned)(c->n_cus * 8);
-    if (c->bt[BT_PER_TILE].reserve(((size_t)T + 2) * 4)) return -1;
-    LSG_HIP(hipMemsetAsync(c->bt[BT_PER_TILE].p, 0, ((size_t)T + 2) * 4, st));
     a.cap_diff = c->bt[BT_PER_TILE].as<int32_t>();
     hipLaunchKernelGGL(k_seg_static, dim3(g_seg), dim3(256), 0, st, a);
     if (c->bt[BT_NETILE].reserve(((size_t)T + 2) * 4) || c->tm[TM_BLK_OFF].reserve(((size_t)T + 2) * 4)) return -1;
     uint32_t* blk_off = c->tm[TM_BLK_OFF].as<uint32_t>();
     unsigned long long* d_sum = c->d_scalars.as<unsigned long long>() + 8;
-    {
-        size_t tb = 0;
-        LSG_HIP(hipcub::DeviceReduce::Max(nullptr, tb, in.read_cb, reinterpret_cast<int32_t*>(d_small + 2), (int)(R > 0 ? R : 1), st));
-        if (tmp.reserve(tb + 256 + 64 * 1024)) return -1;
-        tb = tmp.cap;
-        if (R > 0) LSG_HIP(hipcub::DeviceReduce::Max(tmp.p, tb, in.read_cb, reinterpret_cast<int32_t*>(d_small + 2), (int)R, st));
-    }
     {
         if (c->d_cub_tmp.reserve(64 * 1024)) return -1;
         TtArgs ta{};
@@ -745,6 +754,7 @@
         ta.agg1 = reinterpret_cast<TtAgg1*>(scratch); ta.agg2 = reinterpret_cast<TtAgg2*>(scratch + 16 * 1024); ta.in2 = reinterpret_cast<TtAgg2*>(scratch + 32 * 1024);
         ta.din = reinterpret_cast<int32_t*>(scratch + 48 * 1024);
         ta.cap = c->d_tile_cap.as<uint32_t>(); ta.tile_off = c->d_tile_off.as<uint32_t>(); ta.blk_off = blk_off; ta.netile = c->bt[BT_NETILE].as<uint32_t>();
+        ta.cursor = c->bt[BT_CURSOR].as<uint32_t>();
         ta.d_small = d_small; ta.d_sum = d_sum;
         hipLaunchKernelGGL(k_tt_marks, dim3(ta.n_chunks), dim3(TT_THREADS), 0, st, ta);
         hipLaunchKernelGGL(k_tt_scan1, dim3(1), dim3(TT_MAX_CHUNKS), 0, st, ta);
@@ -803,11 +813,8 @@
     }
     if (win && !keys_only) return RUNG_TILE_KEYS;
     if (keys_only && getenv("LSG_TIMING")) fprintf(stderr, "[lsg] load: keys alone through the scatter and the sort (8 bytes an entry)%s\n", win ? ", entries binned by 128-position windows" : "");
-    if (key_a.reserve(N * 8 + 16) || key_b.reserve(N * 8 + 16) || (!keys_only && (val_a.reserve(N * 4 + 16) || val_b.reserve(N * 4 + 16))) ||
-        c->bt[BT_CURSOR].reserve(((size_t)T + 2) * 4)) return -1;
+    if (key_a.reserve(N * 8 + 16) || key_b.reserve(N * 8 + 16) || (!keys_only && (val_a.reserve(N * 4 + 16) || val_b.reserve(N * 4 + 16)))) return -1;
     a.cursor = c->bt[BT_CURSOR].as<uint32_t>(); a.key = key_a.as<uint64_t>(); a.rdv = keys_only ? nullptr : val_a.as<uint32_t>(); a.cb_bits = bits; a.src_shift = src_shift;
-    LSG_HIP(hipMemcpyAsync(a.cursor, c->d_tile_off.p, ((size_t)T + 1) * 4, hipMemcpyDeviceToDevice, st));
-    LSG_HIP(hipMemsetAsync(c->d_scalars.p, 0, 8, st));
     hipLaunchKernelGGL(k_bin, dim3(g_bin), dim3(BIN_THREADS), 0, st, a);
     LSG_HIP(hipEventRecord(c->evb[1], st));
     if (c->tm[TM_BLK_TILE].reserve(((size_t)nblk + 2) * 4)) return -1;
@@ -857,6 +864,7 @@
     if (tiles_planned) {
         if (int rc = plan_tiles(c, c->copy_stream)) return rc;
         plan_finish_tiles(c);
+        if (keys_only) { if (int rc = count_prepare_early(c, &c->cal_params, c->copy_stream)) return rc; }
     }
     if (n_netile) {
         const size_t seg_pitch = ((size_t)n_netile + 64) & ~(size_t)63;
@@ -916,10 +924,10 @@
     }
     const bool dbg = getenv("LSG_DEBUG_SYNC") != nullptr;
     auto stage = [&](const char* what) { if (dbg) { const hipError_t e = hipStreamSynchronize(st); fprintf(stderr, "[lsg] fused load: %s: %s\n", what, hipGetErrorString(e)); fflush(stderr); } };
-    auto fused_plan = [&]() -> int {
+    auto fused_plan = [&](bool chunks) -> int {
         stage("scatter + sort + block tables");
         c->tm_np = np; c->tm_nblk = nblk;
-        if (int rc = plan_jobs(c, false, key_b.as<uint64_t>(), bits)) return rc;
+        if (int rc = plan_jobs(c, false, key_b.as<uint64_t>(), bits, chunks)) return rc;
         stage("plan");
         return 0;
     };
@@ -928,7 +936,7 @@
     if (win && !fused) return RUNG_TILE_KEYS;
     if (keys_only && getenv("LSG_TEST_KEYS_ONLY_REFUSED")) return win ? RUNG_TILE_KEYS : RUNG_TILE_VALUES;
     if (fused && skip_store) {
-        if (int rc = fused_plan()) return rc;
+        if (int rc = fused_plan(false)) return rc;
         planned = true;
         const int rc = run_gather_count(c, &c->cal_params, gsrc, true);
         LSG_HIP(hipStreamSynchronize(st));
@@ -954,7 +962,7 @@
         if (int rc = blk_tiles(st)) return rc;
     }
     if (fused) {
-        if (int rc = fused_plan()) return rc;
+        if (int rc = fused_plan(true)) return rc;
         c->tm_valid = true;
         int rc = run_gather_count(c, &c->cal_params, gsrc, false);
         LSG_HIP(hipStreamSynchronize(st));
@@ -986,6 +994,7 @@
             plan_rc = plan_jobs(c, false);
         }
     }
+    if (planned && !c->tm_chunks_made && c->tm_njobs) plan_rc = plan_chunks(c);
     LSG_HIP(hipStreamSynchronize(st));
     if (plan_early) LSG_HIP(hipStreamSynchronize(c->copy_stream));
     if (plan_rc) return plan_rc;
@@ -1041,15 +1050,13 @@
     if (e1 - e0 > (uint32_t)TM_JOB_LIMIT) { jb.nj |= TMJ_WIDE; atomicAdd(n_wide, 1u); }
     *out = jb;
 }
-__global__ void k_tm_jobs(const uint32_t* tile_base, int n_contigs, int n_ct, int wsh, RunSrc rs, const uint32_t* tile_off, const uint32_t* cap, const uint32_t* blk_off, const uint32_t* ne_off,
-                          const uint32_t* nj, const uint32_t* job_off, const uint32_t* slab_off, const uint32_t* multi_off, uint32_t n_tiles, TmJob* jobs,
-                          uint32_t* ne_units, int2* ne_geom, uint32_t* ne_nslot, uint32_t* ne_acc, uint32_t* multi, uint32_t* n_wide) {
+__global__ void k_tm_units(const uint32_t* tile_base, int n_contigs, int n_ct, int wsh, const uint32_t* cap, const uint32_t* ne_off, const uint32_t* nj, const uint32_t* slab_off,
+                           const uint32_t* multi_off, uint32_t n_tiles, uint32_t* ne_units, int2* ne_geom, uint32_t* ne_nslot, uint32_t* ne_acc, uint32_t* multi) {
     const uint32_t t = blockIdx.x * blockDim.x + threadIdx.x;
     if (t >= n_tiles) return;
     const uint32_t n = cap[t];
     if (!n) return;
     const uint32_t J = nj[t], ord = ne_off[t];
-    const uint64_t base = (uint64_t)blk_off[t] * 8;
     const uint32_t tile0 = t << wsh;
     int tid = 0;
     { int lo = 0, hi = n_contigs; while (hi - lo > 1) { const int mid = (lo + hi) >> 1; if (tile_base[mid] <= tile0) lo = mid; else hi = mid; } tid = lo; }
@@ -1063,19 +1070,28 @@
         ne_acc[w] = J > 1 ? slab_off[t] + (h * (uint32_t)n_ct + (uint32_t)ct) * J : 0u;
         if (J > 1) multi[(multi_off[t] + h) * (uint32_t)n_ct + ct] = w;
     }
-    if (J > 1) return;
-    tm_make_job(rs, base, tile_off[t], n, 1u, 0u, ord * (uint32_t)n_ct, 0xFFFFFFFFu, t, make_int2(tstart, tid), jobs + job_off[t], n_wide);
-}
-__global__ __launch_bounds__(64) void k_tm_jobs_multi(int n_ct, int wsh, RunSrc rs, const uint32_t* tile_off, const uint32_t* cap, const uint32_t* blk_off, const uint32_t* ne_off, const uint32_t* nj,
-                                                      const uint32_t* job_off, const uint32_t* slab_off, const uint32_t* multi, const uint32_t* ne_units, const int2* ne_geom, uint32_t n_mt,
-                                                      TmJob* jobs, uint32_t* n_wide) {
-    const uint32_t i = blockIdx.x;
+}
+constexpr int TM_JOBS_THREADS = 256;
+__global__ __launch_bounds__(TM_JOBS_THREADS) void k_tm_jobs(int n_ct, int wsh, RunSrc rs, const uint32_t* tile_off, const uint32_t* cap, const uint32_t* blk_off, const uint32_t* ne_off,
+                                                             const uint32_t* nj, const uint32_t* job_off, const uint32_t* slab_off, const uint32_t* multi, const uint32_t* ne_units,
+                                                             const int2* ne_geom, uint32_t n_tiles, uint32_t n_mt, TmJob* jobs, uint32_t* n_wide) {
+    const uint32_t nb1 = (n_tiles + TM_JOBS_THREADS - 1) / TM_JOBS_THREADS;
+    if (blockIdx.x < nb1) {
+        const uint32_t t = blockIdx.x * TM_JOBS_THREADS + threadIdx.x;
+        if (t >= n_tiles) return;
+        const uint32_t n = cap[t];
+        if (!n || nj[t] > 1) return;
+        const uint32_t w0 = ne_off[t] * (uint32_t)n_ct;
+        tm_make_job(rs, (uint64_t)blk_off[t] * 8, tile_off[t], n, 1u, 0u, w0, 0xFFFFFFFFu, t, ne_geom[w0], jobs + job_off[t], n_wide);
+        return;
+    }
+    const uint32_t i = (blockIdx.x - nb1) * (TM_JOBS_THREADS / 64) + (threadIdx.x >> 6);
     if (i >= n_mt) return;
     const uint32_t w = multi[((size_t)i << wsh) * (uint32_t)n_ct], t = (ne_units[w] / (uint32_t)n_ct) >> wsh;
     const uint32_t n = cap[t], J = nj[t];
     const int2 geom = ne_geom[w];
     const uint64_t base = (uint64_t)blk_off[t] * 8;
-    for (uint32_t j = threadIdx.x; j < J; j += 64u)
+    for (uint32_t j = threadIdx.x & 63u; j < J; j += 64u)
         tm_make_job(rs, base, tile_off[t], n, J, j, ne_off[t] * (uint32_t)n_ct, slab_off[t] + j, t, geom, jobs + job_off[t] + j, n_wide);
 }
 struct TmJobWork {
@@ -1113,12 +1129,35 @@
         c->tm[TM_NE_NSLOT].reserve((n_ne + 2) * 4) || c->tm[TM_NE_ACC].reserve((n_ne + 2) * 4) || c->tm[TM_MULTI].reserve((n_multi + 2) * 4)) return -1;
     LSG_HIP(hipMemsetAsync(c->tm[TM_NE_NSLOT].p, 0, (n_ne + 2) * 4, st));
     LSG_HIP(hipMemsetAsync(c->tm[TM_NE_ACC].p, 0, (n_ne + 2) * 4, st));
+    hipLaunchKernelGGL(k_tm_units, dim3((T + 255) / 256), dim3(256), 0, st, c->d_tile_base.as<uint32_t>(), c->n_contigs, c->n_ct, c->wsh, c->d_tile_cap.as<uint32_t>(), ne_off, nj, slab_off,
+                       multi_off, T, c->tm[TM_NE_UNITS].as<uint32_t>(), c->tm[TM_NE_GEOM].as<int2>(), c->tm[TM_NE_NSLOT].as<uint32_t>(), c->tm[TM_NE_ACC].as<uint32_t>(), c->tm[TM_MULTI].as<uint32_t>());
+    LSG_HIP(hipGetLastError());
     LSG_HIP(hipStreamSynchronize(st));
     c->plan1_n_ct = c->n_ct;
     return 0;
 }
 
-static int plan_jobs(lsg_ctx* c, bool finish, const uint64_t* skey, int cb_bits) {
+static int plan_chunks(lsg_ctx* c) {
+    hipStream_t st = c->stream;
+    const uint32_t njobs = c->plan1_tot[1];
+    uint32_t* d_misc = c->d_plan_misc;
+    DevBuf& pex = c->bt[BT_PEX];
+    const uint64_t total_work = c->tm_np + (uint64_t)njobs * TM_JOB_W0;
+    const uint64_t cw = total_work / ((uint64_t)c->n_cus * 14 * 6);
+    const uint32_t chunk_work = (uint32_t)(cw < 256 ? 256 : (cw > TM_CHUNK_WORK ? TM_CHUNK_WORK : cw));
+    if (pex.reserve(((size_t)njobs + 2) * 4) || c->tm[TM_CHUNKS].reserve(((size_t)(total_work / chunk_work) + 4) * 4)) return -1;
+    hipcub::CountingInputIterator<uint32_t> iota(0);
+    TmJobWork wf{c->tm[TM_JOBS].as<TmJob>()};
+    hipcub::TransformInputIterator<uint32_t, TmJobWork, hipcub::CountingInputIterator<uint32_t>> it(iota, wf);
+    SCAN_U32(it, pex.as<uint32_t>(), njobs);
+    hipLaunchKernelGGL(k_tm_chunks, dim3((njobs + 255) / 256), dim3(256), 0, st, pex.as<uint32_t>(), njobs, chunk_work, c->tm[TM_CHUNKS].as<uint32_t>(), d_misc + 1);
+    LSG_HIP(hipMemcpyAsync(c->plan_misc, d_misc, 8, hipMemcpyDeviceToHost, st));
+    LSG_HIP(hipGetLastError());
+    c->tm_chunks_made = true;
+    return 0;
+}
+
+static int plan_jobs(lsg_ctx* c, bool finish, const uint64_t* skey, int cb_bits, bool chunks) {
     hipStream_t st = c->stream;
     const RunSrc rs{c->tm[TM_S0].as<uint32_t>(), skey, skey ? (1u << cb_bits) - 1u : 0u};
     const uint32_t T = c->n_tiles >> c->wsh;
@@ -1126,28 +1165,15 @@
     uint32_t* nj = per_tile.as<uint32_t>() + (T + 2);
     uint32_t* ne_off = offs.as<uint32_t>(); uint32_t* job_off = ne_off + (T + 2); uint32_t* slab_off = job_off + (T + 2); uint32_t* multi_off = slab_off + (T + 2);
     uint32_t* d_misc = multi_off + (T + 2);
-    const uint32_t* tot = c->plan1_tot;
-    const uint32_t njobs = tot[1], n_mt = tot[3];
-    hipLaunchKernelGGL(k_tm_jobs, dim3((T + 255) / 256), dim3(256), 0, st, c->d_tile_base.as<uint32_t>(), c->n_contigs, c->n_ct, c->wsh, rs, c->d_tile_off.as<uint32_t>(),
-                       c->d_tile_cap.as<uint32_t>(), c->tm[TM_BLK_OFF].as<uint32_t>(), ne_off, nj, job_off, slab_off, multi_off, T,
-                       c->tm[TM_JOBS].as<TmJob>(), c->tm[TM_NE_UNITS].as<uint32_t>(), c->tm[TM_NE_GEOM].as<int2>(), c->tm[TM_NE_NSLOT].as<uint32_t>(),
-                       c->tm[TM_NE_ACC].as<uint32_t>(), c->tm[TM_MULTI].as<uint32_t>(), d_misc);
-    if (n_mt) hipLaunchKernelGGL(k_tm_jobs_multi, dim3(n_mt >> c->wsh), dim3(64), 0, st, c->n_ct, c->wsh, rs, c->d_tile_off.as<uint32_t>(), c->d_tile_cap.as<uint32_t>(), c->tm[TM_BLK_OFF].as<uint32_t>(),
-                                 ne_off, nj, job_off, slab_off, c->tm[TM_MULTI].as<uint32_t>(), c->tm[TM_NE_UNITS].as<uint32_t>(), c->tm[TM_NE_GEOM].as<int2>(), n_mt >> c->wsh, c->tm[TM_JOBS].as<TmJob>(), d_misc);
-    {
-        DevBuf& pex = c->bt[BT_PEX];
-        const uint64_t total_work = c->tm_np + (uint64_t)njobs * TM_JOB_W0;
-        const uint64_t cw = total_work / ((uint64_t)c->n_cus * 14 * 6);
-        const uint32_t chunk_work = (uint32_t)(cw < 256 ? 256 : (cw > TM_CHUNK_WORK ? TM_CHUNK_WORK : cw));
-        if (pex.reserve(((size_t)njobs + 2) * 4) || c->tm[TM_CHUNKS].reserve(((size_t)(total_work / chunk_work) + 4) * 4)) return -1;
-        hipcub::CountingInputIterator<uint32_t> iota(0);
-        TmJobWork wf{c->tm[TM_JOBS].as<TmJob>()};
-        hipcub::TransformInputIterator<uint32_t, TmJobWork, hipcub::CountingInputIterator<uint32_t>> it(iota, wf);
-        SCAN_U32(it, pex.as<uint32_t>(), njobs);
-        hipLaunchKernelGGL(k_tm_chunks, dim3((njobs + 255) / 256), dim3(256), 0, st, pex.as<uint32_t>(), njobs, chunk_work, c->tm[TM_CHUNKS].as<uint32_t>(), d_misc + 1);
-    }
-    LSG_HIP(hipMemcpyAsync(c->plan_misc, d_misc, 8, hipMemcpyDeviceToHost, st));
+    const uint32_t n_mt = c->plan1_tot[3];
+    const uint32_t n_mb = n_mt >> c->wsh;
+    hipLaunchKernelGGL(k_tm_jobs, dim3((T + TM_JOBS_THREADS - 1) / TM_JOBS_THREADS + (n_mb + TM_JOBS_THREADS / 64 - 1) / (TM_JOBS_THREADS / 64)), dim3(TM_JOBS_THREADS), 0, st, c->n_ct, c->wsh, rs,
+                       c->d_tile_off.as<uint32_t>(), c->d_tile_cap.as<uint32_t>(), c->tm[TM_BLK_OFF].as<uint32_t>(), ne_off, nj, job_off, slab_off, c->tm[TM_MULTI].as<uint32_t>(),
+                       c->tm[TM_NE_UNITS].as<uint32_t>(), c->tm[TM_NE_GEOM].as<int2>(), T, n_mb, c->tm[TM_JOBS].as<TmJob>(), d_misc);
     c->d_plan_misc = d_misc;
+    c->tm_chunks_made = false; c->tm_nchunks = 0;
+    if (chunks) { if (int rc = plan_chunks(c)) return rc; }
+    else LSG_HIP(hipMemcpyAsync(c->plan_misc, d_misc, 8, hipMemcpyDeviceToHost, st));
     LSG_HIP(hipGetLastError());
     if (finish) LSG_HIP(hipStreamSynchronize(st));
     return 0;
@@ -1160,7 +1186,7 @@
 }
 static void plan_finish(lsg_ctx* c) {
     plan_finish_tiles(c);
-    c->tm_nchunks = c->plan_misc[1]; c->tm_n_wide = c->plan_misc[0];
+    c->tm_nchunks = c->tm_chunks_made ? c->plan_misc[1] : 0u; c->tm_n_wide = c->plan_misc[0];
     c->plan_n_ct = c->n_ct;
     if (getenv("LSG_TIMING")) {
         std::vector<TmJob> jobs(c->tm_njobs);
@@ -1173,7 +1199,13 @@
 
 int ensure_plan(lsg_ctx* c) {
     if (!c->tm_valid) { set_error("lsg_pileup_count: no reads loaded"); return -2; }
-    if (c->plan_n_ct == c->n_ct) return 0;
+    if (c->plan_n_ct == c->n_ct) {
+        if (c->tm_chunks_made || c->tm_nblk == 0 || c->tm_njobs == 0) return 0;
+        if (int rc = plan_chunks(c)) return rc;
+        LSG_HIP(hipStreamSynchronize(c->stream));
+        c->tm_nchunks = c->plan_misc[1];
+        return 0;
+    }
     c->plan_n_ct = 0;
     c->tm_njobs = c->tm_nchunks = c->tm_n_ne = c->tm_n_multi = c->tm_n_slabs = c->tm_n_wide = 0;
     if (c->tm_nblk == 0) { c->plan_n_ct = c->n_ct; return 0; }
```

Result: no change. 3.631 billion, median of 6 (+1.0%).
